# OPTML-Group/Unlearn-Saliency

Hardware: AMD Instinct MI355X
Metric: unlearn_steps_per_sec (ResNet-18/CIFAR-10 10%-forget, RL + SalUn mask, batch 256/GPU) (higher is better)
Workload: dtype f32

## Files before the change

include/salun.h:

```cpp
#ifndef SALUN_H
#define SALUN_H

#include <stddef.h>
#include <stdint.h>

#ifdef __cplusplus
extern "C" {
#endif

#define SALUN_OK 0
#define SALUN_EINVAL (-22)
#define SALUN_ENOSPC (-28)
#define SALUN_EIO (-5)

#define SALUN_MAX_THRESHOLDS 16

typedef void *salun_stream_t;

int salun_version(void);
const char *salun_strerror(int code);
const char *salun_arch(void);
int salun_clock_probe(unsigned long long *out , int samples, int spins, salun_stream_t stream);

int salun_saliency_accumulate(float *acc , const float *g ,
                              double scale, const float *sqnorm ,
                              double max_norm, int64_t n, salun_stream_t stream);

#define SALUN_TOPK_FORCE_FULL_SCAN 1u
#define SALUN_TOPK_VALUES_ONLY 2u
size_t salun_mask_topk_workspace_bytes(int64_t n, int nk);
int salun_mask_topk(const float *acc , int64_t n, const int64_t *ks ,
                    int nk, uint8_t *const *masks_out ,
                    void *ws , size_t ws_bytes, salun_stream_t stream);
int salun_mask_topk_ex(const float *acc , int64_t n, const int64_t *ks ,
                       int nk, uint8_t *const *masks_out ,
                       void *ws , size_t ws_bytes, unsigned flags, salun_stream_t stream);
int salun_mask_topk_status(const void *ws , int *route_out , int *error_out ,
                           salun_stream_t stream);
int salun_mask_topk_thresholds(const void *ws , int nk, float *tau_out ,
                               salun_stream_t stream);

int salun_mask_u8_to_i64(const uint8_t *m , int64_t *out , int64_t n,
                         salun_stream_t stream);
int salun_mask_i64_to_u8(const int64_t *m , uint8_t *out , int64_t n,
                         salun_stream_t stream);
int salun_mask_popcount(const uint8_t *m , int64_t n, int64_t *count ,
                        void *ws , size_t ws_bytes, salun_stream_t stream);

int salun_masked_sgd_step(float *p , const float *g , float *buf ,
                          const uint8_t *m , double lr, double mu,
                          double wd, int first_step, int64_t n, salun_stream_t stream);

size_t salun_reduce_workspace_bytes(int64_t n);
int salun_grad_sqnorm(const float *g , int64_t n, float *out ,
                      void *ws , size_t ws_bytes, salun_stream_t stream);

int salun_masked_adam_step(float *p , const float *g , float *m1 ,
                           float *v , const uint8_t *mask ,
                           const float *sqnorm , double max_norm,
                           double gscale, double lr, double b1, double b2, double eps,
                           double wd, int step, int64_t n, salun_stream_t stream);

int salun_adam_coefficients(int64_t *step , double lr, double b1, double b2, float *coef ,
                            salun_stream_t stream);
int salun_masked_adam_step_coef(float *p , const float *g , float *m1 , float *v ,
                                const uint8_t *mask , const float *sqnorm ,
                                double max_norm, double gscale, const float *coef , double b1, double b2,
                                double eps, double wd, int64_t n, salun_stream_t stream);

int salun_adam_ema_step(float *p , const float *g , float *m1 , float *v ,
                        float *shadow , const uint8_t *mask ,
                        const float *sqnorm , double max_norm, double gscale, double lr, double b1,
                        double b2, double eps, double wd, double mu, int step, int64_t n, salun_stream_t stream);
int salun_adam_ema_step_coef(float *p , const float *g , float *m1 , float *v ,
                             float *shadow , const uint8_t *mask ,
                             const float *sqnorm , double max_norm, double gscale,
                             const float *coef , double b1, double b2, double eps, double wd, double mu,
                             int64_t n, salun_stream_t stream);

int salun_qsample(const float *x0 , const float *e ,
                  const float *sqrt_ab , const float *sqrt_1mab ,
                  const int64_t *t , int64_t T, float *xt , int64_t B,
                  int64_t chw, salun_stream_t stream);

size_t salun_sqerr_workspace_bytes(int64_t B, int64_t chw);
int salun_sqerr_loss(const float *a , const float *b , int64_t B,
                     int64_t chw, double coef, float *loss ,
                     float *per_sample , float *dloss_db ,
                     void *ws , size_t ws_bytes, salun_stream_t stream);

int salun_fim_square_accumulate(float *F , float *tmp , double n_data,
                                int64_t n, salun_stream_t stream);

int salun_conv2d_forward(const float *x , const float *w , const float *bias ,
                         float *y , int N, int C, int H, int W, int K, int R, int stride, int pad,
                         int P, int Q, salun_stream_t stream);
int salun_conv2d_forward_fused(const float *x , const float *w , const float *bias ,
                               const float *nbias , const float *addend ,
                               float *y , int N, int C, int H, int W, int K, int R, int stride, int pad,
                               int P, int Q, void *ws , size_t ws_bytes, salun_stream_t stream);
size_t salun_conv2d_data_workspace_bytes(int N, int outC, int outH, int outW, int R, int conv_stride);
int salun_conv2d_backward_data_ws(const float *dy , const float *w , const float *addend ,
                                  float *dx , int N, int C, int H, int W, int K, int R, int stride, int pad,
                                  int P, int Q, void *ws , size_t ws_bytes, salun_stream_t stream);
int salun_conv2d_backward_data(const float *dy , const float *w , float *dx , int N, int C,
                               int H, int W, int K, int R, int stride, int pad, int P, int Q,
                               salun_stream_t stream);
int salun_conv2d_backward_data_add(const float *dy , const float *w , const float *addend ,
                                   float *dx , int N, int C, int H, int W, int K, int R, int stride, int pad,
                                   int P, int Q, salun_stream_t stream);
size_t salun_channel_sum_workspace_bytes(int N, int K);
int salun_channel_sum(const float *dy , float *out , int N, int K, int HW, int accumulate,
                      void *ws , size_t ws_bytes, salun_stream_t stream);
size_t salun_conv2d_wgrad_workspace_bytes(int N, int C, int K, int R, int P, int Q);
int salun_conv2d_backward_weight(const float *x , const float *dy , float *dw , int N, int C,
                                 int H, int W, int K, int R, int stride, int pad, int P, int Q, int accumulate,
                                 void *ws , size_t ws_bytes, salun_stream_t stream);
#define SALUN_WGRAD_SHARED 1u
int salun_conv2d_backward_weight_ex(const float *x , const float *dy , float *dw , int N, int C,
                                    int H, int W, int K, int R, int stride, int pad, int P, int Q, int accumulate,
                                    unsigned flags, void *ws , size_t ws_bytes, salun_stream_t stream);
#define SALUN_ROUTE_FORWARD 0
#define SALUN_ROUTE_BACKWARD_DATA 1
#define SALUN_ROUTE_BACKWARD_WEIGHT 2
#define SALUN_ROUTE_EPI 2u
#define SALUN_ROUTE_W_UNALIGNED 4u
#define SALUN_ROUTE_OUT_UNALIGNED 8u
#define SALUN_ROUTE_IN_UNALIGNED 16u
int salun_conv2d_route(int direction, int N, int C, int H, int W, int K, int R, int stride, int pad, int P, int Q,
                       unsigned flags, size_t ws_bytes, char *buf, size_t buflen, int *nsplit );

size_t salun_conv3x3_pack_bytes(int K, int C, int dgrad);
#define SALUN_PACK_MAX_JOBS 32
typedef struct {
  const float *w;
  float *img_fwd;
  float *img_dgrad;
  int32_t K, C;
} salun_pack_job_t;
int salun_conv3x3_pack_weights(const salun_pack_job_t *jobs , int njobs, salun_stream_t stream);
int salun_conv3x3_packed(const float *x , const float *img , const float *bias ,
                         const float *nbias , const float *addend , float *y ,
                         int N, int Cred, int H, int W, int Kout, int cfg, salun_stream_t stream);

int salun_conv2d_bf16_supported(int C, int K, int R, int stride, int pad);
int salun_conv2d_bf16_pack_weights(const float *w , uint16_t *wp , int K, int C, int R,
                                   salun_stream_t stream);
#define SALUN_BF16_PACK_MAX_JOBS 64
typedef struct {
  const float *w;
  uint16_t *wp;
  int32_t K, C, R, transposed;
} salun_bf16_pack_job_t;
int salun_bf16_pack_weights_batch(const salun_bf16_pack_job_t *jobs, int n, salun_stream_t stream);
size_t salun_conv2d_bf16_data_workspace_bytes(int N, int H, int W, int C, int K, int R, int stride, int pad);
int salun_conv2d_bf16_forward(const uint16_t *x , const uint16_t *wp , const float *bias ,
                              const float *nbias , const uint16_t *addend ,
                              uint16_t *y , int N, int H, int W, int C, int K, int R, int stride, int pad,
                              void *ws , size_t ws_bytes, salun_stream_t stream);
int salun_conv2d_bf16_backward_data(const uint16_t *dy , const uint16_t *wp ,
                                    const uint16_t *addend , uint16_t *dx , int N, int H, int W,
                                    int C, int K, int R, int stride, int pad, void *ws , size_t ws_bytes,
                                    salun_stream_t stream);
size_t salun_conv2d_bf16_wgrad_workspace_bytes(int N, int H, int W, int C, int K, int R, int stride, int pad);
int salun_conv2d_bf16_backward_weight(const uint16_t *x , const uint16_t *dy , float *dw ,
                                      float *db , int N, int H, int W, int C, int K, int R, int stride,
                                      int pad, int accumulate, void *ws , size_t ws_bytes,
                                      salun_stream_t stream);
size_t salun_colsum_bf16_workspace_bytes(int K);
int salun_colsum_bf16(const uint16_t *dy , float *db , float *dnb , int64_t M, int K,
                      int images, int accumulate, void *ws , size_t ws_bytes, salun_stream_t stream);
int salun_conv2d_bf16_backward_weight_ex(const uint16_t *x , const uint16_t *dy , float *dw ,
                                         float *db , float *dnb , int N, int H, int W, int C,
                                         int K, int R, int stride, int pad, int accumulate, void *ws ,
                                         size_t ws_bytes, salun_stream_t stream);
#define SALUN_ROUTE_RING_SHIFT 8
#define SALUN_ROUTE_RING(v) ((unsigned)((v) + 1) << SALUN_ROUTE_RING_SHIFT)
#define SALUN_ROUTE_WGRAD_TN_SHIFT 12
#define SALUN_ROUTE_WGRAD_TN(v) ((unsigned)((v) + 1) << SALUN_ROUTE_WGRAD_TN_SHIFT)
int salun_conv2d_bf16_route(int direction, int N, int H, int W, int C, int K, int R, int stride, int pad, unsigned flags,
                            size_t ws_bytes, char *buf, size_t buflen, int *nsplit );

size_t salun_gn_bf16_workspace_bytes(int N, int C, int HW, int G);
int salun_gn_bf16_forward(const uint16_t *x , const float *gamma , const float *beta ,
                          uint16_t *y , float *mr , float *ab , int N, int C, int HW, int G,
                          double eps, int silu, void *ws , size_t ws_bytes, salun_stream_t stream);
int salun_gn_bf16_backward(const uint16_t *dy , const uint16_t *x , const float *gamma ,
                           const float *mr , const float *ab , uint16_t *dx , float *dgamma ,
                           float *dbeta , int N, int C, int HW, int G, int silu, int accumulate, void *ws ,
                           size_t ws_bytes, salun_stream_t stream);

int salun_attn_supported(int D);
int salun_attn_forward(const uint16_t *q , const uint16_t *k , const uint16_t *v , uint16_t *o ,
                       float *lse , int B, int H, int Nq, int Nk, int D, long long q_bs, int q_ld,
                       long long k_bs, int k_ld, long long v_bs, int v_ld, long long o_bs, int o_ld, double scale,
                       salun_stream_t stream);
int salun_attn_backward(const uint16_t *q , const uint16_t *k , const uint16_t *v ,
                        const uint16_t *o , const uint16_t *d_o , const float *lse ,
                        uint16_t *dq , uint16_t *dk , uint16_t *dv , float *dsum , int B, int H,
                        int Nq, int Nk, int D, long long q_bs, int q_ld, long long k_bs, int k_ld, long long v_bs, int v_ld,
                        long long o_bs, int o_ld, long long do_bs, int do_ld, double scale, salun_stream_t stream);

size_t salun_ln_bf16_workspace_bytes(int64_t rows, int C);
int salun_ln_bf16_forward(const uint16_t *x , const float *gamma , const float *beta ,
                          uint16_t *y , float *stats , int64_t rows, int C, double eps,
                          salun_stream_t stream);
int salun_ln_bf16_backward(const uint16_t *dy , const uint16_t *x , const float *gamma ,
                           const float *stats , uint16_t *dx , float *dgamma , float *dbeta ,
                           int64_t rows, int C, int accumulate, void *ws , size_t ws_bytes, salun_stream_t stream);
int salun_geglu_bf16_forward(const uint16_t *h , uint16_t *out , int64_t rows, int F, salun_stream_t stream);
int salun_geglu_bf16_backward(const uint16_t *h , const uint16_t *dy , uint16_t *dh , int64_t rows,
                              int F, salun_stream_t stream);

size_t salun_bn_workspace_bytes(int C);
int salun_bn_forward(const float *x , const float *res , float *y ,
                     const float *gamma , const float *beta , float *running_mean ,
                     float *running_var , long long *num_batches_tracked ,
                     float *save_mean , float *save_invstd ,
                     int N, int C, int HW, int training, double momentum, double eps, int relu, void *ws ,
                     size_t ws_bytes, salun_stream_t stream);
int salun_bn_backward(const float *dy , const float *y , const float *x ,
                      const float *gamma , const float *save_mean , const float *save_invstd ,
                      float *dx , float *dres , float *dgamma , float *dbeta ,
                      float *grad_gamma_acc , float *grad_beta_acc ,
                      int N, int C, int HW, int training, int relu, void *ws , size_t ws_bytes,
                      salun_stream_t stream);

size_t salun_gn_workspace_bytes(int N, int C);
int salun_gn_forward(const float *x , float *y , const float *gamma , const float *beta ,
                     float *save_mean , float *save_rstd , int N, int C, int HW, int G, double eps,
                     int silu, salun_stream_t stream);
int salun_gn_backward(const float *dz , const float *x , const float *gamma ,
                      const float *beta , const float *save_mean , const float *save_rstd ,
                      float *dx , float *dgamma , float *dbeta ,
                      float *grad_gamma_acc , float *grad_beta_acc ,
                      int N, int C, int HW, int G, int silu, void *ws , size_t ws_bytes,
                      salun_stream_t stream);

int salun_gn_backward_fused(const float *dz , const float *x , const float *gamma ,
                            const float *beta , const float *save_mean , const float *save_rstd ,
                            const float *addend , float *dx , float *dgamma ,
                            float *dbeta , float *grad_gamma_acc ,
                            float *grad_beta_acc , float *nk_sum ,
                            float *csum , float *csum_acc , int N, int C, int HW, int G,
                            int silu, void *ws , size_t ws_bytes, salun_stream_t stream);

int salun_param_diff(const float *p , const float *p0 , float *out , int64_t n,
                     salun_stream_t stream);
int salun_soft_threshold_step(float *p , const float *p0 , const float *tau ,
                              int64_t n, salun_stream_t stream);

size_t salun_ewc_workspace_bytes(int64_t n);
int salun_ewc_penalty_grad(const float *p , const float *p_star , const float *F ,
                           float *g , double lambda, float *loss_out , int64_t n,
                           void *ws , size_t ws_bytes, salun_stream_t stream);

int salun_image_batch(const uint8_t *data , const int64_t *idx ,
                      const int32_t *crop , const uint8_t *flip ,
                      float *out , int64_t B, int H, int W, int C, int pad,
                      salun_stream_t stream);

#define SALUN_GEMM_MAX_JOBS 32
#define SALUN_GEMM_MAX_SEGS 32
typedef struct {
  const float *A , *B ;
  int32_t K;
  int32_t a_i, a_k, b_j, b_k;
} salun_gemm_seg_t;
typedef struct {
  float *C ;
  const float *bias ;
  int32_t M, N, ldc;
  int32_t seg0, nseg;
  int32_t accumulate;
} salun_gemm_job_t;
size_t salun_gemm_f32_workspace_bytes(const salun_gemm_job_t *jobs , int njobs,
                                      const salun_gemm_seg_t *segs , int nsegs,
                                      int batch_outer, int batch_inner);
int salun_gemm_f32(const salun_gemm_job_t *jobs , int njobs, const salun_gemm_seg_t *segs , int nsegs,
                   int batch_outer, int batch_inner, const int64_t *batch_strides ,
                   double alpha, void *ws , size_t ws_bytes, salun_stream_t stream);
typedef struct {
  int32_t tile, nsplit, nsplit_wanted, njobs, nsegs;
  int64_t tiles;
  int32_t nchunks[SALUN_GEMM_MAX_JOBS], per[SALUN_GEMM_MAX_JOBS], empty_shares[SALUN_GEMM_MAX_JOBS];
  int32_t tile0[SALUN_GEMM_MAX_JOBS], fast_tiles[SALUN_GEMM_MAX_JOBS];
  int32_t amode[SALUN_GEMM_MAX_SEGS], bmode[SALUN_GEMM_MAX_SEGS], chunk0[SALUN_GEMM_MAX_SEGS];
} salun_gemm_route_t;
int salun_gemm_f32_route(const salun_gemm_job_t *jobs , int njobs, const salun_gemm_seg_t *segs , int nsegs,
                         int batch_outer, int batch_inner, const int64_t *batch_strides ,
                         const void *ws , size_t ws_bytes, salun_gemm_route_t *out );
size_t salun_colsum_f32_workspace_bytes(int64_t M, int N);
int salun_colsum_f32(const float *x , float *out , int64_t M, int N, int64_t ld, int accumulate,
                     void *ws , size_t ws_bytes, salun_stream_t stream);
int salun_softmax_rows(float *s , int64_t rows, int n, int ld, salun_stream_t stream);
int salun_softmax_rows_backward(const float *p , float *dp , int64_t rows, int n, int ld,
                                double scale, salun_stream_t stream);

int salun_gemm_bf16_supported(int64_t M, int N, int K);
int salun_gemm_bf16_nt(const void *x , const void *w , const float *bias ,
                       const void *addend , void *y , int64_t M, int N, int K,
                       int variant, salun_stream_t stream);
int salun_gemm_bf16_tn_supported(int64_t M, int Na, int Nb);
size_t salun_gemm_bf16_tn_workspace_bytes(int64_t M, int Na, int Nb, int variant);
int salun_gemm_bf16_tn(const void *dy , const void *x , float *dw , int64_t M, int Na, int Nb,
                       int accumulate, int variant, void *ws , size_t ws_bytes, salun_stream_t stream);
#define SALUN_GEMM_BF16_NT 0
#define SALUN_GEMM_BF16_TN 1
int salun_gemm_bf16_route(int op, int64_t M, int N, int K, int variant, size_t ws_bytes, char *buf, size_t buflen,
                          int *nsplit );
int salun_pack_bf16(const float *w , void *wp , int N, int K, int transposed, salun_stream_t stream);

int salun_dropout(const float *x , float *y , int64_t n_samples, int64_t chw,
                  int64_t sample_offset, double p, uint64_t seed,
                  const uint64_t *seed_dev , salun_stream_t stream);
int salun_u64_add(uint64_t *value , uint64_t inc, salun_stream_t stream);

size_t salun_iu_dot_workspace_bytes(int B, int64_t n);
int salun_iu_conv_dot(const float *y2 , const float *dy , int B, int64_t n, double *out ,
                      void *ws , size_t ws_bytes, salun_stream_t stream);
int salun_iu_bn_dot(const float *x , const float *dy , const float *running_mean ,
                    const float *running_var , double eps, const float *u0_gamma ,
                    const float *u0_beta , const float *u1_gamma , const float *u1_beta ,
                    int B, int C, int HW, double *out , void *ws , size_t ws_bytes,
                    salun_stream_t stream);
int salun_iu_linear_dot(const float *x , const float *dy , const float *u0_w ,
                        const float *u0_b , const float *u1_w , const float *u1_b ,
                        int B, int M, int K, double *out , salun_stream_t stream);
int salun_iu_recurrence(const double *ab , int64_t n, double N, double *out ,
                        salun_stream_t stream);
int salun_iu_apply(float *p , const float *v , const float *g0 , const double *beta ,
                   const uint8_t *mask , double alpha, int64_t n, salun_stream_t stream);

size_t salun_ff_conv_sq_workspace_bytes(int G, int B, int C, int K, int R, int P, int Q);
int salun_ff_conv_sq(const float *x , const float *dy , const float *w , float *F ,
                     int G, int B, int C, int H, int W, int K, int R, int stride, int pad, int P, int Q,
                     void *ws , size_t ws_bytes, salun_stream_t stream);
int salun_ff_linear_sq(const float *x , const float *dy , const float *w , float *F ,
                       int G, int B, int M, int K, salun_stream_t stream);
size_t salun_ff_vec_sq_workspace_bytes(int G, int C);
int salun_ff_vec_sq(const float *x , const float *dy , const float *running_mean ,
                    const float *running_var , double eps, const float *w , int G, int B,
                    int C, int HW, float *F_gamma , float *F_beta , void *ws ,
                    size_t ws_bytes, salun_stream_t stream);
int salun_ff_apply(float *p , const float *F , const int64_t *table , int nparam, int64_t ntiles,
                   double nbatches, double alpha, uint64_t seed, salun_stream_t stream);

int salun_fill_uniform(float *out , int64_t n, uint64_t seed, double lo, double hi,
                       salun_stream_t stream);
int salun_fill_normal(float *out , int64_t n, uint64_t seed, double mean, double std,
                      salun_stream_t stream);
int salun_fill_u8(uint8_t *out , int64_t n, uint64_t seed, salun_stream_t stream);

#define SALUN_SAMPLER_ANCESTRAL 0
#define SALUN_SAMPLER_GENERALIZED 1
int salun_sampler_step(const float *x_t , const float *eps_cond , const float *eps_null ,
                       double cond_scale, const float *abar , int table_len, int idx_t, int idx_next, int variant,
                       double eta, const float *noise , uint64_t seed,
                       const int64_t *image_ids , int64_t step, float *x_next ,
                       float *x0 , int64_t B, int64_t chw, salun_stream_t stream);

int salun_sampler_noise(float *out , uint64_t seed, const int64_t *image_ids , int64_t step, int64_t B,
                        int64_t chw, salun_stream_t stream);

size_t salun_minmax_workspace_bytes(int64_t n);
int salun_minmax(const float *x , int64_t n, float *lohi , void *ws , size_t ws_bytes,
                 salun_stream_t stream);

int salun_images_to_u8(const float *x , uint8_t *out , int64_t B, int C, int HW, int rescaled,
                       const float *range , salun_stream_t stream);

int salun_ldm_ddim_step(const float *x , const float *eps2 , int guided, double scale,
                        double c_s1m, double c_sqrt_at, double c_dir, double c_sqrt_aprev, double c_sigma,
                        const float *z , float *x_prev , float *x0_out , int64_t B,
                        int64_t chw, salun_stream_t stream);

size_t salun_esd_loss_workspace_bytes(int64_t B, int64_t chw);
int salun_esd_loss(const float *e_n , const float *e_0p , int64_t B, int64_t chw,
                   double negative_guidance, float *loss , float *d_e_n ,
                   float *target , void *ws , size_t ws_bytes, salun_stream_t stream);

#define SALUN_PRUNE_MAX_SEGMENTS 512
size_t salun_prune_workspace_bytes(int64_t n_sel);
int salun_prune_global(float *p , float *buf , uint8_t *keep , int64_t n,
                       const int64_t *segs , int nseg, int64_t n_sel, int64_t alive, int64_t k_prune,
                       const float *rnd , unsigned flags, void *ws , size_t ws_bytes,
                       salun_stream_t stream);
int salun_prune_status(const void *ws , int64_t n_sel, int ranked, int *route_out ,
                       int *error_out , salun_stream_t stream);
int salun_prune_count_zeros(const float *p , int64_t n, const int64_t *segs , int nseg,
                            int64_t n_sel, int64_t *count , salun_stream_t stream);

#define SALUN_CLS_HEAD_MAX_C 8192
#define SALUN_CLS_HEAD_MAX_K 1024
size_t salun_cls_head_workspace_bytes(int64_t B, int C, int K);
int salun_cls_head_forward(const float *x , const float *w , const float *bias ,
                           const int64_t *labels , float *pooled , float *logits ,
                           float *p , float *loss , float *loss_mean ,
                           double *loss_sum , int64_t *hits ,
                           int64_t *count , int64_t B, int C, int HW, int K, void *ws ,
                           size_t ws_bytes, salun_stream_t stream);
int salun_cls_head_backward(const float *p , const float *pooled , const float *w ,
                            const int64_t *labels , const float *grad_out ,
                            float *dlogits , float *dx , float *dw ,
                            float *db , int accumulate_w, int accumulate_b, int64_t B, int C, int HW,
                            int K, salun_stream_t stream);

int salun_maxpool2x2_forward(const float *x , float *y , uint8_t *idx ,
                             int64_t NC, int H, int W, salun_stream_t stream);
int salun_maxpool2x2_backward(const float *dy , const uint8_t *idx , float *dx ,
                              int64_t NC, int H, int W, salun_stream_t stream);

#ifdef __cplusplus
}
#endif
#endif
```

unlearn_saliency_amd/_lib.py:

```python
from __future__ import annotations

import ctypes
import os
import subprocess

_HERE = os.path.dirname(os.path.abspath(__file__))
LIB_PATH = os.environ.get("SALUN_LIB") or os.path.join(_HERE, "libsalun.so")
CSRC_DIR = os.path.join(_HERE, "csrc")

SALUN_OK = 0
SALUN_EINVAL = -22
SALUN_ENOSPC = -28
SALUN_EIO = -5
SALUN_MAX_THRESHOLDS = 16
SALUN_TOPK_FORCE_FULL_SCAN = 1
SALUN_TOPK_VALUES_ONLY = 2
SALUN_WGRAD_SHARED = 1

c_void_p, c_int, c_int64, c_uint64 = ctypes.c_void_p, ctypes.c_int, ctypes.c_int64, ctypes.c_uint64
c_double, c_size_t = ctypes.c_double, ctypes.c_size_t

class GemmSeg(ctypes.Structure):
    _fields_ = [("A", c_void_p), ("B", c_void_p), ("K", ctypes.c_int32), ("a_i", ctypes.c_int32),
                ("a_k", ctypes.c_int32), ("b_j", ctypes.c_int32), ("b_k", ctypes.c_int32)]


class GemmJob(ctypes.Structure):
    _fields_ = [("C", c_void_p), ("bias", c_void_p), ("M", ctypes.c_int32), ("N", ctypes.c_int32),
                ("ldc", ctypes.c_int32), ("seg0", ctypes.c_int32), ("nseg", ctypes.c_int32),
                ("accumulate", ctypes.c_int32)]


class GemmRoute(ctypes.Structure):
    _fields_ = [(n, ctypes.c_int32) for n in ("tile", "nsplit", "nsplit_wanted", "njobs", "nsegs")] + \
               [("tiles", ctypes.c_int64)] + \
               [(n, ctypes.c_int32 * 32) for n in ("nchunks", "per", "empty_shares", "tile0", "fast_tiles", "amode", "bmode",
                                                   "chunk0")]


class PackJob(ctypes.Structure):
    _fields_ = [("w", c_void_p), ("img_fwd", c_void_p), ("img_dgrad", c_void_p), ("K", ctypes.c_int32),
                ("C", ctypes.c_int32)]


class Bf16PackJob(ctypes.Structure):
    _fields_ = [("w", c_void_p), ("wp", c_void_p), ("K", ctypes.c_int32), ("C", ctypes.c_int32), ("R", ctypes.c_int32),
                ("transposed", ctypes.c_int32)]


SALUN_BF16_PACK_MAX_JOBS = 64
SALUN_GEMM_MAX_JOBS = 32
SALUN_GEMM_MAX_SEGS = 32
SALUN_CLS_HEAD_MAX_C = 8192
SALUN_CLS_HEAD_MAX_K = 1024

SIGNATURES = {
    "salun_version": (c_int, []),
    "salun_strerror": (ctypes.c_char_p, [c_int]),
    "salun_arch": (ctypes.c_char_p, []),
    "salun_clock_probe": (c_int, [c_void_p, c_int, c_int, c_void_p]),
    "salun_saliency_accumulate": (c_int, [c_void_p, c_void_p, c_double, c_void_p, c_double, c_int64, c_void_p]),
    "salun_mask_topk_workspace_bytes": (c_size_t, [c_int64, c_int]),
    "salun_mask_topk": (c_int, [c_void_p, c_int64, ctypes.POINTER(c_int64), c_int, ctypes.POINTER(c_void_p),
                                c_void_p, c_size_t, c_void_p]),
    "salun_mask_topk_ex": (c_int, [c_void_p, c_int64, ctypes.POINTER(c_int64), c_int, ctypes.POINTER(c_void_p),
                                   c_void_p, c_size_t, ctypes.c_uint, c_void_p]),
    "salun_mask_topk_status": (c_int, [c_void_p, ctypes.POINTER(c_int), ctypes.POINTER(c_int), c_void_p]),
    "salun_mask_topk_thresholds": (c_int, [c_void_p, c_int, c_void_p, c_void_p]),
    "salun_mask_u8_to_i64": (c_int, [c_void_p, c_void_p, c_int64, c_void_p]),
    "salun_mask_i64_to_u8": (c_int, [c_void_p, c_void_p, c_int64, c_void_p]),
    "salun_mask_popcount": (c_int, [c_void_p, c_int64, c_void_p, c_void_p, c_size_t, c_void_p]),
    "salun_masked_sgd_step": (c_int, [c_void_p, c_void_p, c_void_p, c_void_p, c_double, c_double, c_double, c_int,
                                      c_int64, c_void_p]),
    "salun_reduce_workspace_bytes": (c_size_t, [c_int64]),
    "salun_grad_sqnorm": (c_int, [c_void_p, c_int64, c_void_p, c_void_p, c_size_t, c_void_p]),
    "salun_masked_adam_step": (c_int, [c_void_p, c_void_p, c_void_p, c_void_p, c_void_p, c_void_p, c_double,
                                       c_double, c_double, c_double, c_double, c_double, c_double, c_int, c_int64,
                                       c_void_p]),
    "salun_adam_coefficients": (c_int, [c_void_p, c_double, c_double, c_double, c_void_p, c_void_p]),
    "salun_masked_adam_step_coef": (c_int, [c_void_p, c_void_p, c_void_p, c_void_p, c_void_p, c_void_p, c_double,
                                            c_double, c_void_p, c_double, c_double, c_double, c_double, c_int64,
                                            c_void_p]),
    "salun_adam_ema_step": (c_int, [c_void_p, c_void_p, c_void_p, c_void_p, c_void_p, c_void_p, c_void_p, c_double,
                                    c_double, c_double, c_double, c_double, c_double, c_double, c_double, c_int, c_int64,
                                    c_void_p]),
    "salun_adam_ema_step_coef": (c_int, [c_void_p, c_void_p, c_void_p, c_void_p, c_void_p, c_void_p, c_void_p, c_double,
                                         c_double, c_void_p, c_double, c_double, c_double, c_double, c_double, c_int64,
                                         c_void_p]),
    "salun_qsample": (c_int, [c_void_p, c_void_p, c_void_p, c_void_p, c_void_p, c_int64, c_void_p, c_int64, c_int64,
                              c_void_p]),
    "salun_sqerr_workspace_bytes": (c_size_t, [c_int64, c_int64]),
    "salun_sqerr_loss": (c_int, [c_void_p, c_void_p, c_int64, c_int64, c_double, c_void_p, c_void_p, c_void_p,
                                 c_void_p, c_size_t, c_void_p]),
    "salun_fim_square_accumulate": (c_int, [c_void_p, c_void_p, c_double, c_int64, c_void_p]),
    "salun_conv2d_forward": (c_int, [c_void_p, c_void_p, c_void_p, c_void_p] + [c_int] * 10 + [c_void_p]),
    "salun_conv2d_forward_fused": (c_int, [c_void_p] * 6 + [c_int] * 10 + [c_void_p, c_size_t, c_void_p]),
    "salun_conv2d_data_workspace_bytes": (c_size_t, [c_int] * 6),
    "salun_conv2d_backward_data_ws": (c_int, [c_void_p] * 4 + [c_int] * 10 + [c_void_p, c_size_t, c_void_p]),
    "salun_conv2d_backward_data": (c_int, [c_void_p, c_void_p, c_void_p] + [c_int] * 10 + [c_void_p]),
    "salun_channel_sum_workspace_bytes": (c_size_t, [c_int] * 2),
    "salun_channel_sum": (c_int, [c_void_p, c_void_p] + [c_int] * 4 + [c_void_p, c_size_t, c_void_p]),
    "salun_conv2d_wgrad_workspace_bytes": (c_size_t, [c_int] * 6),
    "salun_conv3x3_pack_bytes": (c_size_t, [c_int] * 3),
    "salun_conv3x3_pack_weights": (c_int, [c_void_p, c_int, c_void_p]),
    "salun_conv3x3_packed": (c_int, [c_void_p] * 6 + [c_int] * 6 + [c_void_p]),
    "salun_conv2d_backward_weight": (c_int, [c_void_p, c_void_p, c_void_p] + [c_int] * 11 + [c_void_p, c_size_t,
                                                                                          c_void_p]),
    "salun_conv2d_backward_weight_ex": (c_int, [c_void_p, c_void_p, c_void_p] + [c_int] * 11 + [ctypes.c_uint, c_void_p,
                                                                                                 c_size_t, c_void_p]),
    "salun_conv2d_route": (c_int, [c_int] * 11 + [ctypes.c_uint, c_size_t, ctypes.c_char_p, c_size_t,
                                   ctypes.POINTER(c_int)]),
    "salun_conv2d_bf16_supported": (c_int, [c_int] * 5),
    "salun_conv2d_bf16_pack_weights": (c_int, [c_void_p, c_void_p, c_int, c_int, c_int, c_void_p]),
    "salun_bf16_pack_weights_batch": (c_int, [c_void_p, c_int, c_void_p]),
    "salun_conv2d_bf16_data_workspace_bytes": (c_size_t, [c_int] * 8),
    "salun_conv2d_bf16_forward": (c_int, [c_void_p] * 6 + [c_int] * 8 + [c_void_p, c_size_t, c_void_p]),
    "salun_conv2d_bf16_backward_data": (c_int, [c_void_p] * 4 + [c_int] * 8 + [c_void_p, c_size_t, c_void_p]),
    "salun_conv2d_bf16_wgrad_workspace_bytes": (c_size_t, [c_int] * 8),
    "salun_conv2d_bf16_backward_weight": (c_int, [c_void_p] * 4 + [c_int] * 9 + [c_void_p, c_size_t, c_void_p]),
    "salun_colsum_bf16_workspace_bytes": (c_size_t, [c_int]),
    "salun_colsum_bf16": (c_int, [c_void_p, c_void_p, c_void_p, c_int64, c_int, c_int, c_int, c_void_p, c_size_t, c_void_p]),
    "salun_conv2d_bf16_backward_weight_ex": (c_int, [c_void_p] * 5 + [c_int] * 9 + [c_void_p, c_size_t, c_void_p]),
    "salun_conv2d_bf16_route": (c_int, [c_int] * 9 + [ctypes.c_uint, c_size_t, ctypes.c_char_p, c_size_t,
                                        ctypes.POINTER(c_int)]),
    "salun_gn_bf16_workspace_bytes": (c_size_t, [c_int] * 4),
    "salun_gn_bf16_forward": (c_int, [c_void_p] * 6 + [c_int] * 4 + [c_double, c_int, c_void_p, c_size_t, c_void_p]),
    "salun_gn_bf16_backward": (c_int, [c_void_p] * 8 + [c_int] * 6 + [c_void_p, c_size_t, c_void_p]),
    "salun_attn_supported": (c_int, [c_int]),
    "salun_attn_forward": (c_int, [c_void_p] * 5 + [c_int] * 5 + [ctypes.c_longlong, c_int] * 4 + [c_double, c_void_p]),
    "salun_attn_backward": (c_int, [c_void_p] * 10 + [c_int] * 5 + [ctypes.c_longlong, c_int] * 5 + [c_double, c_void_p]),
    "salun_ln_bf16_workspace_bytes": (c_size_t, [c_int64, c_int]),
    "salun_ln_bf16_forward": (c_int, [c_void_p] * 5 + [c_int64, c_int, c_double, c_void_p]),
    "salun_ln_bf16_backward": (c_int, [c_void_p] * 7 + [c_int64, c_int, c_int, c_void_p, c_size_t, c_void_p]),
    "salun_geglu_bf16_forward": (c_int, [c_void_p, c_void_p, c_int64, c_int, c_void_p]),
    "salun_geglu_bf16_backward": (c_int, [c_void_p, c_void_p, c_void_p, c_int64, c_int, c_void_p]),
    "salun_bn_workspace_bytes": (c_size_t, [c_int]),
    "salun_bn_forward": (c_int, [c_void_p] * 10 + [c_int] * 4 + [c_double, c_double, c_int, c_void_p, c_size_t, c_void_p]),
    "salun_bn_backward": (c_int, [c_void_p] * 12 + [c_int] * 5 + [c_void_p, c_size_t, c_void_p]),
    "salun_conv2d_backward_data_add": (c_int, [c_void_p] * 4 + [c_int] * 10 + [c_void_p]),
    "salun_gn_workspace_bytes": (c_size_t, [c_int, c_int]),
    "salun_gn_forward": (c_int, [c_void_p] * 6 + [c_int] * 4 + [c_double, c_int, c_void_p]),
    "salun_gn_backward": (c_int, [c_void_p] * 11 + [c_int] * 5 + [c_void_p, c_size_t, c_void_p]),
    "salun_gn_backward_fused": (c_int, [c_void_p] * 15 + [c_int] * 5 + [c_void_p, c_size_t, c_void_p]),
    "salun_param_diff": (c_int, [c_void_p, c_void_p, c_void_p, c_int64, c_void_p]),
    "salun_soft_threshold_step": (c_int, [c_void_p, c_void_p, c_void_p, c_int64, c_void_p]),
    "salun_ewc_workspace_bytes": (c_size_t, [c_int64]),
    "salun_ewc_penalty_grad": (c_int, [c_void_p] * 4 + [c_double, c_void_p, c_int64, c_void_p, c_size_t, c_void_p]),
    "salun_image_batch": (c_int, [c_void_p, c_void_p, c_void_p, c_void_p, c_void_p, c_int64, c_int, c_int, c_int,
                                  c_int, c_void_p]),
    "salun_gemm_f32_workspace_bytes": (c_size_t, [ctypes.POINTER(GemmJob), c_int, ctypes.POINTER(GemmSeg), c_int, c_int,
                                                  c_int]),
    "salun_gemm_f32": (c_int, [ctypes.POINTER(GemmJob), c_int, ctypes.POINTER(GemmSeg), c_int, c_int, c_int,
                               ctypes.POINTER(c_int64), c_double, c_void_p, c_size_t, c_void_p]),
    "salun_gemm_f32_route": (c_int, [ctypes.POINTER(GemmJob), c_int, ctypes.POINTER(GemmSeg), c_int, c_int, c_int,
                                     ctypes.POINTER(c_int64), c_void_p, c_size_t, ctypes.POINTER(GemmRoute)]),
    "salun_colsum_f32_workspace_bytes": (c_size_t, [c_int64, c_int]),
    "salun_colsum_f32": (c_int, [c_void_p, c_void_p, c_int64, c_int, c_int64, c_int, c_void_p, c_size_t, c_void_p]),
    "salun_softmax_rows": (c_int, [c_void_p, c_int64, c_int, c_int, c_void_p]),
    "salun_softmax_rows_backward": (c_int, [c_void_p, c_void_p, c_int64, c_int, c_int, c_double, c_void_p]),
    "salun_gemm_bf16_supported": (c_int, [c_int64, c_int, c_int]),
    "salun_gemm_bf16_nt": (c_int, [c_void_p, c_void_p, c_void_p, c_void_p, c_void_p, c_int64, c_int, c_int, c_int, c_void_p]),
    "salun_pack_bf16": (c_int, [c_void_p, c_void_p, c_int, c_int, c_int, c_void_p]),
    "salun_gemm_bf16_tn_supported": (c_int, [c_int64, c_int, c_int]),
    "salun_gemm_bf16_tn_workspace_bytes": (c_size_t, [c_int64, c_int, c_int, c_int]),
    "salun_gemm_bf16_tn": (c_int, [c_void_p, c_void_p, c_void_p, c_int64, c_int, c_int, c_int, c_int, c_void_p, c_size_t, c_void_p]),
    "salun_gemm_bf16_route": (c_int, [c_int, c_int64, c_int, c_int, c_int, c_size_t, ctypes.c_char_p, c_size_t,
                                      ctypes.POINTER(c_int)]),
    "salun_dropout": (c_int, [c_void_p, c_void_p, c_int64, c_int64, c_int64, c_double, c_uint64, c_void_p, c_void_p]),
    "salun_u64_add": (c_int, [c_void_p, c_uint64, c_void_p]),
    "salun_iu_dot_workspace_bytes": (c_size_t, [c_int, c_int64]),
    "salun_iu_conv_dot": (c_int, [c_void_p, c_void_p, c_int, c_int64, c_void_p, c_void_p, c_size_t, c_void_p]),
    "salun_iu_bn_dot": (c_int, [c_void_p] * 4 + [c_double] + [c_void_p] * 4 + [c_int] * 3 + [c_void_p, c_void_p,
                                                                                           c_size_t, c_void_p]),
    "salun_iu_linear_dot": (c_int, [c_void_p] * 6 + [c_int] * 3 + [c_void_p, c_void_p]),
    "salun_iu_recurrence": (c_int, [c_void_p, c_int64, c_double, c_void_p, c_void_p]),
    "salun_iu_apply": (c_int, [c_void_p] * 5 + [c_double, c_int64, c_void_p]),
    "salun_ff_conv_sq_workspace_bytes": (c_size_t, [c_int] * 7),
    "salun_ff_conv_sq": (c_int, [c_void_p] * 4 + [c_int] * 11 + [c_void_p, c_size_t, c_void_p]),
    "salun_ff_linear_sq": (c_int, [c_void_p] * 4 + [c_int] * 4 + [c_void_p]),
    "salun_ff_vec_sq_workspace_bytes": (c_size_t, [c_int, c_int]),
    "salun_ff_vec_sq": (c_int, [c_void_p] * 4 + [c_double, c_void_p] + [c_int] * 4 + [c_void_p] * 3
                        + [c_size_t, c_void_p]),
    "salun_ff_apply": (c_int, [c_void_p] * 3 + [c_int, c_int64, c_double, c_double, c_uint64, c_void_p]),
    "salun_fill_uniform": (c_int, [c_void_p, c_int64, c_uint64, c_double, c_double, c_void_p]),
    "salun_fill_normal": (c_int, [c_void_p, c_int64, c_uint64, c_double, c_double, c_void_p]),
    "salun_fill_u8": (c_int, [c_void_p, c_int64, c_uint64, c_void_p]),
    "salun_sampler_step": (c_int, [c_void_p, c_void_p, c_void_p, c_double, c_void_p, c_int, c_int, c_int, c_int,
                                   c_double, c_void_p, c_uint64, c_void_p, c_int64, c_void_p, c_void_p, c_int64,
                                   c_int64, c_void_p]),
    "salun_sampler_noise": (c_int, [c_void_p, c_uint64, c_void_p, c_int64, c_int64, c_int64, c_void_p]),
    "salun_minmax_workspace_bytes": (c_size_t, [c_int64]),
    "salun_minmax": (c_int, [c_void_p, c_int64, c_void_p, c_void_p, c_size_t, c_void_p]),
    "salun_images_to_u8": (c_int, [c_void_p, c_void_p, c_int64, c_int, c_int, c_int, c_void_p, c_void_p]),
    "salun_ldm_ddim_step": (c_int, [c_void_p, c_void_p, c_int] + [c_double] * 6 + [c_void_p, c_void_p, c_void_p, c_int64,
                                                                                   c_int64, c_void_p]),
    "salun_esd_loss_workspace_bytes": (c_size_t, [c_int64, c_int64]),
    "salun_esd_loss": (c_int, [c_void_p, c_void_p, c_int64, c_int64, c_double, c_void_p, c_void_p, c_void_p, c_void_p,
                               c_size_t, c_void_p]),
    "salun_prune_workspace_bytes": (c_size_t, [c_int64]),
    "salun_prune_global": (c_int, [c_void_p, c_void_p, c_void_p, c_int64, c_void_p, c_int, c_int64, c_int64, c_int64,
                                   c_void_p, ctypes.c_uint, c_void_p, c_size_t, c_void_p]),
    "salun_prune_status": (c_int, [c_void_p, c_int64, c_int, ctypes.POINTER(c_int), ctypes.POINTER(c_int), c_void_p]),
    "salun_prune_count_zeros": (c_int, [c_void_p, c_int64, c_void_p, c_int, c_int64, c_void_p, c_void_p]),
    "salun_cls_head_workspace_bytes": (c_size_t, [c_int64, c_int, c_int]),
    "salun_cls_head_forward": (c_int, [c_void_p] * 12 + [c_int64, c_int, c_int, c_int, c_void_p, c_size_t, c_void_p]),
    "salun_cls_head_backward": (c_int, [c_void_p] * 9 + [c_int, c_int, c_int64, c_int, c_int, c_int, c_void_p]),
    "salun_maxpool2x2_forward": (c_int, [c_void_p, c_void_p, c_void_p, c_int64, c_int, c_int, c_void_p]),
    "salun_maxpool2x2_backward": (c_int, [c_void_p, c_void_p, c_void_p, c_int64, c_int, c_int, c_void_p]),
}

_lib = None


def build(verbose: bool = False) -> str:
    cmd = ["make", "-C", CSRC_DIR, "-j4"] + ([] if verbose else ["-s"])
    subprocess.check_call(cmd)
    if not os.path.exists(LIB_PATH):
        raise RuntimeError(f"build did not produce {LIB_PATH}")
    return LIB_PATH


def lib() -> ctypes.CDLL:
    global _lib
    if _lib is None:
        if not os.path.exists(LIB_PATH):
            raise ImportError(
                f"{LIB_PATH} is missing: the SalUn HIP extension has not been built "
                f"(run `make -C {CSRC_DIR}` or `python -c 'import __graft_entry__ as g; g.build()'`). "
                "There is no CPU fallback.")
        L = ctypes.CDLL(LIB_PATH)
        for name, (res, args) in SIGNATURES.items():
            try:
                fn = getattr(L, name)
            except AttributeError as e:
                raise ImportError(f"{LIB_PATH} does not export {name}; rebuild it") from e
            fn.restype = res
            fn.argtypes = args
        _lib = L
    return _lib


class SalunError(RuntimeError):
    pass


def check(code: int, what: str) -> None:
    if code != SALUN_OK:
        msg = lib().salun_strerror(code).decode()
        raise SalunError(f"{what} failed: {msg} ({code})")
```

unlearn_saliency_amd/csrc/salun_conv_ring.hip:

```cpp
#include "salun_common.h"
#include <mutex>
#include <type_traits>
#include <unordered_set>

namespace {

typedef float f32x16 __attribute__((ext_vector_type(16)));
typedef __attribute__((address_space(3))) char *ring_lds_ptr_t;

constexpr int RCC = 8;
constexpr int RSTEPS = 36;
constexpr int RGROUPS = 9;

__device__ float g_ring_zero[256];

__device__ __forceinline__ void ring_dma16(const float *src, unsigned dst) {
  unsigned keep;
  asm volatile("s_mov_b32 %0, m0\n\ts_mov_b32 m0, %2\n\ts_nop 0\n\tglobal_load_lds_dwordx4 %1, off\n\ts_mov_b32 m0, %0"
               : "=&s"(keep)
               : "v"(src), "s"(dst)
               : "memory");
}

struct PackJobs {
  salun_pack_job_t job[SALUN_PACK_MAX_JOBS];
};

__global__ __launch_bounds__(256) void k_ring_pack(const PackJobs jobs) {
  const salun_pack_job_t jb = jobs.job[blockIdx.y];
  const int dgrad = blockIdx.z;
  float *__restrict__ img = dgrad ? jb.img_dgrad : jb.img_fwd;
  if (!img) return;
  const float *__restrict__ w = jb.w;
  const int K = jb.K, C = jb.C;
  const int rows = dgrad ? C : K, red = dgrad ? K : C;
  if (red % RCC != 0) return;
  const int nchunk = red / RCC, ntile = (rows + 31) / 32;
  const long long total = (long long)ntile * nchunk * RGROUPS * 64;
  for (long long i = (long long)blockIdx.x * 256 + threadIdx.x; i < total; i += (long long)gridDim.x * 256) {
    const int lane = (int)(i & 63);
    long long r = i >> 6;
    const int gq = (int)(r % RGROUPS);
    r /= RGROUPS;
    const int chunk = (int)(r % nchunk), tile = (int)(r / nchunk);
    const int lo = lane & 31, hi = lane >> 5, row = tile * 32 + lo;
    float v[4];
#pragma unroll
    for (int e = 0; e < 4; ++e) {
      const int s = 4 * gq + e, cp = s / 9, rs = s - 9 * cp, ch = chunk * RCC + 2 * cp + hi;
      float t = 0.f;
      if (row < rows) t = dgrad ? w[((size_t)ch * C + row) * 9 + (8 - rs)] : w[((size_t)row * C + ch) * 9 + rs];
      v[e] = t;
    }
    *reinterpret_cast<float4 *>(img + i * 4) = make_float4(v[0], v[1], v[2], v[3]);
  }
}

struct RingArgs {
  const float *x;
  const float *aimg;
  const float *bias;
  const float *nbias;
  const float *addend;
  const float *zero;
  float *y;
  int N, Cred, H, Kout;
  int NI, TP;
  int ntile_k, ntiles;
  int nchunk;
};

template <int LOGW, int PT, int KT, int WP, int WK, bool EPI>
__global__ __launch_bounds__(256, 2) void conv3x3_ring(const RingArgs g) {
  constexpr int W = 1 << LOGW, W4 = W / 4;
  constexpr int KTW = WK * KT, KB = KTW * 32;
  constexpr int A_BYTES = KTW * RGROUPS * 1024;
  constexpr int NA = KTW * RGROUPS;
  constexpr int NAW = (NA + 3) / 4;
  constexpr int NPW = 3;
  static_assert(WP * WK == 4, "four waves");
  extern __shared__ __attribute__((aligned(1024))) char lds[];

  const int tid = threadIdx.x, lane = tid & 63;
  const int wave = __builtin_amdgcn_readfirstlane(tid >> 6);
  const int lo = lane & 31, hi = lane >> 5;
  const int wp = wave % WP, wk = wave / WP;
  const int H = g.H, TP = g.TP, NI = g.NI, N = g.N, Cred = g.Cred;
  const int PRI = TP + 2;
  const int IRS = (W == 4 && NI > 1) ? 12 : PRI;
  const int PSZ = NI * IRS * W;
  const int PSZ4 = PSZ / 4;
  const int npiece = RCC * PSZ4;
  const int P_BYTES = ((npiece + 63) / 64) * 1024;
  const int STAGE = A_BYTES + P_BYTES;
  const int HW = H * W;
  const int tiles_per_img = (NI > 1) ? 1 : H / TP;
  const int nchunk = g.nchunk;
  const unsigned lds_base = (unsigned)(uintptr_t)(ring_lds_ptr_t)lds;

  const float *psrc[NPW];
  int pstep[NPW];
  bool pact[NPW];
  const float *asrc[NAW];
  auto setup_issue = [&](int tile) {
    const int kb = tile % g.ntile_k, ptile = tile / g.ntile_k;
    int n0, p0;
    if (NI > 1) { n0 = ptile * NI; p0 = 0; }
    else { n0 = ptile / tiles_per_img; p0 = (ptile - n0 * tiles_per_img) * TP; }
#pragma unroll
    for (int j = 0; j < NPW; ++j) {
      const int e = (wave + 4 * j) * 64 + lane;
      const int c = e / PSZ4, jj = e - c * PSZ4;
      const int row = jj >> (LOGW - 2), col4 = jj & (W4 - 1);
      const int ni = row / IRS, rr = row - ni * IRS;
      const int ih = p0 - 1 + rr, n = n0 + ni;
      const bool act = e < npiece && rr < PRI;
      const bool valid = act && n < N && ih >= 0 && ih < H;
      pact[j] = act;
      psrc[j] = valid ? g.x + ((size_t)(n * Cred + c) * H + ih) * W + 4 * col4 : g.zero + 4 * lane;
      pstep[j] = valid ? RCC * HW : 0;
    }
#pragma unroll
    for (int j = 0; j < NAW; ++j) {
      const int a = wave + 4 * j, t = a / RGROUPS, gq = a - t * RGROUPS;
      const int rt = min(kb * KTW + t, (g.Kout + 31) / 32 - 1);
      asrc[j] = g.aimg + ((size_t)rt * nchunk * RGROUPS + gq) * 256 + 4 * lane;
    }
  };
  auto issue = [&](int chunk, int stage) {
    const unsigned base = lds_base + stage * STAGE;
#pragma unroll
    for (int j = 0; j < NAW; ++j) {
      const int a = wave + 4 * j;
      if (NA % 4 == 0 || a < NA) {
        const float *p = asrc[j] + (size_t)chunk * (RGROUPS * 256);
        ring_dma16(p, base + a * 1024);
      }
    }
#pragma unroll
    for (int j = 0; j < NPW; ++j) {
      if (pact[j]) {
        const float *p = psrc[j] + (size_t)chunk * pstep[j];
        ring_dma16(p, base + A_BYTES + (wave + 4 * j) * 1024);
      }
    }
  };

  const int total = g.ntiles;
  int it_tile = blockIdx.x, it_chunk = 0;
  if (it_tile < total) {
    setup_issue(it_tile);
    issue(0, 0);
    it_chunk = 1;
    if (it_chunk == nchunk) { it_chunk = 0; it_tile += gridDim.x; if (it_tile < total) setup_issue(it_tile); }
  }
  int stage = 0;

  for (int tile = blockIdx.x; tile < total; tile += gridDim.x) {
    const int kb = tile % g.ntile_k, ptile = tile / g.ntile_k;
    int n0, p0;
    if (NI > 1) { n0 = ptile * NI; p0 = 0; }
    else { n0 = ptile / tiles_per_img; p0 = (ptile - n0 * tiles_per_img) * TP; }
    int q_l[PT], n_l[PT], p_l[PT], boff[PT];
    bool okL[PT], okR[PT];
#pragma unroll
    for (int pt = 0; pt < PT; ++pt) {
      const int mloc = (wp * PT + pt) * 32 + lo;
      q_l[pt] = mloc & (W - 1);
      const int pr = mloc >> LOGW;
      const int ni = pr / TP;
      p_l[pt] = pr - ni * TP;
      n_l[pt] = n0 + ni;
      boff[pt] = ((hi * PSZ) + (ni * IRS + p_l[pt]) * W + q_l[pt] - 1) * 4;
      okL[pt] = q_l[pt] != 0;
      okR[pt] = q_l[pt] != W - 1;
    }

    f32x16 acc[PT][KT];
#pragma unroll
    for (int pt = 0; pt < PT; ++pt)
#pragma unroll
      for (int t = 0; t < KT; ++t)
#pragma unroll
        for (int v = 0; v < 16; ++v) acc[pt][t][v] = 0.f;

    for (int ch = 0; ch < nchunk; ++ch) {
      if (ch > 0 || tile == (int)blockIdx.x) __builtin_amdgcn_s_waitcnt(0x0f70);
      __builtin_amdgcn_s_barrier();
      if (it_tile < total) {
        issue(it_chunk, stage ^ 1);
        if (++it_chunk == nchunk) { it_chunk = 0; it_tile += gridDim.x; if (it_tile < total) setup_issue(it_tile); }
      }
      const char *A = lds + stage * STAGE + (wk * KT * RGROUPS) * 1024 + lane * 16;
      const char *Pb = lds + stage * STAGE + A_BYTES;
      const char *bb[PT][RCC / 2];
#pragma unroll
      for (int pt = 0; pt < PT; ++pt)
#pragma unroll
        for (int cp = 0; cp < RCC / 2; ++cp) bb[pt][cp] = Pb + boff[pt] + cp * (2 * PSZ * 4);
      float4 a_cur[KT], a_nxt[KT];
      float b_cur[PT], b_nxt[PT];
      auto read_b = [&](int s, float (&bv)[PT]) {
        const int cp = s / 9, rs = s % 9, r = rs / 3, sx = rs % 3;
#pragma unroll
        for (int pt = 0; pt < PT; ++pt) bv[pt] = *reinterpret_cast<const float *>(bb[pt][cp] + (r * W + sx) * 4);
      };
      auto mask_b = [&](int s, float (&bv)[PT]) {
        const int sx = (s % 9) % 3;
#pragma unroll
        for (int pt = 0; pt < PT; ++pt) {
          if (sx == 0) bv[pt] = okL[pt] ? bv[pt] : 0.f;
          if (sx == 2) bv[pt] = okR[pt] ? bv[pt] : 0.f;
        }
      };
      auto read_a = [&](int gq, float4 (&av)[KT]) {
#pragma unroll
        for (int t = 0; t < KT; ++t) av[t] = *reinterpret_cast<const float4 *>(A + (t * RGROUPS + gq) * 1024);
      };
      read_a(0, a_cur);
      read_b(0, b_cur);
      mask_b(0, b_cur);
#pragma unroll
      for (int s = 0; s < RSTEPS; ++s) {
        if (s + 1 < RSTEPS) read_b(s + 1, b_nxt);
        if ((s & 3) == 0 && s + 4 < RSTEPS) read_a(s / 4 + 1, a_nxt);
        __builtin_amdgcn_sched_barrier(0);
#pragma unroll
        for (int pt = 0; pt < PT; ++pt)
#pragma unroll
          for (int t = 0; t < KT; ++t) {
            const float4 a4 = a_cur[t];
            const float av = (s & 3) == 0 ? a4.x : (s & 3) == 1 ? a4.y : (s & 3) == 2 ? a4.z : a4.w;
            acc[pt][t] = __builtin_amdgcn_mfma_f32_32x32x2f32(av, b_cur[pt], acc[pt][t], 0, 0, 0);
          }
        __builtin_amdgcn_sched_barrier(0);
        if (s + 1 < RSTEPS) mask_b(s + 1, b_nxt);
#pragma unroll
        for (int pt = 0; pt < PT; ++pt) b_cur[pt] = b_nxt[pt];
        if ((s & 3) == 3) {
#pragma unroll
          for (int t = 0; t < KT; ++t) a_cur[t] = a_nxt[t];
        }
      }
      stage ^= 1;
    }

    __builtin_amdgcn_s_waitcnt(0x0f70);
#pragma unroll
    for (int pt = 0; pt < PT; ++pt) {
      const int n_out = n_l[pt], p_out = p0 + p_l[pt];
      if (n_out < N) {
#pragma unroll
        for (int t = 0; t < KT; ++t) {
          const int kbase = kb * KB + (wk * KT + t) * 32 + 4 * hi;
          const size_t obase = (((size_t)n_out * g.Kout + kbase) * H + p_out) * W + q_l[pt];
          const size_t kstride = (size_t)HW;
          const int klast = g.Kout - 1 - kbase;
          float bv[16], nv[16], av[16];
          if (EPI) {
            if (g.bias) {
#pragma unroll
              for (int v = 0; v < 16; ++v) bv[v] = g.bias[kbase + max(min((v & 3) + 8 * (v >> 2), klast), -kbase)];
            }
            if (g.nbias) {
#pragma unroll
              for (int v = 0; v < 16; ++v)
                nv[v] = g.nbias[(size_t)n_out * g.Kout + kbase + max(min((v & 3) + 8 * (v >> 2), klast), -kbase)];
            }
            if (g.addend) {
#pragma unroll
              for (int v = 0; v < 16; ++v)
                av[v] = g.addend[obase + (long long)max(min((v & 3) + 8 * (v >> 2), klast), -kbase) * (long long)kstride];
            }
          }
#pragma unroll
          for (int v = 0; v < 16; ++v) {
            const int kr = (v & 3) + 8 * (v >> 2);
            if (kbase + kr < g.Kout) {
              float o = acc[pt][t][v];
              if (EPI) {
                if (g.bias) o += bv[v];
                if (g.nbias) o += nv[v];
                if (g.addend) o += av[v];
              }
              g.y[obase + kr * kstride] = o;
            }
          }
        }
      }
    }
  }
}

struct WgradRingArgs {
  const float *x;
  const float *dy;
  const float *zero;
  float *part;
  int N, C, K, nchunks;
};

template <int LOGW>
__global__ __launch_bounds__(256) void conv3x3_wgrad_ring(const WgradRingArgs g) {
  constexpr int W = 1 << LOGW, W4 = W / 4, H = W;
  constexpr int TP = (W * W >= 64) ? 64 / W : W;
  constexpr int NI = (W * W >= 64) ? 1 : 64 / (W * W);
  constexpr int PRI = TP + 2;
  constexpr int PSZ4 = NI * PRI * W4;
  constexpr int PRX = PSZ4 | 1;
  constexpr int DRW = 17;
  constexpr int D_BYTES = 64 * DRW * 16, X_BYTES = 64 * PRX * 16, STAGE = D_BYTES + X_BYTES;
  constexpr int NDU = DRW, NXU = PRX;
  constexpr int NDW = (NDU + 3) / 4, NXW = (NXU + 3) / 4;
  constexpr int TPI = (NI > 1) ? 1 : H / TP;
  extern __shared__ __attribute__((aligned(1024))) char lds[];
  const unsigned lds_base = (unsigned)(uintptr_t)(ring_lds_ptr_t)lds;

  const int tid = threadIdx.x, lane = tid & 63;
  const int wave = __builtin_amdgcn_readfirstlane(tid >> 6);
  const int lo = lane & 31, hi = lane >> 5;
  const int kt = wave & 1, ct = wave >> 1;
  const int k0 = blockIdx.x * 64, c0 = blockIdx.y * 64;
  const int split = blockIdx.z, nsplit = gridDim.z;
  const int N = g.N, C = g.C, K = g.K;
  constexpr int HW = H * W;

  constexpr int NEVER = 1 << 24;
  int d_lane[NDW], d_ni[NDW];
#pragma unroll
  for (int j = 0; j < NDW; ++j) {
    const int e = (wave + 4 * j) * 64 + lane;
    const int k = e / DRW, pc = e - k * DRW;
    const int pix = 4 * pc;
    const int ni = pix / (TP * W), rem = pix - ni * (TP * W);
    d_ni[j] = (pc == 16 || k0 + k >= K) ? NEVER : ni;
    d_lane[j] = (ni * K + k) * HW + rem;
  }
  int x_lane[NXW], x_ni[NXW], x_rr[NXW];
#pragma unroll
  for (int j = 0; j < NXW; ++j) {
    const int e = (wave + 4 * j) * 64 + lane;
    const int c = e / PRX, pc = e - c * PRX;
    const int row = pc / W4, col4 = pc - row * W4;
    const int ni = row / PRI, rr = row - ni * PRI;
    x_ni[j] = (pc >= PSZ4) ? NEVER : ni;
    x_rr[j] = rr;
    x_lane[j] = ((ni * C + c) * H + rr) * W + 4 * col4;
  }
  const float *const zero = g.zero + 4 * lane;
  auto issue_unit = [&](int u, int chunk, int stage) {
    int n0, p0;
    if (NI > 1) { n0 = chunk * NI; p0 = 0; }
    else { n0 = chunk / TPI; p0 = (chunk - n0 * TPI) * TP; }
    const unsigned base = lds_base + stage * STAGE;
    if (u < NDW) {
      const int j = u;
      if ((wave + 4 * j) < NDU) {
        const float *src = g.dy + ((size_t)(n0 * K + k0) * H + p0) * W;
        const float *p = (d_ni[j] < N - n0) ? src + d_lane[j] : zero;
        ring_dma16(p, base + (wave + 4 * j) * 1024);
      }
    } else {
      const int j = u - NDW;
      if ((wave + 4 * j) < NXU) {
        const float *src = g.x + ((long long)(n0 * C + c0) * H + (p0 - 1)) * W;
        const bool ok = x_ni[j] < N - n0 && x_rr[j] >= 1 - p0 && x_rr[j] < H + 1 - p0;
        const float *p = ok ? src + x_lane[j] : zero;
        ring_dma16(p, base + D_BYTES + (wave + 4 * j) * 1024);
      }
    }
  };

  f32x16 acc[9];
#pragma unroll
  for (int t = 0; t < 9; ++t)
#pragma unroll
    for (int v = 0; v < 16; ++v) acc[t][v] = 0.f;

  if (split < g.nchunks) {
#pragma unroll
    for (int u = 0; u < NDW + NXW; ++u) issue_unit(u, split, 0);
    int stage = 0;
    const int a_lane = (kt * 32 + lo) * (DRW * 16) + hi * 16;
    const int b_lane = D_BYTES + (ct * 32 + lo) * (PRX * 16) + hi * 16;
    for (int chunk = split; chunk < g.nchunks; chunk += nsplit) {
      __builtin_amdgcn_s_waitcnt(0x0f70);
      __builtin_amdgcn_s_barrier();
      const int nxt_chunk = chunk + nsplit;
      const bool more = nxt_chunk < g.nchunks;
      const char *A = lds + stage * STAGE + a_lane;
      const char *B = lds + stage * STAGE + b_lane;
      struct Row { float l; float4 v; float r; };
      struct Ops { float4 a; Row b0, b1, b2; };
      auto group_off = [&](int m) {
        const int pix = 8 * m, ni = pix / (TP * W), rem = pix - ni * (TP * W), p = rem / W, q0 = rem - p * W;
        return (ni * PRI + p) * W + q0;
      };
      auto read_row = [&](int off) {
        Row o;
        o.v = *reinterpret_cast<const float4 *>(B + off);
        if (W > 4) {
          typedef float f32x4v __attribute__((ext_vector_type(4)));
          typedef const volatile __attribute__((address_space(3))) f32x4v *lds_v4_t;
          const f32x4v lv = *(lds_v4_t)(ring_lds_ptr_t)(B + off - 16);
          const f32x4v rv = *(lds_v4_t)(ring_lds_ptr_t)(B + off + 16);
          o.l = lv.w;
          o.r = rv.x;
        } else {
          o.l = 0.f;
          o.r = 0.f;
        }
        return o;
      };
      auto read_group = [&](int m) {
        Ops o;
        o.a = *reinterpret_cast<const float4 *>(A + m * 32);
        const int off = group_off(m) * 4;
        o.b0 = read_row(off);
        o.b1 = read_row(off + W * 4);
        o.b2 = read_row(off + 2 * W * 4);
        return o;
      };
      auto mask_row = [&](int m, Row o) {
        if (W > 4) {
          const int q00 = (8 * m) & (W - 1);
          if (q00 == 0) o.l = hi ? o.l : 0.f;
          if (q00 == W - 8) o.r = hi ? 0.f : o.r;
        }
        return o;
      };
      auto pick = [](const Row &o, int i) {
        return i == 0 ? o.l : i == 1 ? o.v.x : i == 2 ? o.v.y : i == 3 ? o.v.z : i == 4 ? o.v.w : o.r;
      };
      Ops cur = read_group(0), nxt = cur;
      cur.b0 = mask_row(0, cur.b0); cur.b1 = mask_row(0, cur.b1); cur.b2 = mask_row(0, cur.b2);
#pragma unroll
      for (int m = 0; m < 8; ++m) {
        if (m + 1 < 8) nxt = read_group(m + 1);
        __builtin_amdgcn_sched_barrier(0);
#pragma unroll
        for (int e = 0; e < 4; ++e) {
          const float av = e == 0 ? cur.a.x : e == 1 ? cur.a.y : e == 2 ? cur.a.z : cur.a.w;
#pragma unroll
          for (int t = 0; t < 9; ++t) {
            const float bv = pick(t / 3 == 0 ? cur.b0 : t / 3 == 1 ? cur.b1 : cur.b2, e + t % 3);
            acc[t] = __builtin_amdgcn_mfma_f32_32x32x2f32(av, bv, acc[t], 0, 0, 0);
            if (t == 0) {
              __builtin_amdgcn_sched_barrier(0);
              const int u = 4 * m + e;
              if (u < NDW + NXW && more) issue_unit(u, nxt_chunk, stage ^ 1);
              __builtin_amdgcn_sched_barrier(0);
            }
          }
        }
        __builtin_amdgcn_sched_barrier(0);
        if (m + 1 < 8) {
          cur.a = nxt.a;
          cur.b0 = mask_row(m + 1, nxt.b0); cur.b1 = mask_row(m + 1, nxt.b1); cur.b2 = mask_row(m + 1, nxt.b2);
        }
      }
      stage ^= 1;
    }
  }
  static_assert(NDW + NXW <= 32, "one DMA unit per MFMA step");
  float *out = g.part + (size_t)split * K * C * 9;
  const int c = c0 + ct * 32 + lo;
#pragma unroll
  for (int t = 0; t < 9; ++t)
#pragma unroll
    for (int v = 0; v < 16; ++v) {
      const int k = k0 + kt * 32 + (v & 3) + 8 * (v >> 2) + 4 * hi;
      if (k < K) out[((size_t)t * K + k) * C + c] = acc[t][v];
    }
}

inline void ring_allow_lds(const void *fn) {
  static std::mutex mu;
  static std::unordered_set<uintptr_t> done;
  std::lock_guard<std::mutex> lk(mu);
  if (done.insert(reinterpret_cast<uintptr_t>(fn) ^ ((uintptr_t)(salun_device_bit() + 1) << 56)).second)
    (void)hipFuncSetAttribute(fn, hipFuncAttributeMaxDynamicSharedMemorySize, 160 * 1024);
}

inline const float *ring_zero_page() {
  static const float *page[64] = {nullptr};
  static std::mutex mu;
  const int b = salun_device_bit();
  std::lock_guard<std::mutex> lk(mu);
  if (!page[b]) {
    void *p = nullptr;
    if (hipGetSymbolAddress(&p, HIP_SYMBOL(g_ring_zero)) != hipSuccess) return nullptr;
    page[b] = static_cast<const float *>(p);
  }
  return page[b];
}

inline int ring_cu_count() {
  static int cus[64] = {0};
  const int b = salun_device_bit();
  if (cus[b] == 0) {
    int dev = 0, n = 0;
    if (hipGetDevice(&dev) != hipSuccess || hipDeviceGetAttribute(&n, hipDeviceAttributeMultiprocessorCount, dev) != hipSuccess || n <= 0)
      n = 256;
    cus[b] = n;
  }
  return cus[b];
}

struct RingTile { int tpix, kb; };

inline int ring_choose(int cfg, int N, int H, int W, int Kout) {
  if (cfg) return cfg;
  const long long pix = (long long)N * H * W;
  const int kb64 = (Kout + 63) / 64;
  if (pix / 256 * kb64 >= 512) return 1;
  if (pix / 128 * kb64 >= 512) return 2;
  if (pix / 64 * kb64 >= 384) return 3;
  return -1;
}

template <int LOGW, int PT, int KT, int WP, int WK>
int ring_launch(RingArgs a, int W, bool epi, int wgs_per_cu, hipStream_t st) {
  constexpr int TPIX = WP * PT * 32, KB = WK * KT * 32;
  const int HW = a.H * W;
  if (TPIX % W != 0) return SALUN_EINVAL;
  if (HW >= TPIX) {
    if (HW % TPIX != 0) return SALUN_EINVAL;
    a.NI = 1;
    a.TP = TPIX / W;
  } else {
    if (TPIX % HW != 0) return SALUN_EINVAL;
    a.NI = TPIX / HW;
    a.TP = a.H;
  }
  const int ptiles = (a.NI > 1) ? (a.N + a.NI - 1) / a.NI : a.N * (HW / TPIX);
  a.ntile_k = (a.Kout + KB - 1) / KB;
  a.ntiles = ptiles * a.ntile_k;
  a.nchunk = a.Cred / RCC;
  const int IRS = (W == 4 && a.NI > 1) ? 12 : a.TP + 2;
  if (IRS < a.TP + 2) return SALUN_EINVAL;
  const int PSZ = a.NI * IRS * W;
  const int npiece = RCC * PSZ / 4;
  if (npiece > 12 * 64) return SALUN_EINVAL;
  const size_t stage = (size_t)(WK * KT) * RGROUPS * 1024 + (size_t)((npiece + 63) / 64) * 1024;
  const size_t ldsb = 2 * stage;
  if (ldsb > 80 * 1024) return SALUN_EINVAL;
  int grid = wgs_per_cu * ring_cu_count();
  if (grid > a.ntiles) grid = a.ntiles;
  if (epi) {
    ring_allow_lds(reinterpret_cast<const void *>(conv3x3_ring<LOGW, PT, KT, WP, WK, true>));
    hipLaunchKernelGGL((conv3x3_ring<LOGW, PT, KT, WP, WK, true>), dim3(grid), dim3(256), ldsb, st, a);
  } else {
    ring_allow_lds(reinterpret_cast<const void *>(conv3x3_ring<LOGW, PT, KT, WP, WK, false>));
    hipLaunchKernelGGL((conv3x3_ring<LOGW, PT, KT, WP, WK, false>), dim3(grid), dim3(256), ldsb, st, a);
  }
  SALUN_LAUNCH_CHECK();
  return SALUN_OK;
}

template <int LOGW>
int ring_dispatch(const RingArgs &a, int cfg, bool epi, int wgs_per_cu, hipStream_t st) {
  constexpr int W = 1 << LOGW;
  switch (ring_choose(cfg, a.N, a.H, W, a.Kout)) {
    case 1: return ring_launch<LOGW, 2, 2, 4, 1>(a, W, epi, wgs_per_cu, st);
    case 2: return ring_launch<LOGW, 1, 2, 4, 1>(a, W, epi, wgs_per_cu, st);
    case 3: return ring_launch<LOGW, 1, 1, 2, 2>(a, W, epi, wgs_per_cu, st);
    case 4: return ring_launch<LOGW, 1, 4, 4, 1>(a, W, epi, wgs_per_cu, st);
    case 5: return ring_launch<LOGW, 1, 2, 2, 2>(a, W, epi, wgs_per_cu, st);
    default: return SALUN_EINVAL;
  }
}

}

bool salun_ring_wgrad_fits(int N, int C, int H, int W, int K, int nchunks, bool in_al16) {
  if (H != W || C % 64 != 0 || K % 32 != 0 || !in_al16) return false;
  if ((long long)N * C * H * W >= (1ll << 31) || (long long)N * K * H * W >= (1ll << 31)) return false;
  if (W != 4 && W != 8 && W != 16 && W != 32) return false;
  const int NI = (W * W >= 64) ? 1 : 64 / (W * W);
  return nchunks == ((NI > 1) ? (N + NI - 1) / NI : N * (W * W / 64));
}

int salun_ring_wgrad_launch(const float *x, const float *dy, float *part, int N, int C, int H, int W, int K, int nsplit,
                            int nchunks, hipStream_t st) {
  if (!salun_ring_wgrad_fits(N, C, H, W, K, nchunks, salun_aligned16(x) && salun_aligned16(dy))) return SALUN_EINVAL;
  const float *zero = ring_zero_page();
  if (!zero) return SALUN_EIO;
  WgradRingArgs a{x, dy, zero, part, N, C, K, nchunks};
  dim3 grid((K + 63) / 64, C / 64, nsplit);
  auto launch = [&](auto logw) {
    constexpr int LOGW = decltype(logw)::value;
    constexpr int W_ = 1 << LOGW, TP_ = (W_ * W_ >= 64) ? 64 / W_ : W_, NI_ = (W_ * W_ >= 64) ? 1 : 64 / (W_ * W_);
    constexpr int PRX_ = (NI_ * (TP_ + 2) * (W_ / 4)) | 1;
    const size_t ldsb = 2 * (size_t)(64 * 17 * 16 + 64 * PRX_ * 16);
    ring_allow_lds(reinterpret_cast<const void *>(conv3x3_wgrad_ring<LOGW>));
    hipLaunchKernelGGL((conv3x3_wgrad_ring<LOGW>), grid, dim3(256), ldsb, st, a);
  };
  switch (W) {
    case 4: launch(std::integral_constant<int, 2>{}); break;
    case 8: launch(std::integral_constant<int, 3>{}); break;
    case 16: launch(std::integral_constant<int, 4>{}); break;
    default: launch(std::integral_constant<int, 5>{}); break;
  }
  SALUN_LAUNCH_CHECK();
  return SALUN_OK;
}

SALUN_EXPORT size_t salun_conv3x3_pack_bytes(int K, int C, int dgrad) {
  const int rows = dgrad ? C : K, red = dgrad ? K : C;
  if (rows <= 0 || red <= 0 || red % RCC != 0) return 0;
  return (size_t)((rows + 31) / 32) * (red / RCC) * RGROUPS * 1024;
}

SALUN_EXPORT int salun_conv3x3_pack_weights(const salun_pack_job_t *jobs, int njobs, salun_stream_t stream) {
  if (!jobs || njobs <= 0) return SALUN_EINVAL;
  for (int j0 = 0; j0 < njobs; j0 += SALUN_PACK_MAX_JOBS) {
    PackJobs pj{};
    const int n = (njobs - j0 < SALUN_PACK_MAX_JOBS) ? njobs - j0 : SALUN_PACK_MAX_JOBS;
    long long most = 0;
    for (int j = 0; j < n; ++j) {
      const salun_pack_job_t &jb = jobs[j0 + j];
      if (!jb.w || jb.K <= 0 || jb.C <= 0 || (!jb.img_fwd && !jb.img_dgrad)) return SALUN_EINVAL;
      if ((jb.img_fwd && (jb.C % RCC != 0 || !salun_aligned16(jb.img_fwd))) ||
          (jb.img_dgrad && (jb.K % RCC != 0 || !salun_aligned16(jb.img_dgrad))))
        return SALUN_EINVAL;
      pj.job[j] = jb;
      const long long it = (long long)(((jb.K > jb.C ? jb.K : jb.C) + 31) / 32) * ((jb.K > jb.C ? jb.K : jb.C) / RCC + 1) *
                           RGROUPS * 64;
      if (it > most) most = it;
    }
    int gx = (int)((most + 255) / 256);
    if (gx > 1024) gx = 1024;
    hipLaunchKernelGGL(k_ring_pack, dim3(gx, n, 2), dim3(256), 0, salun_hip_stream(stream), pj);
    SALUN_LAUNCH_CHECK();
  }
  return SALUN_OK;
}

SALUN_EXPORT int salun_conv3x3_packed(const float *x, const float *img, const float *bias, const float *nbias,
                                      const float *addend, float *y, int N, int Cred, int H, int W, int Kout, int cfg,
                                      salun_stream_t stream) {
  if (!x || !img || !y || N <= 0 || Cred <= 0 || Kout <= 0 || H <= 0) return SALUN_EINVAL;
  if (Cred % RCC != 0 || !salun_aligned16(x) || !salun_aligned16(img)) return SALUN_EINVAL;
  if ((long long)N * Cred * H * W >= (1ll << 31) || (long long)N * Kout * H * W >= (1ll << 31)) return SALUN_EINVAL;
  RingArgs a{};
  a.x = x; a.aimg = img; a.bias = bias; a.nbias = nbias; a.addend = addend; a.y = y;
  a.zero = ring_zero_page();
  if (!a.zero) return SALUN_EIO;
  a.N = N; a.Cred = Cred; a.H = H; a.Kout = Kout;
  const bool epi = bias || nbias || addend;
  const int wgs = (cfg >> 8) ? (cfg >> 8) : 2;
  hipStream_t st = salun_hip_stream(stream);
  switch (W) {
    case 4: return ring_dispatch<2>(a, cfg & 255, epi, wgs, st);
    case 8: return ring_dispatch<3>(a, cfg & 255, epi, wgs, st);
    case 16: return ring_dispatch<4>(a, cfg & 255, epi, wgs, st);
    case 32: return ring_dispatch<5>(a, cfg & 255, epi, wgs, st);
    default: return SALUN_EINVAL;
  }
}
```

unlearn_saliency_amd/csrc/salun_norm.hip:

```cpp
#include "salun_common.h"

namespace {

constexpr int BN_MAX_SPLIT = 64;


struct BnWalk {
  int n, i, dn, di, hw4;
  __device__ __forceinline__ BnWalk(int n_lo, int hw4_) : hw4(hw4_) {
    const int t = threadIdx.x;
    n = n_lo + t / hw4_;
    i = t - (t / hw4_) * hw4_;
    dn = 256 / hw4_;
    di = 256 - dn * hw4_;
  }
  __device__ __forceinline__ void next() {
    n += dn;
    i += di;
    if (i >= hw4) { i -= hw4; ++n; }
  }
};

__global__ __launch_bounds__(256) void k_bn_stats_partial(const float *__restrict__ x, int N, int C, int HW, int nsplit,
                                                          double *__restrict__ partial) {
  __shared__ double lds[4];
  const int c = blockIdx.x, s = blockIdx.y;
  const int n_lo = (int)((int64_t)N * s / nsplit), n_hi = (int)((int64_t)N * (s + 1) / nsplit);
  float s1 = 0.f, s2 = 0.f;
  double d1 = 0.0, d2 = 0.0;
  const int hw4 = HW >> 2;
  const int work = (n_hi - n_lo) * hw4;
  int it = 0;
  BnWalk wk(n_lo, hw4);
#pragma unroll 2
  for (int e = threadIdx.x; e < work; e += 256, ++it, wk.next()) {
    const int n = wk.n, i = wk.i;
    const float4 v = reinterpret_cast<const float4 *>(x + ((size_t)n * C + c) * HW)[i];
    s1 += (v.x + v.y) + (v.z + v.w);
    s2 += (v.x * v.x + v.y * v.y) + (v.z * v.z + v.w * v.w);
    if ((it & 7) == 7) { d1 += s1; d2 += s2; s1 = 0.f; s2 = 0.f; }
  }
  d1 += s1; d2 += s2;
  const double t1 = salun_block_sum(d1, lds);
  const double t2 = salun_block_sum(d2, lds);
  if (threadIdx.x == 0) {
    partial[((size_t)c * nsplit + s) * 2 + 0] = t1;
    partial[((size_t)c * nsplit + s) * 2 + 1] = t2;
  }
}

__device__ __forceinline__ void bn_channel_stats(const double *__restrict__ partial, int c, int nsplit, double M,
                                                 float eps, float *s_out , bool publish,
                                                 float momentum, float *__restrict__ mean, float *__restrict__ invstd,
                                                 float *__restrict__ running_mean, float *__restrict__ running_var) {
  if (threadIdx.x < 64) {
    double s1 = 0.0, s2 = 0.0;
    if ((int)threadIdx.x < nsplit) {
      s1 = partial[((size_t)c * nsplit + threadIdx.x) * 2 + 0];
      s2 = partial[((size_t)c * nsplit + threadIdx.x) * 2 + 1];
    }
    s1 = salun_wave_sum(s1);
    s2 = salun_wave_sum(s2);
    if (threadIdx.x == 0) {
      const double mu = s1 / M;
      double var = s2 / M - mu * mu;
      if (var < 0.0) var = 0.0;
      const float is = (float)(1.0 / sqrt(var + (double)eps));
      s_out[0] = (float)mu;
      s_out[1] = is;
      if (publish) {
        mean[c] = (float)mu;
        invstd[c] = is;
        if (running_mean) {
          running_mean[c] = (1.f - momentum) * running_mean[c] + momentum * (float)mu;
          const double unbiased = (M > 1.0) ? var * M / (M - 1.0) : var;
          running_var[c] = (1.f - momentum) * running_var[c] + momentum * (float)unbiased;
        }
      }
    }
  }
  __syncthreads();
}

template <bool RELU, bool RES, bool TRAIN>
__global__ __launch_bounds__(256) void k_bn_apply(const float *__restrict__ x, const float *__restrict__ res,
                                                  float *__restrict__ y, const double *__restrict__ partial,
                                                  float *__restrict__ mean, float *__restrict__ invstd,
                                                  const float *__restrict__ gamma, const float *__restrict__ beta,
                                                  float *__restrict__ running_mean, float *__restrict__ running_var,
                                                  long long *__restrict__ num_batches_tracked, int N, int C, int HW,
                                                  int nsplit, float eps, float momentum) {
  __shared__ float st[2];
  const int c = blockIdx.x, s = blockIdx.y;
  if (TRAIN) {
    if (num_batches_tracked && c == 0 && s == 0 && threadIdx.x == 0) *num_batches_tracked += 1;
    bn_channel_stats(partial, c, nsplit, (double)N * HW, eps, st, s == 0, momentum, mean, invstd, running_mean,
                     running_var);
  } else {
    if (threadIdx.x == 0) {
      st[0] = running_mean[c];
      st[1] = 1.0f / sqrtf(running_var[c] + eps);
      if (s == 0) { mean[c] = st[0]; invstd[c] = st[1]; }
    }
    __syncthreads();
  }
  const float a = st[1] * gamma[c];
  const float b = beta[c] - st[0] * a;
  const int n_lo = (int)((int64_t)N * s / nsplit), n_hi = (int)((int64_t)N * (s + 1) / nsplit);
  const int hw4 = HW >> 2;
  const int work = (n_hi - n_lo) * hw4;
  BnWalk wk(n_lo, hw4);
#pragma unroll 2
  for (int e = threadIdx.x; e < work; e += 256, wk.next()) {
    const int n = wk.n, i = wk.i;
    const size_t off = ((size_t)n * C + c) * HW;
    const float4 v = reinterpret_cast<const float4 *>(x + off)[i];
    float4 o;
    o.x = v.x * a + b; o.y = v.y * a + b; o.z = v.z * a + b; o.w = v.w * a + b;
    if (RES) {
      const float4 r = reinterpret_cast<const float4 *>(res + off)[i];
      o.x += r.x; o.y += r.y; o.z += r.z; o.w += r.w;
    }
    if (RELU) {
      o.x = o.x > 0.f ? o.x : 0.f; o.y = o.y > 0.f ? o.y : 0.f;
      o.z = o.z > 0.f ? o.z : 0.f; o.w = o.w > 0.f ? o.w : 0.f;
    }
    reinterpret_cast<float4 *>(y + off)[i] = o;
  }
}

template <bool RELU>
__global__ __launch_bounds__(256) void k_bn_bwd_partial(const float *__restrict__ dy, const float *__restrict__ y,
                                                        const float *__restrict__ x, const float *__restrict__ mean,
                                                        const float *__restrict__ invstd, int N, int C, int HW,
                                                        int nsplit, double *__restrict__ partial) {
  __shared__ double lds[4];
  const int c = blockIdx.x, s = blockIdx.y;
  const int n_lo = (int)((int64_t)N * s / nsplit), n_hi = (int)((int64_t)N * (s + 1) / nsplit);
  const float mu = mean[c], is = invstd[c];
  float s1 = 0.f, s2 = 0.f;
  double d1 = 0.0, d2 = 0.0;
  const int hw4 = HW >> 2;
  const int work = (n_hi - n_lo) * hw4;
  int it = 0;
  BnWalk wk(n_lo, hw4);
#pragma unroll 2
  for (int e = threadIdx.x; e < work; e += 256, ++it, wk.next()) {
    const int n = wk.n, i = wk.i;
    const size_t off = ((size_t)n * C + c) * HW;
    float4 g = reinterpret_cast<const float4 *>(dy + off)[i];
    const float4 xv = reinterpret_cast<const float4 *>(x + off)[i];
    if (RELU) {
      const float4 yv = reinterpret_cast<const float4 *>(y + off)[i];
      g.x = yv.x > 0.f ? g.x : 0.f; g.y = yv.y > 0.f ? g.y : 0.f;
      g.z = yv.z > 0.f ? g.z : 0.f; g.w = yv.w > 0.f ? g.w : 0.f;
    }
    s1 += (g.x + g.y) + (g.z + g.w);
    s2 += (g.x * ((xv.x - mu) * is) + g.y * ((xv.y - mu) * is)) + (g.z * ((xv.z - mu) * is) + g.w * ((xv.w - mu) * is));
    if ((it & 7) == 7) { d1 += s1; d2 += s2; s1 = 0.f; s2 = 0.f; }
  }
  d1 += s1; d2 += s2;
  const double t1 = salun_block_sum(d1, lds);
  const double t2 = salun_block_sum(d2, lds);
  if (threadIdx.x == 0) {
    partial[((size_t)c * nsplit + s) * 2 + 0] = t1;
    partial[((size_t)c * nsplit + s) * 2 + 1] = t2;
  }
}

template <bool RELU, bool TRAIN, bool DRES>
__global__ __launch_bounds__(256) void k_bn_bwd_apply(const float *__restrict__ dy, const float *__restrict__ y,
                                                      const float *__restrict__ x, const float *__restrict__ mean,
                                                      const float *__restrict__ invstd,
                                                      const float *__restrict__ gamma,
                                                      const double *__restrict__ partial, float *__restrict__ dgamma,
                                                      float *__restrict__ dbeta, float *__restrict__ gacc,
                                                      float *__restrict__ bacc, float *__restrict__ dx,
                                                      float *__restrict__ dres, int N, int C, int HW, int nsplit,
                                                      float inv_m) {
  __shared__ float sg[2];
  const int c = blockIdx.x, s = blockIdx.y;
  if (threadIdx.x < 64) {
    double s1 = 0.0, s2 = 0.0;
    if ((int)threadIdx.x < nsplit) {
      s1 = partial[((size_t)c * nsplit + threadIdx.x) * 2 + 0];
      s2 = partial[((size_t)c * nsplit + threadIdx.x) * 2 + 1];
    }
    s1 = salun_wave_sum(s1);
    s2 = salun_wave_sum(s2);
    if (threadIdx.x == 0) {
      sg[0] = (float)s1;
      sg[1] = (float)s2;
      if (s == 0) {
        dbeta[c] = (float)s1;
        dgamma[c] = (float)s2;
        if (gacc) gacc[c] += (float)s2;
        if (bacc) bacc[c] += (float)s1;
      }
    }
  }
  __syncthreads();
  const float mu = mean[c], is = invstd[c];
  const float gi = gamma[c] * is;
  const float kb = sg[0] * inv_m, kg = sg[1] * inv_m;
  const int n_lo = (int)((int64_t)N * s / nsplit), n_hi = (int)((int64_t)N * (s + 1) / nsplit);
  const int hw4 = HW >> 2;
  const int work = (n_hi - n_lo) * hw4;
  BnWalk wk(n_lo, hw4);
#pragma unroll 2
  for (int e = threadIdx.x; e < work; e += 256, wk.next()) {
    const int n = wk.n, i = wk.i;
    const size_t off = ((size_t)n * C + c) * HW;
    float4 g = reinterpret_cast<const float4 *>(dy + off)[i];
    if (RELU) {
      const float4 yv = reinterpret_cast<const float4 *>(y + off)[i];
      g.x = yv.x > 0.f ? g.x : 0.f; g.y = yv.y > 0.f ? g.y : 0.f;
      g.z = yv.z > 0.f ? g.z : 0.f; g.w = yv.w > 0.f ? g.w : 0.f;
    }
    if (DRES) reinterpret_cast<float4 *>(dres + off)[i] = g;
    float4 o;
    if (TRAIN) {
      const float4 xv = reinterpret_cast<const float4 *>(x + off)[i];
      o.x = gi * (g.x - (kb + ((xv.x - mu) * is) * kg));
      o.y = gi * (g.y - (kb + ((xv.y - mu) * is) * kg));
      o.z = gi * (g.z - (kb + ((xv.z - mu) * is) * kg));
      o.w = gi * (g.w - (kb + ((xv.w - mu) * is) * kg));
    } else {
      o.x = gi * g.x; o.y = gi * g.y; o.z = gi * g.z; o.w = gi * g.w;
    }
    reinterpret_cast<float4 *>(dx + off)[i] = o;
  }
}

inline int bn_nsplit(int N, int C) {
  int ns = (1024 + C - 1) / C;
  if (ns > N) ns = N;
  if (ns > BN_MAX_SPLIT) ns = BN_MAX_SPLIT;
  if (ns < 1) ns = 1;
  return ns;
}

}

SALUN_EXPORT size_t salun_bn_workspace_bytes(int C) {
  return sizeof(double) * 2 * (size_t)(C > 0 ? C : 0) * BN_MAX_SPLIT;
}

SALUN_EXPORT int salun_bn_forward(const float *x, const float *res, float *y, const float *gamma, const float *beta,
                                  float *running_mean, float *running_var, long long *num_batches_tracked,
                                  float *save_mean, float *save_invstd, int N, int C, int HW, int training,
                                  double momentum, double eps, int relu, void *ws, size_t ws_bytes,
                                  salun_stream_t stream) {
  if (!x || !y || !gamma || !beta || !save_mean || !save_invstd || N < 1 || C < 1 || HW < 4 || (HW & 3))
    return SALUN_EINVAL;
  if (!training && (!running_mean || !running_var)) return SALUN_EINVAL;
  if (!salun_aligned16(x) || !salun_aligned16(y) || (res && !salun_aligned16(res))) return SALUN_EINVAL;
  hipStream_t st = salun_hip_stream(stream);
  const int ns = bn_nsplit(N, C);
  double *partial = static_cast<double *>(ws);
  if (training) {
    if (!ws || ws_bytes < salun_bn_workspace_bytes(C)) return SALUN_ENOSPC;
    hipLaunchKernelGGL(k_bn_stats_partial, dim3(C, ns), dim3(256), 0, st, x, N, C, HW, ns, partial);
    SALUN_LAUNCH_CHECK();
  }
#define SALUN_BN_APPLY(RELU_, RES_, TRAIN_)                                                                       \
  hipLaunchKernelGGL((k_bn_apply<RELU_, RES_, TRAIN_>), dim3(C, ns), dim3(256), 0, st, x, res, y, partial,         \
                     save_mean, save_invstd, gamma, beta, running_mean, running_var, num_batches_tracked, N, C,  \
                     HW, ns, (float)eps, (float)momentum)
  const bool r = relu != 0, a = res != nullptr, t = training != 0;
  if (r && a && t) SALUN_BN_APPLY(true, true, true);
  else if (r && a) SALUN_BN_APPLY(true, true, false);
  else if (r && t) SALUN_BN_APPLY(true, false, true);
  else if (r) SALUN_BN_APPLY(true, false, false);
  else if (a && t) SALUN_BN_APPLY(false, true, true);
  else if (a) SALUN_BN_APPLY(false, true, false);
  else if (t) SALUN_BN_APPLY(false, false, true);
  else SALUN_BN_APPLY(false, false, false);
#undef SALUN_BN_APPLY
  SALUN_LAUNCH_CHECK();
  return SALUN_OK;
}

SALUN_EXPORT int salun_bn_backward(const float *dy, const float *y, const float *x, const float *gamma,
                                   const float *save_mean, const float *save_invstd, float *dx, float *dres,
                                   float *dgamma, float *dbeta, float *grad_gamma_acc, float *grad_beta_acc, int N,
                                   int C, int HW, int training, int relu, void *ws, size_t ws_bytes,
                                   salun_stream_t stream) {
  if (!dy || !x || !gamma || !save_mean || !save_invstd || !dx || !dgamma || !dbeta || N < 1 || C < 1 || HW < 4 ||
      (HW & 3) || (relu && !y))
    return SALUN_EINVAL;
  if (!ws || ws_bytes < salun_bn_workspace_bytes(C)) return SALUN_ENOSPC;
  if (!salun_aligned16(dy) || !salun_aligned16(x) || !salun_aligned16(dx) || (y && !salun_aligned16(y)) ||
      (dres && !salun_aligned16(dres)))
    return SALUN_EINVAL;
  hipStream_t st = salun_hip_stream(stream);
  const int ns = bn_nsplit(N, C);
  double *partial = static_cast<double *>(ws);
  if (relu) hipLaunchKernelGGL(k_bn_bwd_partial<true>, dim3(C, ns), dim3(256), 0, st, dy, y, x, save_mean, save_invstd, N, C, HW, ns, partial);
  else hipLaunchKernelGGL(k_bn_bwd_partial<false>, dim3(C, ns), dim3(256), 0, st, dy, y, x, save_mean, save_invstd, N, C, HW, ns, partial);
  SALUN_LAUNCH_CHECK();
  const float inv_m = (float)(1.0 / ((double)N * HW));
#define SALUN_BN_BWD(RELU_, TRAIN_, DRES_)                                                                          \
  hipLaunchKernelGGL((k_bn_bwd_apply<RELU_, TRAIN_, DRES_>), dim3(C, ns), dim3(256), 0, st, dy, y, x, save_mean,   \
                     save_invstd, gamma, partial, dgamma, dbeta, grad_gamma_acc, grad_beta_acc, dx, dres, N, C, HW, \
                     ns, inv_m)
  const bool r = relu != 0, t = training != 0, d = dres != nullptr;
  if (r && t && d) SALUN_BN_BWD(true, true, true);
  else if (r && t) SALUN_BN_BWD(true, true, false);
  else if (r && d) SALUN_BN_BWD(true, false, true);
  else if (r) SALUN_BN_BWD(true, false, false);
  else if (t && d) SALUN_BN_BWD(false, true, true);
  else if (t) SALUN_BN_BWD(false, true, false);
  else if (d) SALUN_BN_BWD(false, false, true);
  else SALUN_BN_BWD(false, false, false);
#undef SALUN_BN_BWD
  SALUN_LAUNCH_CHECK();
  return SALUN_OK;
}

namespace {

constexpr int GN_ITEMS = 16;
constexpr int GN_MAX_SEG = 1024;

__device__ __forceinline__ float gn_sigmoid(float y) { return 1.0f / (1.0f + expf(-y)); }

__device__ __forceinline__ float seg_sum(float v, int r) {
  for (int off = 1; off < r; off <<= 1) v += __shfl_xor(v, off, 64);
  return v;
}

template <bool SILU, int ITEMS>
__global__ __launch_bounds__(256) void k_gn_fwd(const float *__restrict__ x, float *__restrict__ y,
                                                const float *__restrict__ gamma, const float *__restrict__ beta,
                                                float *__restrict__ mean, float *__restrict__ rstd, int C, int HW,
                                                int G, float eps) {
  constexpr bool CACHED = ITEMS > 0;
  __shared__ double lds[4];
  __shared__ float st[2];
  const int ng = blockIdx.x, n = ng / G, g = ng - n * G;
  const int cpg = C / G;
  const int L = cpg * HW, nvec = L >> 2;
  const size_t base = ((size_t)n * C + (size_t)g * cpg) * HW;
  const float4 *xv = reinterpret_cast<const float4 *>(x + base);
  float4 v[CACHED ? ITEMS : 1];
  float s1 = 0.f, s2 = 0.f;
  double d1 = 0.0, d2 = 0.0;
  if (CACHED) {
#pragma unroll
    for (int i = 0; i < (CACHED ? ITEMS : 1); ++i) {
      const int e = threadIdx.x + i * 256;
      if (e < nvec) v[i] = xv[e];
    }
#pragma unroll
    for (int i = 0; i < (CACHED ? ITEMS : 1); ++i) {
      const int e = threadIdx.x + i * 256;
      if (e < nvec) {
        s1 += (v[i].x + v[i].y) + (v[i].z + v[i].w);
        s2 += (v[i].x * v[i].x + v[i].y * v[i].y) + (v[i].z * v[i].z + v[i].w * v[i].w);
      }
    }
    d1 = s1; d2 = s2;
  } else {
    int it = 0;
    for (int e = threadIdx.x; e < nvec; e += 256, ++it) {
      const float4 t = xv[e];
      s1 += (t.x + t.y) + (t.z + t.w);
      s2 += (t.x * t.x + t.y * t.y) + (t.z * t.z + t.w * t.w);
      if ((it & 15) == 15) { d1 += s1; d2 += s2; s1 = 0.f; s2 = 0.f; }
    }
    d1 += s1; d2 += s2;
  }
  const double t1 = salun_block_sum(d1, lds);
  const double t2 = salun_block_sum(d2, lds);
  if (threadIdx.x == 0) {
    const double mu = t1 / L;
    double var = t2 / L - mu * mu;
    if (var < 0.0) var = 0.0;
    st[0] = (float)mu;
    st[1] = (float)(1.0 / sqrt(var + (double)eps));
    mean[ng] = st[0];
    rstd[ng] = st[1];
  }
  __syncthreads();
  const float mu = st[0], rs = st[1];
  const int hw4 = HW >> 2;
  float4 *yv = reinterpret_cast<float4 *>(y + base);
  auto apply = [&](int e, float4 t) {
    const int c = g * cpg + e / hw4;
    const float a = rs * gamma[c];
    const float b = beta[c] - mu * a;
    float4 o;
    o.x = t.x * a + b; o.y = t.y * a + b; o.z = t.z * a + b; o.w = t.w * a + b;
    if (SILU) {
      o.x = o.x * gn_sigmoid(o.x); o.y = o.y * gn_sigmoid(o.y);
      o.z = o.z * gn_sigmoid(o.z); o.w = o.w * gn_sigmoid(o.w);
    }
    yv[e] = o;
  };
  if (CACHED) {
#pragma unroll
    for (int i = 0; i < (CACHED ? ITEMS : 1); ++i) {
      const int e = threadIdx.x + i * 256;
      if (e < nvec) apply(e, v[i]);
    }
  } else {
    for (int e = threadIdx.x; e < nvec; e += 256) apply(e, xv[e]);
  }
}

template <bool SILU, int ITEMS, bool EXTRA>
__global__ __launch_bounds__(256) void k_gn_bwd(const float *__restrict__ dz, const float *__restrict__ x,
                                                const float *__restrict__ gamma, const float *__restrict__ beta,
                                                const float *__restrict__ mean, const float *__restrict__ rstd,
                                                float *__restrict__ dx, float *__restrict__ part_dgamma,
                                                float *__restrict__ part_dbeta, int C, int HW, int G,
                                                const float *__restrict__ addend, float *__restrict__ nk_sum) {
  constexpr bool CACHED = ITEMS > 0;
  __shared__ float seg_g[GN_MAX_SEG], seg_b[GN_MAX_SEG];
  __shared__ float grp[2];
  const int ng = blockIdx.x, n = ng / G, g = ng - n * G;
  const int cpg = C / G;
  const int L = cpg * HW, nvec = L >> 2, hw4 = HW >> 2;
  const size_t base = ((size_t)n * C + (size_t)g * cpg) * HW;
  const float4 *xv = reinterpret_cast<const float4 *>(x + base);
  const float4 *gv = reinterpret_cast<const float4 *>(dz + base);
  const float mu = mean[ng], rs = rstd[ng];
  const int r = hw4 < 64 ? hw4 : 64;
  const int segs_per_ch = hw4 / r;
  float4 xc[CACHED ? ITEMS : 1], dc[CACHED ? ITEMS : 1];
  float gac[CACHED ? ITEMS : 1], bec[CACHED ? ITEMS : 1];

  auto dy_of = [&](float ga, float be, float4 xt, float4 gt, float4 &xh) {
    xh.x = (xt.x - mu) * rs; xh.y = (xt.y - mu) * rs; xh.z = (xt.z - mu) * rs; xh.w = (xt.w - mu) * rs;
    if (SILU) {
      const float y0 = xh.x * ga + be, y1 = xh.y * ga + be, y2 = xh.z * ga + be, y3 = xh.w * ga + be;
      const float s0 = gn_sigmoid(y0), s1 = gn_sigmoid(y1), s2 = gn_sigmoid(y2), s3 = gn_sigmoid(y3);
      gt.x = gt.x * (s0 * (1.0f + y0 * (1.0f - s0)));
      gt.y = gt.y * (s1 * (1.0f + y1 * (1.0f - s1)));
      gt.z = gt.z * (s2 * (1.0f + y2 * (1.0f - s2)));
      gt.w = gt.w * (s3 * (1.0f + y3 * (1.0f - s3)));
    }
    return gt;
  };
  auto seg_accumulate = [&](int e, float4 dyv, float4 xh, bool valid) {
    float sg = valid ? (dyv.x * xh.x + dyv.y * xh.y) + (dyv.z * xh.z + dyv.w * xh.w) : 0.f;
    float sb = valid ? (dyv.x + dyv.y) + (dyv.z + dyv.w) : 0.f;
    sg = seg_sum(sg, r);
    sb = seg_sum(sb, r);
    if (valid && (threadIdx.x & (r - 1)) == 0) {
      seg_g[e / r] = sg;
      seg_b[e / r] = sb;
    }
  };
  const int nround = (nvec + 255) / 256;
  if (CACHED) {
#pragma unroll
    for (int i = 0; i < (CACHED ? ITEMS : 1); ++i) {
      const int e = threadIdx.x + i * 256;
      if (e < nvec) {
        xc[i] = xv[e];
        dc[i] = gv[e];
        const int c = g * cpg + e / hw4;
        gac[i] = gamma[c];
        bec[i] = beta[c];
      }
    }
#pragma unroll
    for (int i = 0; i < (CACHED ? ITEMS : 1); ++i) {
      if (i < nround) {
        const int e = threadIdx.x + i * 256;
        const bool valid = e < nvec;
        float4 xh = make_float4(0.f, 0.f, 0.f, 0.f);
        if (valid) dc[i] = dy_of(gac[i], bec[i], xc[i], dc[i], xh);
        seg_accumulate(valid ? e : 0, valid ? dc[i] : xh, xh, valid);
      }
    }
  } else {
    for (int i = 0; i < nround; ++i) {
      const int e = threadIdx.x + i * 256;
      const bool valid = e < nvec;
      float4 xh = make_float4(0.f, 0.f, 0.f, 0.f), d = xh;
      if (valid) {
        const int c = g * cpg + e / hw4;
        d = dy_of(gamma[c], beta[c], xv[e], gv[e], xh);
      }
      seg_accumulate(valid ? e : 0, d, xh, valid);
    }
  }
  __syncthreads();
  float my_g = 0.f, my_b = 0.f;
  if ((int)threadIdx.x < cpg) {
    for (int s = 0; s < segs_per_ch; ++s) {
      my_g += seg_g[threadIdx.x * segs_per_ch + s];
      my_b += seg_b[threadIdx.x * segs_per_ch + s];
    }
    const int c = g * cpg + threadIdx.x;
    part_dgamma[(size_t)n * C + c] = my_g;
    part_dbeta[(size_t)n * C + c] = my_b;
  }
  __syncthreads();
  if ((int)threadIdx.x < cpg) {
    const float ga = gamma[g * cpg + threadIdx.x];
    seg_g[threadIdx.x] = my_g * ga;
    seg_b[threadIdx.x] = my_b * ga;
  }
  __syncthreads();
  if (threadIdx.x == 0) {
    float a = 0.f, b = 0.f;
    for (int c = 0; c < cpg; ++c) { b += seg_g[c]; a += seg_b[c]; }
    grp[0] = a / (float)L;
    grp[1] = b / (float)L;
  }
  __syncthreads();
  const float ma = grp[0], mb = grp[1];
  float4 *ov = reinterpret_cast<float4 *>(dx + base);
  const float4 *av = reinterpret_cast<const float4 *>(EXTRA && addend ? addend + base : nullptr);
  auto emit = [&](int e, float ga, float4 xt, float4 dyv) {
    float4 o;
    o.x = rs * (dyv.x * ga - ma - ((xt.x - mu) * rs) * mb);
    o.y = rs * (dyv.y * ga - ma - ((xt.y - mu) * rs) * mb);
    o.z = rs * (dyv.z * ga - ma - ((xt.z - mu) * rs) * mb);
    o.w = rs * (dyv.w * ga - ma - ((xt.w - mu) * rs) * mb);
    if (EXTRA && av) {
      const float4 ad = av[e];
      o.x += ad.x; o.y += ad.y; o.z += ad.z; o.w += ad.w;
    }
    ov[e] = o;
    return o;
  };
  const bool want_nk = EXTRA && nk_sum != nullptr;
  auto nk_accumulate = [&](int e, float4 o, bool valid) {
    float sv = valid ? (o.x + o.y) + (o.z + o.w) : 0.f;
    sv = seg_sum(sv, r);
    if (valid && (threadIdx.x & (r - 1)) == 0) seg_g[e / r] = sv;
  };
  if (CACHED) {
#pragma unroll
    for (int i = 0; i < (CACHED ? ITEMS : 1); ++i) {
      const int e = threadIdx.x + i * 256;
      const bool valid = e < nvec;
      float4 o = make_float4(0.f, 0.f, 0.f, 0.f);
      if (valid) o = emit(e, gac[i], xc[i], dc[i]);
      if (EXTRA) {
        if (want_nk && i < nround) nk_accumulate(valid ? e : 0, o, valid);
      }
    }
  } else {
    for (int i = 0; i < nround; ++i) {
      const int e = threadIdx.x + i * 256;
      const bool valid = e < nvec;
      float4 o = make_float4(0.f, 0.f, 0.f, 0.f);
      if (valid) {
        float4 xh;
        const float4 xt = xv[e];
        const int c = g * cpg + e / hw4;
        const float ga = gamma[c];
        o = emit(e, ga, xt, dy_of(ga, beta[c], xt, gv[e], xh));
      }
      if (EXTRA) {
        if (want_nk) nk_accumulate(valid ? e : 0, o, valid);
      }
    }
  }
  if (EXTRA) {
    if (want_nk) {
      __syncthreads();
      if ((int)threadIdx.x < cpg) {
        float t = 0.f;
        for (int sgi = 0; sgi < segs_per_ch; ++sgi) t += seg_g[threadIdx.x * segs_per_ch + sgi];
        nk_sum[(size_t)n * C + g * cpg + threadIdx.x] = t;
      }
    }
  }
}

__global__ __launch_bounds__(256) void k_gn_bwd_final(const float *__restrict__ part_dgamma,
                                                      const float *__restrict__ part_dbeta, int N, int C,
                                                      float *__restrict__ dgamma, float *__restrict__ dbeta,
                                                      float *__restrict__ gacc, float *__restrict__ bacc,
                                                      const float *__restrict__ part_nk ,
                                                      float *__restrict__ csum ,
                                                      float *__restrict__ csum_acc ) {
  __shared__ double s_g[8][33], s_b[8][33], s_k[8][33];
  const int cx = threadIdx.x & 31, ry = threadIdx.x >> 5;
  const int c = blockIdx.x * 32 + cx;
  double sg = 0.0, sb = 0.0, sk = 0.0;
  if (c < C)
    for (int n = ry; n < N; n += 8) {
      sg += (double)part_dgamma[(size_t)n * C + c];
      sb += (double)part_dbeta[(size_t)n * C + c];
      if (part_nk) sk += (double)part_nk[(size_t)n * C + c];
    }
  s_g[ry][cx] = sg; s_b[ry][cx] = sb; s_k[ry][cx] = sk;
  __syncthreads();
  if (ry != 0 || c >= C) return;
  for (int q = 1; q < 8; ++q) { sg += s_g[q][cx]; sb += s_b[q][cx]; sk += s_k[q][cx]; }
  dgamma[c] = (float)sg;
  dbeta[c] = (float)sb;
  if (gacc) gacc[c] += (float)sg;
  if (bacc) bacc[c] += (float)sb;
  if (part_nk && csum) csum[c] = (float)sk;
  if (part_nk && csum_acc) csum_acc[c] += (float)sk;
}

inline int gn_items(int C, int HW, int G) {
  const int64_t nvec = (int64_t)(C / G) * HW / 4;
  for (int it = 1; it <= GN_ITEMS; it <<= 1)
    if (nvec <= (int64_t)it * 256) return it;
  return 0;
}

inline bool gn_shape_ok(int N, int C, int HW, int G) {
  if (N < 1 || C < 1 || G < 1 || C % G != 0 || HW < 4 || (HW & (HW - 1)) != 0) return false;
  const int cpg = C / G;
  if (cpg > 256) return false;
  const int hw4 = HW >> 2, r = hw4 < 64 ? hw4 : 64;
  return (int64_t)cpg * hw4 / r <= GN_MAX_SEG && (int64_t)cpg * HW < (1 << 30);
}

}

SALUN_EXPORT size_t salun_gn_workspace_bytes(int N, int C) {
  return sizeof(float) * 2 * (size_t)(N > 0 ? N : 0) * (size_t)(C > 0 ? C : 0);
}

SALUN_EXPORT int salun_gn_forward(const float *x, float *y, const float *gamma, const float *beta, float *save_mean,
                                  float *save_rstd, int N, int C, int HW, int G, double eps, int silu,
                                  salun_stream_t stream) {
  if (!x || !y || !gamma || !beta || !save_mean || !save_rstd || !gn_shape_ok(N, C, HW, G)) return SALUN_EINVAL;
  if (!salun_aligned16(x) || !salun_aligned16(y)) return SALUN_EINVAL;
  hipStream_t st = salun_hip_stream(stream);
  const int items = gn_items(C, HW, G);
#define SALUN_GN_FWD(S_, I_) \
  hipLaunchKernelGGL((k_gn_fwd<S_, I_>), dim3(N * G), dim3(256), 0, st, x, y, gamma, beta, save_mean, save_rstd, C, HW, G, (float)eps)
#define SALUN_GN_FWD_I(S_)                    \
  switch (items) {                            \
    case 1: SALUN_GN_FWD(S_, 1); break;       \
    case 2: SALUN_GN_FWD(S_, 2); break;       \
    case 4: SALUN_GN_FWD(S_, 4); break;       \
    case 8: SALUN_GN_FWD(S_, 8); break;       \
    case 16: SALUN_GN_FWD(S_, 16); break;     \
    default: SALUN_GN_FWD(S_, 0); break;      \
  }
  if (silu) { SALUN_GN_FWD_I(true) } else { SALUN_GN_FWD_I(false) }
#undef SALUN_GN_FWD_I
#undef SALUN_GN_FWD
  SALUN_LAUNCH_CHECK();
  return SALUN_OK;
}

SALUN_EXPORT int salun_gn_backward_fused(const float *dz, const float *x, const float *gamma, const float *beta,
                                         const float *save_mean, const float *save_rstd, const float *addend,
                                         float *dx, float *dgamma, float *dbeta, float *grad_gamma_acc,
                                         float *grad_beta_acc, float *nk_sum, float *csum, float *csum_acc, int N,
                                         int C, int HW, int G, int silu, void *ws, size_t ws_bytes,
                                         salun_stream_t stream) {
  if (!dz || !x || !gamma || !beta || !save_mean || !save_rstd || !dx || !dgamma || !dbeta || !gn_shape_ok(N, C, HW, G))
    return SALUN_EINVAL;
  if ((csum || csum_acc) && !nk_sum) return SALUN_EINVAL;
  if (addend == dx) return SALUN_EINVAL;
  if (!ws || ws_bytes < salun_gn_workspace_bytes(N, C)) return SALUN_ENOSPC;
  if (!salun_aligned16(dz) || !salun_aligned16(x) || !salun_aligned16(dx) || (addend && !salun_aligned16(addend)))
    return SALUN_EINVAL;
  hipStream_t st = salun_hip_stream(stream);
  float *pg = static_cast<float *>(ws), *pb = pg + (size_t)N * C;
  const int items = gn_items(C, HW, G);
  const bool extra = addend != nullptr || nk_sum != nullptr;
#define SALUN_GN_BWD(S_, I_, E_) \
  hipLaunchKernelGGL((k_gn_bwd<S_, I_, E_>), dim3(N * G), dim3(256), 0, st, dz, x, gamma, beta, save_mean, save_rstd, dx, pg, pb, C, HW, G, addend, nk_sum)
#define SALUN_GN_BWD_I(S_, E_)                    \
  switch (items) {                                \
    case 1: SALUN_GN_BWD(S_, 1, E_); break;       \
    case 2: SALUN_GN_BWD(S_, 2, E_); break;       \
    case 4: SALUN_GN_BWD(S_, 4, E_); break;       \
    case 8: SALUN_GN_BWD(S_, 8, E_); break;       \
    case 16: SALUN_GN_BWD(S_, 16, E_); break;     \
    default: SALUN_GN_BWD(S_, 0, E_); break;      \
  }
  if (silu) {
    if (extra) { SALUN_GN_BWD_I(true, true) } else { SALUN_GN_BWD_I(true, false) }
  } else {
    if (extra) { SALUN_GN_BWD_I(false, true) } else { SALUN_GN_BWD_I(false, false) }
  }
#undef SALUN_GN_BWD_I
#undef SALUN_GN_BWD
  SALUN_LAUNCH_CHECK();
  hipLaunchKernelGGL(k_gn_bwd_final, dim3((C + 31) / 32), dim3(256), 0, st, pg, pb, N, C, dgamma, dbeta,
                     grad_gamma_acc, grad_beta_acc, nk_sum, csum, csum_acc);
  SALUN_LAUNCH_CHECK();
  return SALUN_OK;
}

SALUN_EXPORT int salun_gn_backward(const float *dz, const float *x, const float *gamma, const float *beta,
                                   const float *save_mean, const float *save_rstd, float *dx, float *dgamma,
                                   float *dbeta, float *grad_gamma_acc, float *grad_beta_acc, int N, int C, int HW,
                                   int G, int silu, void *ws, size_t ws_bytes, salun_stream_t stream) {
  return salun_gn_backward_fused(dz, x, gamma, beta, save_mean, save_rstd, nullptr, dx, dgamma, dbeta, grad_gamma_acc,
                                 grad_beta_acc, nullptr, nullptr, nullptr, N, C, HW, G, silu, ws, ws_bytes, stream);
}
```

unlearn_saliency_amd/ops.py:

```python
from __future__ import annotations

import ctypes
from typing import Optional, Sequence

import torch

from .fastfn import FastFunction

from . import _lib, ringpack, weightimg
from ._lib import c_double, c_int, c_int64, c_size_t, c_uint64, c_void_p, check
from .streams import _stream, _stream_handle


def _dev(t: Optional[torch.Tensor], dtype: torch.dtype, name: str, allow_none: bool = False) -> c_void_p:
    if t is None:
        if allow_none:
            return c_void_p(None)
        raise ValueError(f"{name} must not be None")
    if not t.is_cuda:
        raise RuntimeError(f"{name}: the SalUn HIP kernels need a device tensor (got {t.device}); no CPU fallback")
    if t.dtype != dtype:
        raise TypeError(f"{name}: expected {dtype}, got {t.dtype}")
    if not t.is_contiguous():
        raise ValueError(f"{name} must be contiguous")
    return c_void_p(t.data_ptr())


_shape_memo: dict = {}


def _q(name: str, *args):
    key = (name,) + args
    v = _shape_memo.get(key)
    if v is None:
        fn = getattr(_lib.lib(), name)
        v = _shape_memo[key] = fn(*[c_int64(a) if t is c_int64 else a for a, t in zip(args, fn.argtypes)])
    return v


_ws: dict[tuple, torch.Tensor] = {}


def workspace(nbytes: int, device: torch.device, tag: str = "",
              stream: Optional[torch.cuda.Stream] = None) -> torch.Tensor:
    idx = device.index if device.index is not None else torch.cuda.current_device()
    key = (idx, None if tag == "topk" else _stream_handle(idx) if stream is None else stream.cuda_stream, tag)
    w = _ws.get(key)
    if w is None or w.numel() < nbytes:
        with torch.cuda.stream(stream):
            w = torch.empty(max(int(nbytes), 1 << 20), dtype=torch.uint8, device=device)
        _ws[key] = w
    return w


PARAM_EPOCH = weightimg.PARAM_EPOCH
PACK_CALLS = weightimg.BF16_LAUNCHES


def saliency_accumulate(acc: torch.Tensor, g: torch.Tensor, scale: float = 1.0,
                        sqnorm: Optional[torch.Tensor] = None, max_norm: float = 1.0) -> None:
    assert acc.numel() == g.numel()
    check(_lib.lib().salun_saliency_accumulate(_dev(acc, torch.float32, "acc"), _dev(g, torch.float32, "g"),
                                               c_double(scale), _dev(sqnorm, torch.float32, "sqnorm", True),
                                               c_double(max_norm), c_int64(acc.numel()), _stream()),
          "salun_saliency_accumulate")


class TopkFailed(RuntimeError):
    """The full-scan route's grid barrier timed out (its workgroups were not co-resident): the masks are garbage."""


def mask_topk(acc: torch.Tensor, ks: Sequence[int], out: Optional[Sequence[torch.Tensor]] = None,
              flags: int = 0, check: bool = False) -> list[torch.Tensor]:
    L = _lib.lib()
    n, nk = acc.numel(), len(ks)
    if not 1 <= nk <= _lib.SALUN_MAX_THRESHOLDS:
        raise ValueError(f"1 <= len(ks) <= {_lib.SALUN_MAX_THRESHOLDS}")
    values_only = bool(flags & _lib.SALUN_TOPK_VALUES_ONLY)
    if values_only:
        out, marr = [], None
    else:
        if out is None:
            n_pad = (n + 255) & ~255
            out = [r[:n] for r in torch.empty((nk, n_pad), dtype=torch.uint8, device=acc.device).unbind(0)]
        assert len(out) == nk and all(o.numel() == n for o in out)
        marr = (c_void_p * nk)(*[_dev(o, torch.uint8, "mask").value for o in out])
    nbytes = L.salun_mask_topk_workspace_bytes(c_int64(n), c_int(nk))
    ws = workspace(nbytes, acc.device, "topk")
    karr = (c_int64 * nk)(*[int(k) for k in ks])
    _lib.check(L.salun_mask_topk_ex(_dev(acc, torch.float32, "acc"), c_int64(n), karr, c_int(nk), marr,
                                    c_void_p(ws.data_ptr()), c_size_t(ws.numel()), ctypes.c_uint(flags), _stream()),
               "salun_mask_topk")
    if check:
        route, err = mask_topk_status(acc.device)
        from . import dist as sdist
        if sdist.collectives_on():
            flag = torch.tensor([int(err)], dtype=torch.int32, device=acc.device)
            torch.distributed.all_reduce(flag, op=torch.distributed.ReduceOp.MAX)
            err = int(flag.item())
        if err:
            raise TopkFailed(f"salun_mask_topk: the full scan's grid barrier timed out (route {route}, n = {n}): "
                             "its workgroups were not co-resident; no mask was produced")
    return list(out)


def mask_topk_status(device: torch.device) -> tuple[int, int]:
    ws = workspace(0, device, "topk")
    route, err = c_int(0), c_int(0)
    check(_lib.lib().salun_mask_topk_status(c_void_p(ws.data_ptr()), ctypes.byref(route), ctypes.byref(err), _stream()),
          "salun_mask_topk_status")
    return route.value, err.value


def mask_topk_thresholds(device: torch.device, nk: int) -> torch.Tensor:
    ws = workspace(0, device, "topk")
    out = torch.empty(nk, dtype=torch.float32, device=device)
    check(_lib.lib().salun_mask_topk_thresholds(c_void_p(ws.data_ptr()), c_int(nk), c_void_p(out.data_ptr()),
                                                _stream()), "salun_mask_topk_thresholds")
    return out


def mask_u8_to_i64(m: torch.Tensor) -> torch.Tensor:
    out = torch.empty(m.shape, dtype=torch.int64, device=m.device)
    check(_lib.lib().salun_mask_u8_to_i64(_dev(m, torch.uint8, "mask"), c_void_p(out.data_ptr()),
                                          c_int64(m.numel()), _stream()), "salun_mask_u8_to_i64")
    return out


def mask_i64_to_u8(m: torch.Tensor, out: Optional[torch.Tensor] = None) -> torch.Tensor:
    if out is None:
        out = torch.empty(m.shape, dtype=torch.uint8, device=m.device)
    check(_lib.lib().salun_mask_i64_to_u8(_dev(m, torch.int64, "mask"), _dev(out, torch.uint8, "out"),
                                          c_int64(m.numel()), _stream()), "salun_mask_i64_to_u8")
    return out


def mask_popcount(m: torch.Tensor) -> int:
    L = _lib.lib()
    ws = workspace(L.salun_reduce_workspace_bytes(c_int64(m.numel())), m.device)
    out = torch.empty(1, dtype=torch.int64, device=m.device)
    check(L.salun_mask_popcount(_dev(m, torch.uint8, "mask"), c_int64(m.numel()), c_void_p(out.data_ptr()),
                                c_void_p(ws.data_ptr()), c_size_t(ws.numel()), _stream()), "salun_mask_popcount")
    return int(out.item())


def masked_sgd_step(p: torch.Tensor, g: torch.Tensor, buf: Optional[torch.Tensor], m: Optional[torch.Tensor],
                    lr: float, momentum: float, weight_decay: float, first_step: bool) -> None:
    n = p.numel()
    assert g.numel() == n and (buf is None or buf.numel() == n) and (m is None or m.numel() == n)
    weightimg.params_written()
    check(_lib.lib().salun_masked_sgd_step(_dev(p, torch.float32, "p"), _dev(g, torch.float32, "g"),
                                           _dev(buf, torch.float32, "buf", True), _dev(m, torch.uint8, "mask", True),
                                           c_double(lr), c_double(momentum), c_double(weight_decay),
                                           c_int(int(first_step)), c_int64(n), _stream()), "salun_masked_sgd_step")


def grad_sqnorm(g: torch.Tensor, out: Optional[torch.Tensor] = None) -> torch.Tensor:
    L = _lib.lib()
    if out is None:
        out = torch.empty(1, dtype=torch.float32, device=g.device)
    ws = workspace(L.salun_reduce_workspace_bytes(c_int64(g.numel())), g.device)
    check(L.salun_grad_sqnorm(_dev(g, torch.float32, "g"), c_int64(g.numel()), _dev(out, torch.float32, "out"),
                              c_void_p(ws.data_ptr()), c_size_t(ws.numel()), _stream()), "salun_grad_sqnorm")
    return out


def masked_adam_step(p: torch.Tensor, g: torch.Tensor, m1: torch.Tensor, v: torch.Tensor,
                     mask: Optional[torch.Tensor], lr: float, beta1: float, beta2: float, eps: float,
                     weight_decay: float, step: int, sqnorm: Optional[torch.Tensor] = None,
                     max_norm: float = 1.0, gscale: float = 1.0) -> None:
    n = p.numel()
    assert g.numel() == n and m1.numel() == n and v.numel() == n and (mask is None or mask.numel() == n)
    weightimg.params_written()
    check(_lib.lib().salun_masked_adam_step(_dev(p, torch.float32, "p"), _dev(g, torch.float32, "g"),
                                            _dev(m1, torch.float32, "exp_avg"), _dev(v, torch.float32, "exp_avg_sq"),
                                            _dev(mask, torch.uint8, "mask", True),
                                            _dev(sqnorm, torch.float32, "sqnorm", True), c_double(max_norm),
                                            c_double(gscale), c_double(lr), c_double(beta1), c_double(beta2),
                                            c_double(eps), c_double(weight_decay), c_int(int(step)), c_int64(n),
                                            _stream()), "salun_masked_adam_step")


def adam_coefficients(step_dev: torch.Tensor, lr: float, beta1: float, beta2: float, coef: torch.Tensor) -> None:
    check(_lib.lib().salun_adam_coefficients(_dev(step_dev, torch.int64, "step"), c_double(lr), c_double(beta1),
                                             c_double(beta2), _dev(coef, torch.float32, "coef"), _stream()),
          "salun_adam_coefficients")


def masked_adam_step_coef(p, g, m1, v, mask, coef, beta1, beta2, eps, weight_decay, sqnorm=None, max_norm=1.0,
                          gscale=1.0) -> None:
    n = p.numel()
    weightimg.params_written()
    check(_lib.lib().salun_masked_adam_step_coef(_dev(p, torch.float32, "p"), _dev(g, torch.float32, "g"),
                                                 _dev(m1, torch.float32, "exp_avg"), _dev(v, torch.float32, "exp_avg_sq"),
                                                 _dev(mask, torch.uint8, "mask", True),
                                                 _dev(sqnorm, torch.float32, "sqnorm", True), c_double(max_norm),
                                                 c_double(gscale), _dev(coef, torch.float32, "coef"), c_double(beta1),
                                                 c_double(beta2), c_double(eps), c_double(weight_decay), c_int64(n),
                                                 _stream()), "salun_masked_adam_step_coef")


def adam_ema_step(p: torch.Tensor, g: torch.Tensor, m1: torch.Tensor, v: torch.Tensor, shadow: torch.Tensor,
                  mask: Optional[torch.Tensor], lr: float, beta1: float, beta2: float, eps: float, weight_decay: float,
                  mu: float, step: int, sqnorm: Optional[torch.Tensor] = None, max_norm: float = 1.0,
                  gscale: float = 1.0) -> None:
    n = p.numel()
    assert g.numel() == n and m1.numel() == n and v.numel() == n and shadow.numel() == n
    assert mask is None or mask.numel() == n
    weightimg.params_written()
    check(_lib.lib().salun_adam_ema_step(_dev(p, torch.float32, "p"), _dev(g, torch.float32, "g"),
                                         _dev(m1, torch.float32, "exp_avg"), _dev(v, torch.float32, "exp_avg_sq"),
                                         _dev(shadow, torch.float32, "shadow"), _dev(mask, torch.uint8, "mask", True),
                                         _dev(sqnorm, torch.float32, "sqnorm", True), c_double(max_norm),
                                         c_double(gscale), c_double(lr), c_double(beta1), c_double(beta2),
                                         c_double(eps), c_double(weight_decay), c_double(mu), c_int(int(step)),
                                         c_int64(n), _stream()), "salun_adam_ema_step")


def adam_ema_step_coef(p, g, m1, v, shadow, mask, coef, beta1, beta2, eps, weight_decay, mu, sqnorm=None, max_norm=1.0,
                       gscale=1.0) -> None:
    n = p.numel()
    assert g.numel() == n and m1.numel() == n and v.numel() == n and shadow.numel() == n
    assert mask is None or mask.numel() == n
    weightimg.params_written()
    check(_lib.lib().salun_adam_ema_step_coef(_dev(p, torch.float32, "p"), _dev(g, torch.float32, "g"),
                                              _dev(m1, torch.float32, "exp_avg"), _dev(v, torch.float32, "exp_avg_sq"),
                                              _dev(shadow, torch.float32, "shadow"),
                                              _dev(mask, torch.uint8, "mask", True),
                                              _dev(sqnorm, torch.float32, "sqnorm", True), c_double(max_norm),
                                              c_double(gscale), _dev(coef, torch.float32, "coef"), c_double(beta1),
                                              c_double(beta2), c_double(eps), c_double(weight_decay), c_double(mu),
                                              c_int64(n), _stream()), "salun_adam_ema_step_coef")


def qsample(x0: torch.Tensor, e: torch.Tensor, sqrt_ab: torch.Tensor, sqrt_1mab: torch.Tensor,
            t: torch.Tensor) -> torch.Tensor:
    B = x0.shape[0]
    chw = x0.numel() // max(B, 1)
    xt = torch.empty_like(x0)
    check(_lib.lib().salun_qsample(_dev(x0, torch.float32, "x0"), _dev(e, torch.float32, "e"),
                                   _dev(sqrt_ab, torch.float32, "sqrt_ab"), _dev(sqrt_1mab, torch.float32, "sqrt_1mab"),
                                   _dev(t, torch.int64, "t"), c_int64(sqrt_ab.numel()), c_void_p(xt.data_ptr()),
                                   c_int64(B), c_int64(chw), _stream()), "salun_qsample")
    return xt


def sqerr_loss(a: torch.Tensor, b: torch.Tensor, coef: float, want_per_sample: bool = False,
               want_grad: bool = True):
    L = _lib.lib()
    B = a.shape[0]
    chw = a.numel() // B
    loss = torch.empty(1, dtype=torch.float32, device=a.device)
    per = torch.empty(B, dtype=torch.float32, device=a.device) if want_per_sample else None
    d = torch.empty_like(b) if want_grad else None
    ws = workspace(L.salun_sqerr_workspace_bytes(c_int64(B), c_int64(chw)), a.device)
    check(L.salun_sqerr_loss(_dev(a, torch.float32, "a"), _dev(b, torch.float32, "b"), c_int64(B), c_int64(chw),
                             c_double(coef), c_void_p(loss.data_ptr()), _dev(per, torch.float32, "per_sample", True),
                             _dev(d, torch.float32, "dloss", True), c_void_p(ws.data_ptr()), c_size_t(ws.numel()),
                             _stream()), "salun_sqerr_loss")
    return loss, per, d


class _SqErr(FastFunction):

    @staticmethod
    def forward(ctx, target, pred, coef):
        loss, _, d = sqerr_loss(target.contiguous(), pred.contiguous(), coef, want_grad=True)
        ctx.save_for_backward(d)
        return loss.reshape(())

    @staticmethod
    def backward(ctx, grad_out):
        (d,) = ctx.saved_tensors
        return None, d * grad_out, None


def eps_mse(e: torch.Tensor, out: torch.Tensor) -> torch.Tensor:
    return _SqErr.apply(e, out, 1.0 / e.shape[0])


def mse_loss(target: torch.Tensor, pred: torch.Tensor) -> torch.Tensor:
    return _SqErr.apply(target, pred, 1.0 / target.numel())


def esd_loss_raw(e_n: torch.Tensor, e_0p: torch.Tensor, negative_guidance: float, want_grad: bool = True,
                 want_target: bool = False):
    L = _lib.lib()
    B = e_n.shape[0]
    if e_0p.shape[0] != 2 * B or e_0p.shape[1:] != e_n.shape[1:]:
        raise ValueError(f"e_0p {tuple(e_0p.shape)} is not the two-fold batch of e_n {tuple(e_n.shape)}")
    chw = e_n.numel() // B
    loss = torch.empty(1, dtype=torch.float32, device=e_n.device)
    d = torch.empty_like(e_n) if want_grad else None
    tgt = torch.empty_like(e_n) if want_target else None
    ws = workspace(L.salun_esd_loss_workspace_bytes(c_int64(B), c_int64(chw)), e_n.device)
    check(L.salun_esd_loss(_dev(e_n, torch.float32, "e_n"), _dev(e_0p, torch.float32, "e_0p"), c_int64(B), c_int64(chw),
                           c_double(negative_guidance), c_void_p(loss.data_ptr()), _dev(d, torch.float32, "d_e_n", True),
                           _dev(tgt, torch.float32, "target", True), c_void_p(ws.data_ptr()), c_size_t(ws.numel()),
                           _stream()), "salun_esd_loss")
    return loss, d, tgt


class _EsdLoss(FastFunction):

    @staticmethod
    def forward(ctx, e_n, e_0p, negative_guidance):
        loss, d, _ = esd_loss_raw(e_n.contiguous(), e_0p.contiguous(), negative_guidance)
        ctx.save_for_backward(d)
        return loss.reshape(())

    @staticmethod
    def backward(ctx, grad_out):
        (d,) = ctx.saved_tensors
        return d * grad_out, None, None


def esd_loss(e_n: torch.Tensor, e_0p: torch.Tensor, negative_guidance: float) -> torch.Tensor:
    return _EsdLoss.apply(e_n, e_0p, float(negative_guidance))


def dropout(x: torch.Tensor, p: float, key: int, sample_offset: int = 0, out: Optional[torch.Tensor] = None,
            seed_dev: Optional[torch.Tensor] = None) -> torch.Tensor:
    n = x.shape[0]
    chw = x.numel() // max(n, 1)
    y = out if out is not None else torch.empty_like(x)
    check(_lib.lib().salun_dropout(_dev(x, torch.float32, "x"), _dev(y, torch.float32, "y"), c_int64(n), c_int64(chw),
                                   c_int64(sample_offset), c_double(p), c_uint64(key & 0xFFFFFFFFFFFFFFFF),
                                   _dev(seed_dev, torch.int64, "seed_dev", True), _stream()), "salun_dropout")
    return y


class _Dropout(FastFunction):
    @staticmethod
    def forward(ctx, x, p, key, offset):
        ctx.cfg = (float(p), int(key), int(offset))
        return dropout(x.contiguous(), p, key, offset)

    @staticmethod
    def backward(ctx, dy):
        p, key, offset = ctx.cfg
        return dropout(dy.contiguous(), p, key, offset), None, None, None


def dropout_fn(x: torch.Tensor, p: float, key: int, sample_offset: int = 0) -> torch.Tensor:
    return _Dropout.apply(x, float(p), int(key), int(sample_offset))


def fim_square_accumulate(F: torch.Tensor, tmp: torch.Tensor, n_data: float) -> None:
    check(_lib.lib().salun_fim_square_accumulate(_dev(F, torch.float32, "F"), _dev(tmp, torch.float32, "tmp"),
                                                 c_double(n_data), c_int64(F.numel()), _stream()),
          "salun_fim_square_accumulate")


def _data_ws_bytes(N: int, outC: int, outH: int, outW: int, R: int, conv_stride: int) -> int:
    return _q("salun_conv2d_data_workspace_bytes", N, outC, outH, outW, R, conv_stride)


def conv2d_forward(x: torch.Tensor, w: torch.Tensor, bias: Optional[torch.Tensor], stride: int, pad: int,
                   P: int, Q: int, nbias: Optional[torch.Tensor] = None,
                   addend: Optional[torch.Tensor] = None) -> Optional[torch.Tensor]:
    N, C, H, W = x.shape
    K, _, R, _ = w.shape
    if nbias is not None and tuple(nbias.shape) != (N, K):
        raise ValueError(f"nbias must be [{N}, {K}], got {tuple(nbias.shape)}")
    if addend is not None and tuple(addend.shape) != (N, K, P, Q):
        raise ValueError(f"addend must be {(N, K, P, Q)}, got {tuple(addend.shape)}")
    if R == 3 and stride == 1 and pad == 1 and P == H and Q == W:
        imgs = ringpack.images(w)
        if imgs is not None:
            y = conv3x3_packed(x, imgs[0], K, bias=bias, nbias=nbias, addend=addend)
            if y is not None:
                return y
    y = torch.empty((N, K, P, Q), dtype=torch.float32, device=x.device)
    L = _lib.lib()
    wsb = _data_ws_bytes(N, K, P, Q, R, stride)
    ws = workspace(wsb, x.device) if wsb else None
    rc = L.salun_conv2d_forward_fused(_dev(x, torch.float32, "x"), _dev(w, torch.float32, "w"),
                                      _dev(bias, torch.float32, "bias", True),
                                      _dev(nbias, torch.float32, "nbias", True),
                                      _dev(addend, torch.float32, "addend", True), c_void_p(y.data_ptr()),
                                      N, C, H, W, K, R, stride, pad, P, Q,
                                      c_void_p(ws.data_ptr() if ws is not None else None), c_size_t(wsb), _stream())
    if rc == _lib.SALUN_EINVAL:
        return None
    check(rc, "salun_conv2d_forward_fused")
    return y


def conv2d_backward_data(dy: torch.Tensor, w: torch.Tensor, x_shape, stride: int, pad: int,
                         addend: Optional[torch.Tensor] = None) -> Optional[torch.Tensor]:
    N, C, H, W = x_shape
    K, _, R, _ = w.shape
    P, Q = dy.shape[2], dy.shape[3]
    if R == 3 and stride == 1 and pad == 1 and P == H and Q == W:
        imgs = ringpack.images(w)
        if imgs is not None:
            dx = conv3x3_packed(dy, imgs[1], C, addend=addend)
            if dx is not None:
                return dx
    dx = torch.empty((N, C, H, W), dtype=torch.float32, device=dy.device)
    L = _lib.lib()
    wsb = _data_ws_bytes(N, C, H, W, R, 1) if stride == 1 else 0
    ws = workspace(wsb, dy.device) if wsb else None
    rc = L.salun_conv2d_backward_data_ws(_dev(dy, torch.float32, "dy"), _dev(w, torch.float32, "w"),
                                         _dev(addend, torch.float32, "addend", True),
                                         c_void_p(dx.data_ptr()), N, C, H, W, K, R, stride, pad, P, Q,
                                         c_void_p(ws.data_ptr() if ws is not None else None), c_size_t(wsb), _stream())
    if rc == _lib.SALUN_EINVAL:
        return None
    check(rc, "salun_conv2d_backward_data")
    return dx


WGRAD_KERNEL = [None]


def conv2d_backward_weight(x: torch.Tensor, dy: torch.Tensor, w_shape, stride: int, pad: int,
                           out: Optional[torch.Tensor] = None, accumulate: bool = False,
                           shared: bool = False, stream: Optional[torch.cuda.Stream] = None) -> Optional[torch.Tensor]:
    N, C, H, W = x.shape
    K, _, R, _ = w_shape
    P, Q = dy.shape[2], dy.shape[3]
    L = _lib.lib()
    nbytes = L.salun_conv2d_wgrad_workspace_bytes(N, C, K, R, P, Q)
    if nbytes == 0:
        return None
    ws = workspace(nbytes, x.device, stream=stream)
    dw = out if out is not None else torch.empty(tuple(w_shape), dtype=torch.float32, device=x.device)
    rc = L.salun_conv2d_backward_weight_ex(_dev(x, torch.float32, "x"), _dev(dy, torch.float32, "dy"),
                                           _dev(dw, torch.float32, "dw"), N, C, H, W, K, R, stride, pad, P, Q,
                                           int(bool(accumulate and out is not None)),
                                           _lib.SALUN_WGRAD_SHARED if (shared if WGRAD_KERNEL[0] is None
                                                                       else WGRAD_KERNEL[0] == "shared") else 0,
                                           c_void_p(ws.data_ptr()), c_size_t(ws.numel()),
                                           c_void_p(_stream_handle() if stream is None else stream.cuda_stream))
    if rc == _lib.SALUN_EINVAL:
        return None
    check(rc, "salun_conv2d_backward_weight")
    return dw


def conv3x3_pack(w: torch.Tensor, dgrad: bool, out: Optional[torch.Tensor] = None) -> Optional[torch.Tensor]:
    K, C = w.shape[0], w.shape[1]
    L = _lib.lib()
    nbytes = int(L.salun_conv3x3_pack_bytes(K, C, int(dgrad)))
    if nbytes == 0 or tuple(w.shape[2:]) != (3, 3):
        return None
    img = out if out is not None and out.numel() * 4 == nbytes else torch.empty(nbytes // 4, dtype=torch.float32,
                                                                                device=w.device)
    _dev(w, torch.float32, "w")
    job = _lib.PackJob(w.data_ptr(), None if dgrad else img.data_ptr(), img.data_ptr() if dgrad else None, K, C)
    check(L.salun_conv3x3_pack_weights(ctypes.cast(ctypes.pointer(job), c_void_p), 1, _stream()),
          "salun_conv3x3_pack_weights")
    return img


def conv3x3_packed(x: torch.Tensor, img: torch.Tensor, Kout: int, bias: Optional[torch.Tensor] = None,
                   nbias: Optional[torch.Tensor] = None, addend: Optional[torch.Tensor] = None,
                   out: Optional[torch.Tensor] = None, cfg: int = 0) -> Optional[torch.Tensor]:
    N, Cred, H, W = x.shape
    y = out if out is not None else torch.empty((N, Kout, H, W), dtype=torch.float32, device=x.device)
    rc = _lib.lib().salun_conv3x3_packed(_dev(x, torch.float32, "x"), c_void_p(img.data_ptr()),
                                         _dev(bias, torch.float32, "bias", True),
                                         _dev(nbias, torch.float32, "nbias", True),
                                         _dev(addend, torch.float32, "addend", True), c_void_p(y.data_ptr()),
                                         N, Cred, H, W, Kout, int(cfg), _stream())
    if rc == _lib.SALUN_EINVAL:
        return None
    check(rc, "salun_conv3x3_packed")
    return y


def channel_sum(dy: torch.Tensor, out: Optional[torch.Tensor] = None, accumulate: bool = False) -> torch.Tensor:
    N, K = dy.shape[0], dy.shape[1]
    HW = dy.shape[2] * dy.shape[3]
    L = _lib.lib()
    ws = workspace(L.salun_channel_sum_workspace_bytes(N, K), dy.device)
    res = out if out is not None else torch.empty(K, dtype=torch.float32, device=dy.device)
    check(L.salun_channel_sum(_dev(dy, torch.float32, "dy"), _dev(res, torch.float32, "out"), N, K, HW,
                              int(bool(accumulate and out is not None)), c_void_p(ws.data_ptr()), c_size_t(ws.numel()),
                              _stream()), "salun_channel_sum")
    return res


def conv2d_bf16_supported(C: int, K: int, R: int, stride: int, pad: int) -> bool:
    return bool(_q("salun_conv2d_bf16_supported", C, K, R, stride, pad))


def conv2d_bf16_pack(w: torch.Tensor, out: Optional[torch.Tensor] = None) -> torch.Tensor:
    K, C, R, _ = w.shape
    if out is None:
        out = torch.empty((K, R * R, C), dtype=torch.bfloat16, device=w.device)
    check(_lib.lib().salun_conv2d_bf16_pack_weights(_dev(w, torch.float32, "w"), _dev(out, torch.bfloat16, "wp"), K, C, R,
                                                    _stream()), "salun_conv2d_bf16_pack_weights")
    return out


def bf16_pack_batch(jobs) -> int:
    jobs = list(jobs)
    if not jobs:
        return 0
    L, st, cap = _lib.lib(), _stream(), _lib.SALUN_BF16_PACK_MAX_JOBS
    launches = 0
    for i in range(0, len(jobs), cap):
        part = jobs[i:i + cap]
        arr = (_lib.Bf16PackJob * len(part))()
        for a, (w, wp, K, C, R, tr) in zip(arr, part):
            _dev(w, torch.float32, "w")
            _dev(wp, torch.bfloat16, "wp")
            a.w, a.wp, a.K, a.C, a.R, a.transposed = w.data_ptr(), wp.data_ptr(), K, C, R, int(bool(tr))
        check(L.salun_bf16_pack_weights_batch(ctypes.cast(arr, c_void_p), len(part), st), "salun_bf16_pack_weights_batch")
        launches += 1
    return launches


def conv2d_bf16_forward(x: torch.Tensor, wp: torch.Tensor, R: int, stride: int, pad: int,
                        bias: Optional[torch.Tensor] = None, nbias: Optional[torch.Tensor] = None,
                        addend: Optional[torch.Tensor] = None) -> torch.Tensor:
    N, H, W, C = x.shape
    K = wp.shape[0]
    OH, OW = (H + 2 * pad - R) // stride + 1, (W + 2 * pad - R) // stride + 1
    _dev(x, torch.bfloat16, "x")
    y = torch.empty((N, OH, OW, K), dtype=torch.bfloat16, device=x.device)
    ws = workspace(_q("salun_conv2d_bf16_data_workspace_bytes", N, H, W, C, K, R, stride, pad), x.device)
    check(_lib.lib().salun_conv2d_bf16_forward(_dev(x, torch.bfloat16, "x"), _dev(wp, torch.bfloat16, "wp"),
                                               _dev(bias, torch.float32, "bias", True),
                                               _dev(nbias, torch.float32, "nbias", True),
                                               _dev(addend, torch.bfloat16, "addend", True), c_void_p(y.data_ptr()),
                                               N, H, W, C, K, R, stride, pad, c_void_p(ws.data_ptr()),
                                               c_size_t(ws.numel()), _stream()), "salun_conv2d_bf16_forward")
    return y


def conv2d_bf16_backward_data(dy: torch.Tensor, wp: torch.Tensor, x_shape, R: int, stride: int, pad: int,
                              addend: Optional[torch.Tensor] = None) -> torch.Tensor:
    N, H, W, C = x_shape
    K = wp.shape[0]
    _dev(dy, torch.bfloat16, "dy")
    dx = torch.empty((N, H, W, C), dtype=torch.bfloat16, device=dy.device)
    ws = workspace(_q("salun_conv2d_bf16_data_workspace_bytes", N, H, W, C, K, R, stride, pad), dy.device)
    check(_lib.lib().salun_conv2d_bf16_backward_data(_dev(dy, torch.bfloat16, "dy"), _dev(wp, torch.bfloat16, "wp"),
                                                     _dev(addend, torch.bfloat16, "addend", True),
                                                     c_void_p(dx.data_ptr()), N, H, W, C, K, R, stride, pad,
                                                     c_void_p(ws.data_ptr()), c_size_t(ws.numel()), _stream()),
          "salun_conv2d_bf16_backward_data")
    return dx


def conv2d_bf16_backward_weight(x: torch.Tensor, dy: torch.Tensor, w_shape, stride: int, pad: int,
                                out: Optional[torch.Tensor] = None, accumulate: bool = False,
                                bias_out: Optional[torch.Tensor] = None,
                                nbias_out: Optional[torch.Tensor] = None,
                                stream: Optional[torch.cuda.Stream] = None) -> torch.Tensor:
    N, H, W, C = x.shape
    K, _, R, _ = w_shape
    L = _lib.lib()
    nbytes = _q("salun_conv2d_bf16_wgrad_workspace_bytes", N, H, W, C, K, R, stride, pad)
    if nbytes == 0:
        raise ValueError(f"bf16 backward-weight: unsupported shape C={C} K={K} R={R} stride={stride} pad={pad}")
    ws = workspace(nbytes, x.device, stream=stream)
    dw = out if out is not None else torch.empty(tuple(w_shape), dtype=torch.float32, device=x.device)
    if nbias_out is not None and tuple(nbias_out.shape) != (N, K):
        raise ValueError(f"nbias_out must be [{N}, {K}]")
    check(L.salun_conv2d_bf16_backward_weight_ex(_dev(x, torch.bfloat16, "x"), _dev(dy, torch.bfloat16, "dy"),
                                                 _dev(dw, torch.float32, "dw"), _dev(bias_out, torch.float32, "db", True),
                                                 _dev(nbias_out, torch.float32, "dnb", True),
                                                 N, H, W, C, K, R, stride, pad, int(bool(accumulate and out is not None)),
                                                 c_void_p(ws.data_ptr()), c_size_t(ws.numel()),
                                                 c_void_p(_stream_handle() if stream is None else stream.cuda_stream)),
          "salun_conv2d_bf16_backward_weight_ex")
    return dw


def colsum_bf16(dy: torch.Tensor, images: int, bias_out: Optional[torch.Tensor] = None,
                nbias_out: Optional[torch.Tensor] = None, accumulate: bool = False) -> None:
    K = dy.shape[-1]
    M = dy.numel() // K
    ws = workspace(_q("salun_colsum_bf16_workspace_bytes", K), dy.device)
    check(_lib.lib().salun_colsum_bf16(_dev(dy, torch.bfloat16, "dy"), _dev(bias_out, torch.float32, "db", True),
                                       _dev(nbias_out, torch.float32, "dnb", True), c_int64(M), K, int(images),
                                       int(bool(accumulate)), c_void_p(ws.data_ptr()), c_size_t(ws.numel()), _stream()),
          "salun_colsum_bf16")


def gemm_bf16_supported(M: int, N: int, K: int) -> bool:
    return bool(_q("salun_gemm_bf16_supported", int(M), int(N), int(K)))


def gemm_bf16_nt(x: torch.Tensor, w: torch.Tensor, bias: Optional[torch.Tensor] = None,
                 addend: Optional[torch.Tensor] = None, variant: int = 0) -> torch.Tensor:
    M, K = x.shape
    N = w.shape[0]
    assert w.shape[1] == K
    y = torch.empty((M, N), dtype=torch.bfloat16, device=x.device)
    check(_lib.lib().salun_gemm_bf16_nt(_dev(x, torch.bfloat16, "x"), _dev(w, torch.bfloat16, "w"),
                                        _dev(bias, torch.float32, "bias", True), _dev(addend, torch.bfloat16, "addend", True),
                                        c_void_p(y.data_ptr()), c_int64(M), N, K, int(variant), _stream()),
          "salun_gemm_bf16_nt")
    return y


def gemm_bf16_tn_supported(M: int, Na: int, Nb: int) -> bool:
    return bool(_lib.lib().salun_gemm_bf16_tn_supported(c_int64(M), int(Na), int(Nb)))


def gemm_bf16_tn(dy: torch.Tensor, x: torch.Tensor, out: Optional[torch.Tensor] = None, accumulate: bool = False,
                 variant: int = 0) -> torch.Tensor:
    M, Na = dy.shape
    Nb = x.shape[1]
    assert x.shape[0] == M
    L = _lib.lib()
    if not L.salun_gemm_bf16_tn_supported(c_int64(M), Na, Nb):
        raise ValueError(f"gemm_bf16_tn: unsupported shape M={M} Na={Na} Nb={Nb}")
    nbytes = L.salun_gemm_bf16_tn_workspace_bytes(c_int64(M), Na, Nb, int(variant))
    ws = workspace(nbytes, x.device) if nbytes else None
    dw = out if out is not None else torch.empty((Na, Nb), dtype=torch.float32, device=x.device)
    check(L.salun_gemm_bf16_tn(_dev(dy, torch.bfloat16, "dy"), _dev(x, torch.bfloat16, "x"), _dev(dw, torch.float32, "dw"),
                               c_int64(M), Na, Nb, int(bool(accumulate and out is not None)), int(variant),
                               c_void_p(ws.data_ptr() if ws is not None else None), c_size_t(nbytes), _stream()),
          "salun_gemm_bf16_tn")
    return dw


def pack_bf16(w: torch.Tensor, transposed: bool = False, out: Optional[torch.Tensor] = None) -> torch.Tensor:
    N, K = w.shape
    if out is None:
        out = torch.empty((K, N) if transposed else (N, K), dtype=torch.bfloat16, device=w.device)
    check(_lib.lib().salun_pack_bf16(_dev(w, torch.float32, "w"), _dev(out, torch.bfloat16, "wp"), N, K, int(bool(transposed)),
                                     _stream()), "salun_pack_bf16")
    return out


def gn_bf16_forward(x: torch.Tensor, gamma: torch.Tensor, beta: torch.Tensor, groups: int, eps: float, silu: bool):
    N, H, W, C = x.shape
    L = _lib.lib()
    ws = workspace(_q("salun_gn_bf16_workspace_bytes", N, C, H * W, groups), x.device)
    y = torch.empty_like(x)
    mr = torch.empty((N, groups, 2), dtype=torch.float32, device=x.device)
    ab = torch.empty((N, C, 2), dtype=torch.float32, device=x.device)
    check(L.salun_gn_bf16_forward(_dev(x, torch.bfloat16, "x"), _dev(gamma, torch.float32, "gamma"),
                                  _dev(beta, torch.float32, "beta"), c_void_p(y.data_ptr()), c_void_p(mr.data_ptr()),
                                  c_void_p(ab.data_ptr()), N, C, H * W, groups, c_double(eps), int(bool(silu)),
                                  c_void_p(ws.data_ptr()), c_size_t(ws.numel()), _stream()), "salun_gn_bf16_forward")
    return y, mr, ab


def gn_bf16_backward(dy: torch.Tensor, x: torch.Tensor, gamma: torch.Tensor, mr: torch.Tensor, ab: torch.Tensor,
                     groups: int, silu: bool, dgamma: torch.Tensor, dbeta: torch.Tensor, accumulate: bool) -> torch.Tensor:
    N, H, W, C = x.shape
    L = _lib.lib()
    ws = workspace(_q("salun_gn_bf16_workspace_bytes", N, C, H * W, groups), x.device)
    dx = torch.empty_like(x)
    check(L.salun_gn_bf16_backward(_dev(dy, torch.bfloat16, "dy"), _dev(x, torch.bfloat16, "x"),
                                   _dev(gamma, torch.float32, "gamma"), _dev(mr, torch.float32, "mr"),
                                   _dev(ab, torch.float32, "ab"), c_void_p(dx.data_ptr()),
                                   _dev(dgamma, torch.float32, "dgamma"), _dev(dbeta, torch.float32, "dbeta"), N, C, H * W,
                                   groups, int(bool(silu)), int(bool(accumulate)), c_void_p(ws.data_ptr()),
                                   c_size_t(ws.numel()), _stream()), "salun_gn_bf16_backward")
    return dx


def attn_supported(D: int) -> bool:
    return bool(_q("salun_attn_supported", int(D)))


def _tok_view(t: torch.Tensor, name: str):
    if not t.is_cuda or t.dtype != torch.bfloat16 or t.dim() != 4:
        raise TypeError(f"{name}: expected a 4-D bfloat16 device tensor [B, tokens, H, D]")
    B, N, H, D = t.shape
    if t.stride(3) != 1 or (H > 1 and t.stride(2) != D):
        raise ValueError(f"{name}: heads must be adjacent runs of D contiguous channels")
    return c_void_p(t.data_ptr()), ctypes.c_longlong(t.stride(0) if B > 1 else N * t.stride(1)), c_int(t.stride(1))


def attn_forward(q: torch.Tensor, k: torch.Tensor, v: torch.Tensor, scale: float, need_lse: bool = True):
    B, Nq, H, D = q.shape
    Nk = k.shape[1]
    o = torch.empty((B, Nq, H, D), dtype=torch.bfloat16, device=q.device)
    lse = torch.empty((B * H, Nq), dtype=torch.float32, device=q.device) if need_lse else None
    qp, qb, ql = _tok_view(q, "q")
    kp, kb, kl = _tok_view(k, "k")
    vp, vb, vl = _tok_view(v, "v")
    op, ob, ol = _tok_view(o, "o")
    check(_lib.lib().salun_attn_forward(qp, kp, vp, op, c_void_p(lse.data_ptr() if need_lse else None), B, H, Nq, Nk, D,
                                        qb, ql, kb, kl, vb, vl, ob, ol, c_double(scale), _stream()), "salun_attn_forward")
    return o, lse


def attn_backward(q, k, v, o, d_o, lse, scale: float):
    B, Nq, H, D = q.shape
    Nk = k.shape[1]
    dq = torch.empty((B, Nq, H, D), dtype=torch.bfloat16, device=q.device)
    dk = torch.empty((B, Nk, H, D), dtype=torch.bfloat16, device=q.device)
    dv = torch.empty((B, Nk, H, D), dtype=torch.bfloat16, device=q.device)
    dsum = torch.empty((B * H, Nq), dtype=torch.float32, device=q.device)
    qp, qb, ql = _tok_view(q, "q")
    kp, kb, kl = _tok_view(k, "k")
    vp, vb, vl = _tok_view(v, "v")
    op, ob, ol = _tok_view(o, "o")
    dp, db, dl = _tok_view(d_o, "d_o")
    check(_lib.lib().salun_attn_backward(qp, kp, vp, op, dp, _dev(lse, torch.float32, "lse"), c_void_p(dq.data_ptr()),
                                         c_void_p(dk.data_ptr()), c_void_p(dv.data_ptr()), c_void_p(dsum.data_ptr()),
                                         B, H, Nq, Nk, D, qb, ql, kb, kl, vb, vl, ob, ol, db, dl, c_double(scale), _stream()),
          "salun_attn_backward")
    return dq, dk, dv


class _Attn(FastFunction):
    @staticmethod
    def forward(ctx, q, k, v, scale):
        o, lse = attn_forward(q, k, v, scale, need_lse=True)
        ctx.save_for_backward(q, k, v, o, lse)
        ctx.scale = float(scale)
        return o

    @staticmethod
    def backward(ctx, d_o):
        q, k, v, o, lse = ctx.saved_tensors
        if d_o.stride(3) != 1 or d_o.stride(2) != d_o.shape[3]:
            d_o = d_o.contiguous()
        dq, dk, dv = attn_backward(q, k, v, o, d_o.to(torch.bfloat16), lse, ctx.scale)
        return dq, dk, dv, None


def attention(q: torch.Tensor, k: torch.Tensor, v: torch.Tensor, scale: float) -> torch.Tensor:
    return _Attn.apply(q, k, v, float(scale))


class _LayerNorm16(FastFunction):

    @staticmethod
    def forward(ctx, x, weight, bias, eps):
        C = x.shape[-1]
        xc = x.contiguous()
        rows = xc.numel() // C
        y = torch.empty_like(xc)
        stats = torch.empty((rows, 2), dtype=torch.float32, device=x.device)
        check(_lib.lib().salun_ln_bf16_forward(_dev(xc, torch.bfloat16, "x"), _dev(weight, torch.float32, "gamma"),
                                               _dev(bias, torch.float32, "beta"), c_void_p(y.data_ptr()),
                                               c_void_p(stats.data_ptr()), c_int64(rows), C, c_double(eps), _stream()),
              "salun_ln_bf16_forward")
        ctx.save_for_backward(xc, stats)
        ctx.params = (weight, bias)
        return y

    @staticmethod
    def backward(ctx, dy):
        from . import gradsink
        xc, stats = ctx.saved_tensors
        weight, bias = ctx.params
        C = xc.shape[-1]
        rows = xc.numel() // C
        dyc = dy.to(torch.bfloat16).contiguous()
        L = _lib.lib()
        ws = workspace(_q("salun_ln_bf16_workspace_bytes", rows, C), xc.device)
        dg, db = gradsink.pair(weight, bias, torch.empty)
        dx = torch.empty_like(xc)
        check(L.salun_ln_bf16_backward(_dev(dyc, torch.bfloat16, "dy"), _dev(xc, torch.bfloat16, "x"),
                                       _dev(weight, torch.float32, "gamma"), _dev(stats, torch.float32, "stats"),
                                       c_void_p(dx.data_ptr()), _dev(dg.out, torch.float32, "dgamma"),
                                       _dev(db.out, torch.float32, "dbeta"), c_int64(rows), C, int(dg.accumulate),
                                       c_void_p(ws.data_ptr()), c_size_t(ws.numel()), _stream()), "salun_ln_bf16_backward")
        return dx, dg.returned(), db.returned(), None


def layer_norm_bf16(x: torch.Tensor, ln: "torch.nn.LayerNorm") -> torch.Tensor:
    return _LayerNorm16.apply(x, ln.weight, ln.bias, float(ln.eps))


class _Geglu16(FastFunction):

    @staticmethod
    def forward(ctx, h):
        hc = h.contiguous()
        F2 = hc.shape[-1]
        rows = hc.numel() // F2
        out = torch.empty(hc.shape[:-1] + (F2 // 2,), dtype=torch.bfloat16, device=h.device)
        check(_lib.lib().salun_geglu_bf16_forward(_dev(hc, torch.bfloat16, "h"), c_void_p(out.data_ptr()), c_int64(rows),
                                                  F2 // 2, _stream()), "salun_geglu_bf16_forward")
        ctx.save_for_backward(hc)
        return out

    @staticmethod
    def backward(ctx, dy):
        (hc,) = ctx.saved_tensors
        F2 = hc.shape[-1]
        rows = hc.numel() // F2
        dyc = dy.to(torch.bfloat16).contiguous()
        dh = torch.empty_like(hc)
        check(_lib.lib().salun_geglu_bf16_backward(_dev(hc, torch.bfloat16, "h"), _dev(dyc, torch.bfloat16, "dy"),
                                                   c_void_p(dh.data_ptr()), c_int64(rows), F2 // 2, _stream()),
              "salun_geglu_bf16_backward")
        return dh


def geglu_bf16(h: torch.Tensor) -> torch.Tensor:
    return _Geglu16.apply(h)


def bn_forward(x, res, gamma, beta, running_mean, running_var, training, momentum, eps, relu,
               num_batches_tracked=None):
    N, C, H, W = x.shape
    L = _lib.lib()
    y = torch.empty_like(x)
    mean = torch.empty(C, dtype=torch.float32, device=x.device)
    invstd = torch.empty(C, dtype=torch.float32, device=x.device)
    ws = workspace(L.salun_bn_workspace_bytes(C), x.device)
    rc = L.salun_bn_forward(_dev(x, torch.float32, "x"), _dev(res, torch.float32, "res", True), c_void_p(y.data_ptr()),
                            _dev(gamma, torch.float32, "weight"), _dev(beta, torch.float32, "bias"),
                            _dev(running_mean, torch.float32, "running_mean", True),
                            _dev(running_var, torch.float32, "running_var", True),
                            _dev(num_batches_tracked, torch.int64, "num_batches_tracked", True),
                            c_void_p(mean.data_ptr()),
                            c_void_p(invstd.data_ptr()), N, C, H * W, int(bool(training)), c_double(momentum),
                            c_double(eps), int(bool(relu)), c_void_p(ws.data_ptr()), c_size_t(ws.numel()), _stream())
    if rc == _lib.SALUN_EINVAL:
        return None
    check(rc, "salun_bn_forward")
    return y, mean, invstd


def bn_backward(dy, y, x, gamma, mean, invstd, training, relu, want_dres, gamma_grad_acc=None, beta_grad_acc=None):
    N, C, H, W = x.shape
    L = _lib.lib()
    dx = torch.empty_like(x)
    dres = torch.empty_like(x) if want_dres else None
    dgamma = torch.empty(C, dtype=torch.float32, device=x.device)
    dbeta = torch.empty(C, dtype=torch.float32, device=x.device)
    ws = workspace(L.salun_bn_workspace_bytes(C), x.device)
    check(L.salun_bn_backward(_dev(dy, torch.float32, "dy"), _dev(y, torch.float32, "y", True),
                              _dev(x, torch.float32, "x"), _dev(gamma, torch.float32, "weight"),
                              _dev(mean, torch.float32, "mean"), _dev(invstd, torch.float32, "invstd"),
                              c_void_p(dx.data_ptr()), _dev(dres, torch.float32, "dres", True),
                              c_void_p(dgamma.data_ptr()), c_void_p(dbeta.data_ptr()),
                              _dev(gamma_grad_acc, torch.float32, "gamma.grad", True),
                              _dev(beta_grad_acc, torch.float32, "beta.grad", True), N, C, H * W,
                              int(bool(training)), int(bool(relu)), c_void_p(ws.data_ptr()), c_size_t(ws.numel()),
                              _stream()), "salun_bn_backward")
    return dx, dres, dgamma, dbeta


def gn_forward(x, gamma, beta, groups, eps, silu):
    N, C, H, W = x.shape
    z = torch.empty_like(x)
    mean = torch.empty(N * groups, dtype=torch.float32, device=x.device)
    rstd = torch.empty(N * groups, dtype=torch.float32, device=x.device)
    rc = _lib.lib().salun_gn_forward(_dev(x, torch.float32, "x"), c_void_p(z.data_ptr()),
                                     _dev(gamma, torch.float32, "weight"), _dev(beta, torch.float32, "bias"),
                                     c_void_p(mean.data_ptr()), c_void_p(rstd.data_ptr()), N, C, H * W, int(groups),
                                     c_double(eps), int(bool(silu)), _stream())
    if rc == _lib.SALUN_EINVAL:
        return None
    check(rc, "salun_gn_forward")
    return z, mean, rstd


def gn_backward(dz, x, gamma, beta, mean, rstd, groups, silu, gamma_grad_acc=None, beta_grad_acc=None, addend=None,
                nk_sum: bool = False, csum: bool = False, csum_acc=None):
    N, C, H, W = x.shape
    L = _lib.lib()
    dx = torch.empty_like(x)
    dgamma = torch.empty(C, dtype=torch.float32, device=x.device)
    dbeta = torch.empty(C, dtype=torch.float32, device=x.device)
    ws = workspace(L.salun_gn_workspace_bytes(N, C), x.device)
    if addend is not None and addend.shape != x.shape:
        raise ValueError("gn_backward: addend must have the shape of x")
    want_nk = bool(nk_sum or csum or csum_acc is not None)
    nk = torch.empty((N, C), dtype=torch.float32, device=x.device) if want_nk else None
    cs = torch.empty(C, dtype=torch.float32, device=x.device) if csum else None
    check(L.salun_gn_backward_fused(_dev(dz, torch.float32, "dz"), _dev(x, torch.float32, "x"),
                                    _dev(gamma, torch.float32, "weight"), _dev(beta, torch.float32, "bias"),
                                    _dev(mean, torch.float32, "mean"), _dev(rstd, torch.float32, "rstd"),
                                    _dev(addend, torch.float32, "addend", True),
                                    c_void_p(dx.data_ptr()), c_void_p(dgamma.data_ptr()), c_void_p(dbeta.data_ptr()),
                                    _dev(gamma_grad_acc, torch.float32, "weight.grad", True),
                                    _dev(beta_grad_acc, torch.float32, "bias.grad", True),
                                    _dev(nk, torch.float32, "nk_sum", True), _dev(cs, torch.float32, "csum", True),
                                    _dev(csum_acc, torch.float32, "csum_acc", True), N, C, H * W, int(groups),
                                    int(bool(silu)), c_void_p(ws.data_ptr()), c_size_t(ws.numel()), _stream()),
          "salun_gn_backward_fused")
    if want_nk:
        return dx, dgamma, dbeta, nk, cs
    return dx, dgamma, dbeta


def proximal_step(p: torch.Tensor, p0: torch.Tensor, ratio: int, scratch: Optional[torch.Tensor] = None,
                  scratch_mask: Optional[torch.Tensor] = None) -> torch.Tensor:
    weightimg.params_written()
    n = p.numel()
    if ratio < 1:
        raise IndexError("index -1 is out of bounds for dimension 0 with size 0")
    if ratio > n:
        raise RuntimeError("selected index k out of range")
    L = _lib.lib()
    d = scratch if scratch is not None else torch.empty(n, dtype=torch.float32, device=p.device)
    check(L.salun_param_diff(_dev(p, torch.float32, "p"), _dev(p0, torch.float32, "p0"), _dev(d, torch.float32, "d"),
                             c_int64(n), _stream()), "salun_param_diff")
    mask_topk(d, [n - ratio + 1], flags=_lib.SALUN_TOPK_VALUES_ONLY)
    tau = mask_topk_thresholds(p.device, 1)
    check(L.salun_soft_threshold_step(_dev(p, torch.float32, "p"), _dev(p0, torch.float32, "p0"),
                                      c_void_p(tau.data_ptr()), c_int64(n), _stream()), "salun_soft_threshold_step")
    return tau


def ewc_penalty_grad(p: torch.Tensor, p_star: torch.Tensor, F: torch.Tensor, g: torch.Tensor, lam: float
                     ) -> torch.Tensor:
    n = p.numel()
    L = _lib.lib()
    out = torch.empty(2, dtype=torch.float32, device=p.device)
    ws = workspace(L.salun_ewc_workspace_bytes(c_int64(n)), p.device)
    check(L.salun_ewc_penalty_grad(_dev(p, torch.float32, "p"), _dev(p_star, torch.float32, "p_star"),
                                   _dev(F, torch.float32, "F"), _dev(g, torch.float32, "g"), c_double(lam),
                                   c_void_p(out.data_ptr()), c_int64(n), c_void_p(ws.data_ptr()),
                                   c_size_t(ws.numel()), _stream()), "salun_ewc_penalty_grad")
    return out


def image_batch(data: torch.Tensor, idx: torch.Tensor, crop: Optional[torch.Tensor] = None,
                flip: Optional[torch.Tensor] = None, pad: int = 4, out: Optional[torch.Tensor] = None) -> torch.Tensor:
    num, H, W, C = data.shape
    B = idx.numel()
    if out is None:
        out = torch.empty((B, C, H, W), dtype=torch.float32, device=data.device)
    check(_lib.lib().salun_image_batch(_dev(data, torch.uint8, "data"), _dev(idx, torch.int64, "idx"),
                                       _dev(crop, torch.int32, "crop", True), _dev(flip, torch.uint8, "flip", True),
                                       c_void_p(out.data_ptr()), c_int64(B), c_int(H), c_int(W), c_int(C), c_int(pad),
                                       _stream()), "salun_image_batch")
    return out


def fill_uniform(n: int, seed: int, lo: float = 0.0, hi: float = 1.0, device="cuda") -> torch.Tensor:
    out = torch.empty(n, dtype=torch.float32, device=device)
    check(_lib.lib().salun_fill_uniform(c_void_p(out.data_ptr()), c_int64(n), c_uint64(seed), c_double(lo),
                                        c_double(hi), _stream()), "salun_fill_uniform")
    return out


def fill_normal(n: int, seed: int, mean: float = 0.0, std: float = 1.0, device="cuda") -> torch.Tensor:
    out = torch.empty(n, dtype=torch.float32, device=device)
    check(_lib.lib().salun_fill_normal(c_void_p(out.data_ptr()), c_int64(n), c_uint64(seed), c_double(mean),
                                       c_double(std), _stream()), "salun_fill_normal")
    return out


def fill_u8(n: int, seed: int, device="cuda") -> torch.Tensor:
    out = torch.empty(n, dtype=torch.uint8, device=device)
    check(_lib.lib().salun_fill_u8(c_void_p(out.data_ptr()), c_int64(n), c_uint64(seed), _stream()), "salun_fill_u8")
    return out


def prune_amount(amount: float, alive: int) -> int:
    if not 0.0 <= float(amount) <= 1.0:
        raise ValueError(f"amount should be a float in the range [0, 1], got {amount}")
    return int(round(float(amount) * int(alive)))


def prune_global(p: torch.Tensor, buf: Optional[torch.Tensor], keep: torch.Tensor, segs: torch.Tensor, n_sel: int,
                 alive: int, k_prune: int, rnd: Optional[torch.Tensor] = None, flags: int = 0,
                 check: bool = True) -> None:
    L = _lib.lib()
    n, nseg = p.numel(), segs.shape[0]
    assert keep.numel() == n and (buf is None or buf.numel() == n) and segs.dim() == 2 and segs.shape[1] == 2
    assert rnd is None or rnd.numel() == n_sel
    if k_prune == 0:
        return
    weightimg.params_written()
    ws = workspace(L.salun_prune_workspace_bytes(c_int64(n_sel)), p.device, "prune")
    _lib.check(L.salun_prune_global(_dev(p, torch.float32, "p"), _dev(buf, torch.float32, "buf", True),
                                    _dev(keep, torch.uint8, "keep"), c_int64(n), _dev(segs, torch.int64, "segs"),
                                    c_int(nseg), c_int64(n_sel), c_int64(alive), c_int64(k_prune),
                                    _dev(rnd, torch.float32, "rnd", True), ctypes.c_uint(flags),
                                    c_void_p(ws.data_ptr()), c_size_t(ws.numel()), _stream()), "salun_prune_global")
    if check:
        route, err = prune_status(p.device, n_sel, ranked=0 < k_prune < alive)
        if err & 2:
            raise TopkFailed("salun_prune_global: the kernels refused the segment table (not ascending and disjoint, "
                             "outside [0, n), or not n_sel elements in all); nothing was changed")
        if err:
            raise TopkFailed(f"salun_prune_global: the select's grid barrier timed out (route {route}); the round's "
                             "result is invalid")


def prune_status(device: torch.device, n_sel: int, ranked: bool = True) -> tuple[int, int]:
    L = _lib.lib()
    ws = workspace(L.salun_prune_workspace_bytes(c_int64(n_sel)), device, "prune")
    route, err = c_int(0), c_int(0)
    check(L.salun_prune_status(c_void_p(ws.data_ptr()), c_int64(n_sel), c_int(int(ranked)), ctypes.byref(route),
                               ctypes.byref(err), _stream()), "salun_prune_status")
    return route.value, err.value


def prune_count_zeros(p: torch.Tensor, segs: torch.Tensor, n_sel: int) -> torch.Tensor:
    out = torch.empty(1, dtype=torch.int64, device=p.device)
    check(_lib.lib().salun_prune_count_zeros(_dev(p, torch.float32, "p"), c_int64(p.numel()),
                                             _dev(segs, torch.int64, "segs"), c_int(segs.shape[0]), c_int64(n_sel),
                                             c_void_p(out.data_ptr()), _stream()), "salun_prune_count_zeros")
    return out


def maxpool2x2_forward(x: torch.Tensor):
    N, C, H, W = x.shape
    y = torch.empty((N, C, H // 2, W // 2), dtype=torch.float32, device=x.device)
    idx = torch.empty((N, C, H // 2, W // 2), dtype=torch.uint8, device=x.device)
    check(_lib.lib().salun_maxpool2x2_forward(_dev(x, torch.float32, "x"), c_void_p(y.data_ptr()),
                                              c_void_p(idx.data_ptr()), c_int64(N * C), H, W, _stream()),
          "salun_maxpool2x2_forward")
    return y, idx


def maxpool2x2_backward(dy: torch.Tensor, idx: torch.Tensor) -> torch.Tensor:
    N, C, P, Q = dy.shape
    dx = torch.empty((N, C, 2 * P, 2 * Q), dtype=torch.float32, device=dy.device)
    check(_lib.lib().salun_maxpool2x2_backward(_dev(dy, torch.float32, "dy"), _dev(idx, torch.uint8, "idx"),
                                               c_void_p(dx.data_ptr()), c_int64(N * C), 2 * P, 2 * Q, _stream()),
          "salun_maxpool2x2_backward")
    return dx
```

unlearn_saliency_amd/resblock.py:

```python
from __future__ import annotations

import torch

from .fastfn import FastFunction
import torch.nn as nn

import os

from . import draws, gradsink, ops, wgrad_side

FWD_SHORTCUT_BESIDE = os.environ.get("SALUN_FWD_SHORTCUT_BESIDE", "1") != "0"


def _bn_args(bn: nn.BatchNorm2d):
    return bn.running_mean, bn.running_var, bn.training, bn.momentum, bn.eps


class _BasicBlockFn(FastFunction):
    @staticmethod
    def forward(ctx, x, blk, w1, g1, b1, w2, g2, b2, wd, gd, bd):
        s = blk.conv1.stride[0]
        N, C, H, W = x.shape
        P, Q = (H + 2 - 3) // s + 1, (W + 2 - 3) // s + 1
        training = blk.bn1.training
        cd = md = idd = None
        fork = None
        if wd is not None:
            def shortcut():
                cd_ = ops.conv2d_forward(x, wd, None, s, 0, P, Q)
                return (cd_,) + tuple(ops.bn_forward(cd_, None, gd, bd, *_bn_args(blk.downsample[1]), False,
                                                     blk.downsample[1].num_batches_tracked))
            if (FWD_SHORTCUT_BESIDE and wgrad_side.OVERLAP and x.is_cuda
                    and not torch.cuda.is_current_stream_capturing()):
                main, fork = torch.cuda.current_stream(x.device), wgrad_side.stream(x.device)
                fork.wait_stream(main)
                with torch.cuda.stream(fork):
                    cd, skip, md, idd = shortcut()
                x.record_stream(fork)
        c1 = ops.conv2d_forward(x, w1, None, s, 1, P, Q)
        y1, m1, i1 = ops.bn_forward(c1, None, g1, b1, *_bn_args(blk.bn1), True, blk.bn1.num_batches_tracked)
        c2 = ops.conv2d_forward(y1, w2, None, 1, 1, P, Q)
        if wd is None:
            skip = x
        elif fork is None:
            cd, skip, md, idd = shortcut()
        else:
            main.wait_stream(fork)
            for t in (cd, skip, md, idd):
                if t is not None:
                    t.record_stream(main)
        out, m2, i2 = ops.bn_forward(c2, skip, g2, b2, *_bn_args(blk.bn2), True, blk.bn2.num_batches_tracked)
        ctx.save_for_backward(x, c1, y1, c2, out, cd, w1, g1, b1, w2, g2, b2, wd, gd, bd, m1, i1, m2, i2, md, idd)
        ctx.cfg = (s, training)
        return out

    @staticmethod
    def backward(ctx, dout):
        x, c1, y1, c2, out, cd, w1, g1, b1, w2, g2, b2, wd, gd, bd, m1, i1, m2, i2, md, idd = ctx.saved_tensors
        s, training = ctx.cfg
        dout = dout.contiguous()
        grads = {}

        def bn_bwd(dy, y, xin, g, b, m, i, relu, want_dres):
            to_g, to_b = gradsink.pair(g, b)
            dx, dres, dg, db = ops.bn_backward(dy, y, xin, g, m, i, training, relu, want_dres, to_g.out, to_b.out)
            return dx, dres, to_g.returned(dg), to_b.returned(db)

        wgrad = wgrad_side.ConvWgrad(dout.device)

        dc2, dskip, dg2, db2 = bn_bwd(dout, out, c2, g2, b2, m2, i2, True, True)
        dwd = dgd = dbd = None
        dxd = dskip
        if wd is not None:
            dcd, _, dgd, dbd = bn_bwd(dskip, None, cd, gd, bd, md, idd, False, False)
            dwd = wgrad(x, dcd, wd, s, 0)
            dxd = ops.conv2d_backward_data(dcd, wd, x.shape, s, 0) if ctx.needs_input_grad[0] else None
        dw2 = wgrad(y1, dc2, w2, 1, 1)
        dy1 = ops.conv2d_backward_data(dc2, w2, y1.shape, 1, 1)
        dc1, _, dg1, db1 = bn_bwd(dy1, y1, c1, g1, b1, m1, i1, True, False)
        dw1 = wgrad(x, dc1, w1, s, 1)
        dx = ops.conv2d_backward_data(dc1, w1, x.shape, s, 1, addend=dxd) if ctx.needs_input_grad[0] else None
        wgrad.finish()
        return dx, None, dw1, dg1, db1, dw2, dg2, db2, dwd, dgd, dbd


def _probe(blk, shape, device) -> bool:
    N, C, H, W = shape
    s = blk.conv1.stride[0]
    P, Q = (H + 2 - 3) // s + 1, (W + 2 - 3) // s + 1
    K = blk.conv1.out_channels
    if (P * Q) % 4 or (H * W) % 4:
        return False
    e = lambda *sh: torch.empty(sh, dtype=torch.float32, device=device)
    x, y1, dy = e(N, C, H, W), e(N, K, P, Q), e(N, K, P, Q)
    convs = [(x, blk.conv1.weight, s, 1), (y1, blk.conv2.weight, 1, 1)]
    if blk.downsample is not None:
        convs.append((x, blk.downsample[0].weight, s, 0))
    for xin, w, st, pad in convs:
        if ops.conv2d_forward(xin, w, None, st, pad, P, Q) is None:
            return False
        if ops.conv2d_backward_data(dy, w, xin.shape, st, pad, addend=xin) is None:
            return False
        if ops.conv2d_backward_weight(xin, dy, w.shape, st, pad) is None:
            return False
    return True


def _structure_ok(blk) -> bool:
    convs = [blk.conv1, blk.conv2] + ([blk.downsample[0]] if blk.downsample is not None else [])
    bns = [blk.bn1, blk.bn2] + ([blk.downsample[1]] if blk.downsample is not None else [])
    if any(type(b) is not nn.BatchNorm2d or not b.affine or not b.track_running_stats or b.momentum is None
           for b in bns):
        return False
    if any(c.bias is not None or c.groups != 1 or c.dilation != (1, 1) or c.weight.dtype != torch.float32
           for c in convs):
        return False
    if len({b.training for b in bns}) != 1:
        return False
    c1, c2 = blk.conv1, blk.conv2
    ok = (c1.kernel_size == (3, 3) and c1.padding == (1, 1) and c1.stride[0] == c1.stride[1] and c1.stride[0] in (1, 2)
          and c2.kernel_size == (3, 3) and c2.padding == (1, 1) and c2.stride == (1, 1))
    if blk.downsample is not None:
        d = blk.downsample[0]
        ok = ok and d.kernel_size == (1, 1) and d.padding == (0, 0) and d.stride == c1.stride
    else:
        ok = ok and c1.stride == (1, 1) and c1.in_channels == c1.out_channels
    return ok


def _admitted(blk, x: torch.Tensor, structure_ok, probe) -> bool:
    cache = blk.__dict__.setdefault("_fused_shapes", {})
    key = (tuple(x.shape), x.device)
    ok = cache.get(key)
    if ok is None:
        with torch.no_grad():
            ok = cache[key] = structure_ok(blk) and probe(blk, tuple(x.shape), x.device)
    return ok and structure_ok(blk)


def fused_basic_block(blk, x: torch.Tensor):
    if not (x.is_cuda and x.dtype == torch.float32 and x.dim() == 4) or torch.is_autocast_enabled():
        return None
    if not _admitted(blk, x, _structure_ok, _probe):
        return None
    x = x.contiguous()
    d = blk.downsample
    return _BasicBlockFn.apply(x, blk, blk.conv1.weight, blk.bn1.weight, blk.bn1.bias, blk.conv2.weight,
                               blk.bn2.weight, blk.bn2.bias, d[0].weight if d is not None else None,
                               d[1].weight if d is not None else None, d[1].bias if d is not None else None)


class _DiffusionResnetBlockFn(FastFunction):
    @staticmethod
    def forward(ctx, x, proj, blk, n1w, n1b, w1, b1, n2w, n2b, w2, b2, ws, bs):
        N, C, H, W = x.shape
        G1, G2 = blk.norm1.num_groups, blk.norm2.num_groups
        a1, m1, r1 = ops.gn_forward(x, n1w, n1b, G1, blk.norm1.eps, True)
        c1 = ops.conv2d_forward(a1, w1, b1, 1, 1, H, W, nbias=proj)
        a2, m2, r2 = ops.gn_forward(c1, n2w, n2b, G2, blk.norm2.eps, True)
        p = float(blk.dropout.p) if blk.dropout.training else 0.0
        dkey = None
        if p > 0.0:
            dkey = draws.dropout_key()
            a2 = ops.dropout(a2, p, dkey[0], dkey[1], out=a2)
        if ws is not None:
            sc = ops.conv2d_forward(x, ws, bs, 1, (ws.shape[2] - 1) // 2, H, W)
        else:
            sc = x
        out = ops.conv2d_forward(a2, w2, b2, 1, 1, H, W, addend=sc)
        ctx.save_for_backward(x, a1, c1, a2, n1w, n1b, w1, b1, n2w, n2b, w2, b2, ws, bs, m1, r1, m2, r2)
        ctx.cfg = (G1, G2, p, dkey)
        return out

    @staticmethod
    def backward(ctx, dout):
        x, a1, c1, a2, n1w, n1b, w1, b1, n2w, n2b, w2, b2, ws, bs, m1, r1, m2, r2 = ctx.saved_tensors
        G1, G2, p, dkey = ctx.cfg
        dout = dout.contiguous()
        wgrad = wgrad_side.ConvWgrad(dout.device)
        dbs = None
        to_b2 = gradsink.dest(b2)
        if bs is None:
            db2 = to_b2.returned(ops.channel_sum(dout, out=to_b2.out, accumulate=to_b2.accumulate))
        else:
            csum = ops.channel_sum(dout)
            db2, dbs = to_b2.add(csum), gradsink.dest(bs).add(csum)
            if dbs is db2 is csum:
                dbs = csum.clone()
        dw2 = wgrad(a2, dout, w2, 1, 1)
        da2 = ops.conv2d_backward_data(dout, w2, a2.shape, 1, 1)
        if dkey is not None:
            da2 = ops.dropout(da2, p, dkey[0], dkey[1], out=da2)
        to_g, to_b = gradsink.pair(n2w, n2b)
        to_b1 = gradsink.dest(b1)
        dc1, dg2, dbt2, nk, cs = ops.gn_backward(da2, c1, n2w, n2b, m2, r2, G2, True, to_g.out, to_b.out, nk_sum=True,
                                                 csum=not to_b1.accumulate, csum_acc=to_b1.out)
        dg2, dbt2, db1 = to_g.returned(dg2), to_b.returned(dbt2), to_b1.returned(cs)
        dproj = nk if ctx.needs_input_grad[1] else None
        dw1 = wgrad(a1, dc1, w1, 1, 1)
        da1 = ops.conv2d_backward_data(dc1, w1, a1.shape, 1, 1)
        to_g, to_b = gradsink.pair(n1w, n1b)
        dws = None
        if ws is None:
            dx, dg1, dbt1 = ops.gn_backward(da1, x, n1w, n1b, m1, r1, G1, True, to_g.out, to_b.out, addend=dout)
        else:
            pad = (ws.shape[2] - 1) // 2
            dws = wgrad(x, dout, ws, 1, pad)
            dxg, dg1, dbt1 = ops.gn_backward(da1, x, n1w, n1b, m1, r1, G1, True, to_g.out, to_b.out)
            dx = ops.conv2d_backward_data(dout, ws, x.shape, 1, pad, addend=dxg)
        dg1, dbt1 = to_g.returned(dg1), to_b.returned(dbt1)
        wgrad.finish()
        if not ctx.needs_input_grad[0]:
            dx = None
        return dx, dproj, None, dg1, dbt1, dw1, db1, dg2, dbt2, dw2, db2, dws, dbs


def _diffusion_block_structure_ok(blk) -> bool:
    convs = [blk.conv1, blk.conv2]
    skip = getattr(blk, "conv_shortcut", None) if blk.use_conv_shortcut else getattr(blk, "nin_shortcut", None)
    if blk.in_channels != blk.out_channels:
        if skip is None:
            return False
        convs.append(skip)
    if any(type(n) is not nn.GroupNorm or not n.affine or n.weight.dtype != torch.float32
           for n in (blk.norm1, blk.norm2)):
        return False
    for c in convs:
        if (c.bias is None or c.groups != 1 or c.dilation != (1, 1) or c.stride != (1, 1)
                or c.padding_mode != "zeros" or c.weight.dtype != torch.float32):
            return False
    ok = all(c.kernel_size == (3, 3) and c.padding == (1, 1) for c in (blk.conv1, blk.conv2))
    if len(convs) == 3:
        k = convs[2].kernel_size
        ok = ok and k in ((1, 1), (3, 3)) and convs[2].padding == ((k[0] - 1) // 2,) * 2
    return ok and type(blk.dropout) is draws.CounterDropout and 0.0 <= blk.dropout.p < 1.0 and not blk.dropout.inplace


def _diffusion_block_probe(blk, shape, device) -> bool:
    N, C, H, W = shape
    K = blk.out_channels
    hw = H * W
    if hw < 4 or hw & (hw - 1) or C // blk.norm1.num_groups > 256 or K // blk.norm2.num_groups > 256:
        return False
    e = lambda *sh: torch.empty(sh, dtype=torch.float32, device=device)
    x, h, proj = e(N, C, H, W), e(N, K, H, W), e(N, K)
    try:
        for t, n in ((x, blk.norm1), (h, blk.norm2)):
            z, m, r = ops.gn_forward(t, n.weight, n.bias, n.num_groups, n.eps, True)
            ops.gn_backward(z, t, n.weight, n.bias, m, r, n.num_groups, True, addend=t, nk_sum=True)
    except Exception:
        return False
    convs = [(x, blk.conv1), (h, blk.conv2)]
    if C != K:
        convs.append((x, blk.conv_shortcut if blk.use_conv_shortcut else blk.nin_shortcut))
    for xin, c in convs:
        pad = c.padding[0]
        if ops.conv2d_forward(xin, c.weight, c.bias, 1, pad, H, W, nbias=proj, addend=h) is None:
            return False
        if ops.conv2d_backward_data(h, c.weight, xin.shape, 1, pad, addend=xin) is None:
            return False
        if ops.conv2d_backward_weight(xin, h, c.weight.shape, 1, pad) is None:
            return False
    return True


def fused_diffusion_resnet_block(blk, x: torch.Tensor, emb_act: torch.Tensor, proj: torch.Tensor = None):
    from . import norm
    if not (x.is_cuda and x.dtype == torch.float32 and x.dim() == 4) or torch.is_autocast_enabled() or not norm._FUSED_GN:
        return None
    if not _admitted(blk, x, _diffusion_block_structure_ok, _diffusion_block_probe):
        return None
    if proj is None:
        proj = blk.temb_cemb_proj(emb_act)
    if proj.dtype != torch.float32 or tuple(proj.shape) != (x.shape[0], blk.out_channels):
        return None
    skip = None
    if blk.in_channels != blk.out_channels:
        skip = blk.conv_shortcut if blk.use_conv_shortcut else blk.nin_shortcut
    return _DiffusionResnetBlockFn.apply(x.contiguous(), proj.contiguous(), blk, blk.norm1.weight, blk.norm1.bias,
                                         blk.conv1.weight, blk.conv1.bias, blk.norm2.weight, blk.norm2.bias,
                                         blk.conv2.weight, blk.conv2.bias,
                                         skip.weight if skip is not None else None,
                                         skip.bias if skip is not None else None)
```

Baseline: 118.2.

## Fuse BatchNorm statistics reduction into 3x3 ring conv epilogue

Adds a statistics variant of the ring 3x3 conv kernel that reduces per-channel sum and sum-of-squares in registers via cross-lane shuffles, then writes per-workgroup double partials. A new BN forward path consumes those partials, so BN no longer re-reads the conv output to compute its statistics. Stride-1 convs in fused ResNet basic blocks use this path by default during training. Costs: extra register pressure and shuffles in the conv kernel, a grid trimmed to a multiple of the k-tile count, and the path only applies to configs with WK*KT==2.

After: 118.9 (median of 5 runs). No clear change (+0.6%).

```diff
diff --git a/include/salun.h b/include/salun.h
--- a/include/salun.h
+++ b/include/salun.h
@@ -142,6 +142,10 @@
 int salun_conv3x3_packed(const float *x , const float *img , const float *bias ,
                          const float *nbias , const float *addend , float *y ,
                          int N, int Cred, int H, int W, int Kout, int cfg, salun_stream_t stream);
+size_t salun_conv3x3_stats_bytes(int N, int Cred, int H, int W, int Kout, int cfg);
+int salun_conv3x3_packed_stats(const float *x , const float *img , float *y ,
+                               double *partials , size_t partials_bytes, int N, int Cred, int H, int W, int Kout,
+                               int cfg, salun_stream_t stream);
 
 int salun_conv2d_bf16_supported(int C, int K, int R, int stride, int pad);
 int salun_conv2d_bf16_pack_weights(const float *w , uint16_t *wp , int K, int C, int R,
@@ -219,6 +223,12 @@
                      float *save_mean , float *save_invstd ,
                      int N, int C, int HW, int training, double momentum, double eps, int relu, void *ws ,
                      size_t ws_bytes, salun_stream_t stream);
+int salun_bn_forward_from_partials(const float *x , const float *res , float *y ,
+                                   const float *gamma , const float *beta ,
+                                   float *running_mean , float *running_var ,
+                                   long long *num_batches_tracked , float *save_mean ,
+                                   float *save_invstd , int N, int C, int HW, double momentum, double eps,
+                                   int relu, const double *partials , int nslots, salun_stream_t stream);
 int salun_bn_backward(const float *dy , const float *y , const float *x ,
                       const float *gamma , const float *save_mean , const float *save_invstd ,
                       float *dx , float *dres , float *dgamma , float *dbeta ,
diff --git a/unlearn_saliency_amd/_lib.py b/unlearn_saliency_amd/_lib.py
--- a/unlearn_saliency_amd/_lib.py
+++ b/unlearn_saliency_amd/_lib.py
@@ -104,6 +104,8 @@
     "salun_conv3x3_pack_bytes": (c_size_t, [c_int] * 3),
     "salun_conv3x3_pack_weights": (c_int, [c_void_p, c_int, c_void_p]),
     "salun_conv3x3_packed": (c_int, [c_void_p] * 6 + [c_int] * 6 + [c_void_p]),
+    "salun_conv3x3_stats_bytes": (c_size_t, [c_int] * 6),
+    "salun_conv3x3_packed_stats": (c_int, [c_void_p] * 4 + [c_size_t] + [c_int] * 6 + [c_void_p]),
     "salun_conv2d_backward_weight": (c_int, [c_void_p, c_void_p, c_void_p] + [c_int] * 11 + [c_void_p, c_size_t,
                                                                                           c_void_p]),
     "salun_conv2d_backward_weight_ex": (c_int, [c_void_p, c_void_p, c_void_p] + [c_int] * 11 + [ctypes.c_uint, c_void_p,
@@ -136,6 +138,8 @@
     "salun_geglu_bf16_backward": (c_int, [c_void_p, c_void_p, c_void_p, c_int64, c_int, c_void_p]),
     "salun_bn_workspace_bytes": (c_size_t, [c_int]),
     "salun_bn_forward": (c_int, [c_void_p] * 10 + [c_int] * 4 + [c_double, c_double, c_int, c_void_p, c_size_t, c_void_p]),
+    "salun_bn_forward_from_partials": (c_int, [c_void_p] * 10 + [c_int] * 3 + [c_double, c_double, c_int, c_void_p, c_int,
+                                                                             c_void_p]),
     "salun_bn_backward": (c_int, [c_void_p] * 12 + [c_int] * 5 + [c_void_p, c_size_t, c_void_p]),
     "salun_conv2d_backward_data_add": (c_int, [c_void_p] * 4 + [c_int] * 10 + [c_void_p]),
     "salun_gn_workspace_bytes": (c_size_t, [c_int, c_int]),
diff --git a/unlearn_saliency_amd/csrc/salun_conv_ring.hip b/unlearn_saliency_amd/csrc/salun_conv_ring.hip
--- a/unlearn_saliency_amd/csrc/salun_conv_ring.hip
+++ b/unlearn_saliency_amd/csrc/salun_conv_ring.hip
@@ -70,8 +70,29 @@
   int nchunk;
 };
 
-template <int LOGW, int PT, int KT, int WP, int WK, bool EPI>
-__global__ __launch_bounds__(256, 2) void conv3x3_ring(const RingArgs g) {
+struct RingStatsArgs {
+  RingArgs g;
+  double *part;
+  int nslots;
+};
+__device__ __forceinline__ const RingArgs &ring_args(const RingArgs &a) { return a; }
+__device__ __forceinline__ const RingArgs &ring_args(const RingStatsArgs &a) { return a.g; }
+
+template <int HALF>
+__device__ __forceinline__ void ring_scatter_step(float (&q)[32], int lo) {
+  const bool up = (lo & HALF) != 0;
+#pragma unroll
+  for (int j = 0; j < HALF; ++j) {
+    const float keep = up ? q[j + HALF] : q[j];
+    const float send = up ? q[j] : q[j + HALF];
+    q[j] = keep + __shfl_xor(send, HALF, 64);
+  }
+}
+
+template <int LOGW, int PT, int KT, int WP, int WK, bool EPI, bool STATS = false>
+__global__ __launch_bounds__(256, 2) void conv3x3_ring(const std::conditional_t<STATS, RingStatsArgs, RingArgs> ga) {
+  const RingArgs &g = ring_args(ga);
+  static_assert(!(STATS && EPI), "the statistics variant is built without epilogue terms: the stored value is the accumulator");
   constexpr int W = 1 << LOGW, W4 = W / 4;
   constexpr int KTW = WK * KT, KB = KTW * 32;
   constexpr int A_BYTES = KTW * RGROUPS * 1024;
@@ -155,6 +176,11 @@
     if (it_chunk == nchunk) { it_chunk = 0; it_tile += gridDim.x; if (it_tile < total) setup_issue(it_tile); }
   }
   int stage = 0;
+  [[maybe_unused]] double run[KT];
+  if constexpr (STATS) {
+#pragma unroll
+    for (int t = 0; t < KT; ++t) run[t] = 0.0;
+  }
 
   for (int tile = blockIdx.x; tile < total; tile += gridDim.x) {
     const int kb = tile % g.ntile_k, ptile = tile / g.ntile_k;
@@ -288,6 +314,47 @@
           }
         }
       }
+    }
+    if constexpr (STATS) {
+#pragma unroll
+      for (int t = 0; t < KT; ++t) {
+        float q[32];
+#pragma unroll
+        for (int v = 0; v < 16; ++v) {
+          float s1 = 0.f, s2 = 0.f;
+#pragma unroll
+          for (int pt = 0; pt < PT; ++pt) {
+            const float o = (n_l[pt] < N) ? acc[pt][t][v] : 0.f;
+            if (pt == 0) { s1 = o; s2 = o * o; }
+            else { s1 += o; s2 += o * o; }
+          }
+          q[v] = s1;
+          q[16 + v] = s2;
+        }
+        ring_scatter_step<16>(q, lo);
+        ring_scatter_step<8>(q, lo);
+        ring_scatter_step<4>(q, lo);
+        ring_scatter_step<2>(q, lo);
+        ring_scatter_step<1>(q, lo);
+        run[t] += (double)q[0];
+      }
+    }
+  }
+  if constexpr (STATS) {
+    __syncthreads();
+    double *sd = reinterpret_cast<double *>(lds);
+#pragma unroll
+    for (int t = 0; t < KT; ++t) sd[(wave * KT + t) * 64 + lane] = run[t];
+    __syncthreads();
+    if (tid < WK * KT * 64) {
+      const int wk_o = tid / (KT * 64), t_o = (tid >> 6) % KT, ln = tid & 63;
+      double sum = 0.0;
+#pragma unroll
+      for (int w = 0; w < WP; ++w) sum += sd[((wk_o * WP + w) * KT + t_o) * 64 + ln];
+      const int l = ln & 31, which = l >> 4, v = l & 15;
+      const int kb = blockIdx.x % g.ntile_k, slot = blockIdx.x / g.ntile_k;
+      const int ch = kb * KB + (wk_o * KT + t_o) * 32 + (v & 3) + 8 * (v >> 2) + 4 * (ln >> 5);
+      if (ch < g.Kout) ga.part[((size_t)ch * ga.nslots + slot) * 2 + which] = sum;
     }
   }
 }
@@ -519,8 +586,15 @@
   return -1;
 }
 
+struct RingStats {
+  double *part;
+  size_t bytes;
+  bool query;
+  int nslots;
+};
+
 template <int LOGW, int PT, int KT, int WP, int WK>
-int ring_launch(RingArgs a, int W, bool epi, int wgs_per_cu, hipStream_t st) {
+int ring_launch(RingArgs a, int W, bool epi, int wgs_per_cu, hipStream_t st, RingStats *rs) {
   constexpr int TPIX = WP * PT * 32, KB = WK * KT * 32;
   const int HW = a.H * W;
   if (TPIX % W != 0) return SALUN_EINVAL;
@@ -547,6 +621,27 @@
   if (ldsb > 80 * 1024) return SALUN_EINVAL;
   int grid = wgs_per_cu * ring_cu_count();
   if (grid > a.ntiles) grid = a.ntiles;
+  if (rs) {
+    rs->nslots = 0;
+    if constexpr (WK * KT == 2) {
+      const int sgrid = grid - grid % a.ntile_k;
+      if (!epi && sgrid > 0) {
+        const int nslots = sgrid / a.ntile_k;
+        if (rs->query) {
+          rs->nslots = nslots;
+          return SALUN_OK;
+        }
+        if (!rs->part || rs->bytes < sizeof(double) * 2 * (size_t)a.Kout * nslots) return SALUN_ENOSPC;
+        const RingStatsArgs sa{a, rs->part, nslots};
+        ring_allow_lds(reinterpret_cast<const void *>(conv3x3_ring<LOGW, PT, KT, WP, WK, false, true>));
+        hipLaunchKernelGGL((conv3x3_ring<LOGW, PT, KT, WP, WK, false, true>), dim3(sgrid), dim3(256), ldsb, st, sa);
+        SALUN_LAUNCH_CHECK();
+        rs->nslots = nslots;
+        return SALUN_OK;
+      }
+    }
+    if (rs->query) return SALUN_OK;
+  }
   if (epi) {
     ring_allow_lds(reinterpret_cast<const void *>(conv3x3_ring<LOGW, PT, KT, WP, WK, true>));
     hipLaunchKernelGGL((conv3x3_ring<LOGW, PT, KT, WP, WK, true>), dim3(grid), dim3(256), ldsb, st, a);
@@ -559,14 +654,25 @@
 }
 
 template <int LOGW>
-int ring_dispatch(const RingArgs &a, int cfg, bool epi, int wgs_per_cu, hipStream_t st) {
+int ring_dispatch(const RingArgs &a, int cfg, bool epi, int wgs_per_cu, hipStream_t st, RingStats *rs = nullptr) {
   constexpr int W = 1 << LOGW;
   switch (ring_choose(cfg, a.N, a.H, W, a.Kout)) {
-    case 1: return ring_launch<LOGW, 2, 2, 4, 1>(a, W, epi, wgs_per_cu, st);
-    case 2: return ring_launch<LOGW, 1, 2, 4, 1>(a, W, epi, wgs_per_cu, st);
-    case 3: return ring_launch<LOGW, 1, 1, 2, 2>(a, W, epi, wgs_per_cu, st);
-    case 4: return ring_launch<LOGW, 1, 4, 4, 1>(a, W, epi, wgs_per_cu, st);
-    case 5: return ring_launch<LOGW, 1, 2, 2, 2>(a, W, epi, wgs_per_cu, st);
+    case 1: return ring_launch<LOGW, 2, 2, 4, 1>(a, W, epi, wgs_per_cu, st, rs);
+    case 2: return ring_launch<LOGW, 1, 2, 4, 1>(a, W, epi, wgs_per_cu, st, rs);
+    case 3: return ring_launch<LOGW, 1, 1, 2, 2>(a, W, epi, wgs_per_cu, st, rs);
+    case 4: return ring_launch<LOGW, 1, 4, 4, 1>(a, W, epi, wgs_per_cu, st, rs);
+    case 5: return ring_launch<LOGW, 1, 2, 2, 2>(a, W, epi, wgs_per_cu, st, rs);
+    default: return SALUN_EINVAL;
+  }
+}
+
+int ring_dispatch_w(const RingArgs &a, int W, int cfg, bool epi, hipStream_t st, RingStats *rs = nullptr) {
+  const int wgs = (cfg >> 8) ? (cfg >> 8) : 2;
+  switch (W) {
+    case 4: return ring_dispatch<2>(a, cfg & 255, epi, wgs, st, rs);
+    case 8: return ring_dispatch<3>(a, cfg & 255, epi, wgs, st, rs);
+    case 16: return ring_dispatch<4>(a, cfg & 255, epi, wgs, st, rs);
+    case 32: return ring_dispatch<5>(a, cfg & 255, epi, wgs, st, rs);
     default: return SALUN_EINVAL;
   }
 }
@@ -649,13 +755,31 @@
   if (!a.zero) return SALUN_EIO;
   a.N = N; a.Cred = Cred; a.H = H; a.Kout = Kout;
   const bool epi = bias || nbias || addend;
-  const int wgs = (cfg >> 8) ? (cfg >> 8) : 2;
-  hipStream_t st = salun_hip_stream(stream);
-  switch (W) {
-    case 4: return ring_dispatch<2>(a, cfg & 255, epi, wgs, st);
-    case 8: return ring_dispatch<3>(a, cfg & 255, epi, wgs, st);
-    case 16: return ring_dispatch<4>(a, cfg & 255, epi, wgs, st);
-    case 32: return ring_dispatch<5>(a, cfg & 255, epi, wgs, st);
-    default: return SALUN_EINVAL;
-  }
-}
+  return ring_dispatch_w(a, W, cfg, epi, salun_hip_stream(stream));
+}
+
+SALUN_EXPORT size_t salun_conv3x3_stats_bytes(int N, int Cred, int H, int W, int Kout, int cfg) {
+  if (N <= 0 || Cred <= 0 || Kout <= 0 || H <= 0 || Cred % RCC != 0) return 0;
+  RingArgs a{};
+  a.N = N; a.Cred = Cred; a.H = H; a.Kout = Kout;
+  RingStats rs{nullptr, 0, true, 0};
+  if (ring_dispatch_w(a, W, cfg, false, nullptr, &rs) != SALUN_OK) return 0;
+  return sizeof(double) * 2 * (size_t)Kout * rs.nslots;
+}
+
+SALUN_EXPORT int salun_conv3x3_packed_stats(const float *x, const float *img, float *y, double *partials,
+                                            size_t partials_bytes, int N, int Cred, int H, int W, int Kout, int cfg,
+                                            salun_stream_t stream) {
+  if (!x || !img || !y || N <= 0 || Cred <= 0 || Kout <= 0 || H <= 0) return SALUN_EINVAL;
+  if (Cred % RCC != 0 || !salun_aligned16(x) || !salun_aligned16(img)) return SALUN_EINVAL;
+  if ((long long)N * Cred * H * W >= (1ll << 31) || (long long)N * Kout * H * W >= (1ll << 31)) return SALUN_EINVAL;
+  if (partials && (reinterpret_cast<uintptr_t>(partials) & 7u)) return SALUN_EINVAL;
+  RingArgs a{};
+  a.x = x; a.aimg = img; a.y = y;
+  a.zero = ring_zero_page();
+  if (!a.zero) return SALUN_EIO;
+  a.N = N; a.Cred = Cred; a.H = H; a.Kout = Kout;
+  RingStats rs{partials, partials_bytes, false, 0};
+  const int rc = ring_dispatch_w(a, W, cfg, false, salun_hip_stream(stream), &rs);
+  return rc != SALUN_OK ? rc : rs.nslots;
+}
diff --git a/unlearn_saliency_amd/csrc/salun_norm.hip b/unlearn_saliency_amd/csrc/salun_norm.hip
--- a/unlearn_saliency_amd/csrc/salun_norm.hip
+++ b/unlearn_saliency_amd/csrc/salun_norm.hip
@@ -49,6 +49,27 @@
   }
 }
 
+__device__ __forceinline__ void bn_stats_from_sums(double s1, double s2, int c, double M, float eps,
+                                                   float *s_out , bool publish, float momentum,
+                                                   float *__restrict__ mean, float *__restrict__ invstd,
+                                                   float *__restrict__ running_mean, float *__restrict__ running_var) {
+  const double mu = s1 / M;
+  double var = s2 / M - mu * mu;
+  if (var < 0.0) var = 0.0;
+  const float is = (float)(1.0 / sqrt(var + (double)eps));
+  s_out[0] = (float)mu;
+  s_out[1] = is;
+  if (publish) {
+    mean[c] = (float)mu;
+    invstd[c] = is;
+    if (running_mean) {
+      running_mean[c] = (1.f - momentum) * running_mean[c] + momentum * (float)mu;
+      const double unbiased = (M > 1.0) ? var * M / (M - 1.0) : var;
+      running_var[c] = (1.f - momentum) * running_var[c] + momentum * (float)unbiased;
+    }
+  }
+}
+
 __device__ __forceinline__ void bn_channel_stats(const double *__restrict__ partial, int c, int nsplit, double M,
                                                  float eps, float *s_out , bool publish,
                                                  float momentum, float *__restrict__ mean, float *__restrict__ invstd,
@@ -61,25 +82,56 @@
     }
     s1 = salun_wave_sum(s1);
     s2 = salun_wave_sum(s2);
-    if (threadIdx.x == 0) {
-      const double mu = s1 / M;
-      double var = s2 / M - mu * mu;
-      if (var < 0.0) var = 0.0;
-      const float is = (float)(1.0 / sqrt(var + (double)eps));
-      s_out[0] = (float)mu;
-      s_out[1] = is;
-      if (publish) {
-        mean[c] = (float)mu;
-        invstd[c] = is;
-        if (running_mean) {
-          running_mean[c] = (1.f - momentum) * running_mean[c] + momentum * (float)mu;
-          const double unbiased = (M > 1.0) ? var * M / (M - 1.0) : var;
-          running_var[c] = (1.f - momentum) * running_var[c] + momentum * (float)unbiased;
-        }
-      }
-    }
-  }
-  __syncthreads();
+    if (threadIdx.x == 0)
+      bn_stats_from_sums(s1, s2, c, M, eps, s_out, publish, momentum, mean, invstd, running_mean, running_var);
+  }
+  __syncthreads();
+}
+
+__device__ __forceinline__ void bn_channel_stats_slots(const double *__restrict__ partial, int c, int nslots, double M,
+                                                       float eps, float *s_out, double *lds4, bool publish,
+                                                       float momentum, float *__restrict__ mean,
+                                                       float *__restrict__ invstd, float *__restrict__ running_mean,
+                                                       float *__restrict__ running_var) {
+  double s1 = 0.0, s2 = 0.0;
+  const double2 *p = reinterpret_cast<const double2 *>(partial) + (size_t)c * nslots;
+  for (int i = threadIdx.x; i < nslots; i += 256) {
+    const double2 v = p[i];
+    s1 += v.x;
+    s2 += v.y;
+  }
+  s1 = salun_block_sum(s1, lds4);
+  s2 = salun_block_sum(s2, lds4);
+  if (threadIdx.x == 0)
+    bn_stats_from_sums(s1, s2, c, M, eps, s_out, publish, momentum, mean, invstd, running_mean, running_var);
+  __syncthreads();
+}
+
+template <bool RELU, bool RES>
+__device__ __forceinline__ void bn_apply_slice(const float *__restrict__ x, const float *__restrict__ res,
+                                               float *__restrict__ y, float a, float b, int c, int s, int N, int C,
+                                               int HW, int nsplit) {
+  const int n_lo = (int)((int64_t)N * s / nsplit), n_hi = (int)((int64_t)N * (s + 1) / nsplit);
+  const int hw4 = HW >> 2;
+  const int work = (n_hi - n_lo) * hw4;
+  BnWalk wk(n_lo, hw4);
+#pragma unroll 2
+  for (int e = threadIdx.x; e < work; e += 256, wk.next()) {
+    const int n = wk.n, i = wk.i;
+    const size_t off = ((size_t)n * C + c) * HW;
+    const float4 v = reinterpret_cast<const float4 *>(x + off)[i];
+    float4 o;
+    o.x = v.x * a + b; o.y = v.y * a + b; o.z = v.z * a + b; o.w = v.w * a + b;
+    if (RES) {
+      const float4 r = reinterpret_cast<const float4 *>(res + off)[i];
+      o.x += r.x; o.y += r.y; o.z += r.z; o.w += r.w;
+    }
+    if (RELU) {
+      o.x = o.x > 0.f ? o.x : 0.f; o.y = o.y > 0.f ? o.y : 0.f;
+      o.z = o.z > 0.f ? o.z : 0.f; o.w = o.w > 0.f ? o.w : 0.f;
+    }
+    reinterpret_cast<float4 *>(y + off)[i] = o;
+  }
 }
 
 template <bool RELU, bool RES, bool TRAIN>
@@ -106,27 +158,28 @@
   }
   const float a = st[1] * gamma[c];
   const float b = beta[c] - st[0] * a;
-  const int n_lo = (int)((int64_t)N * s / nsplit), n_hi = (int)((int64_t)N * (s + 1) / nsplit);
-  const int hw4 = HW >> 2;
-  const int work = (n_hi - n_lo) * hw4;
-  BnWalk wk(n_lo, hw4);
-#pragma unroll 2
-  for (int e = threadIdx.x; e < work; e += 256, wk.next()) {
-    const int n = wk.n, i = wk.i;
-    const size_t off = ((size_t)n * C + c) * HW;
-    const float4 v = reinterpret_cast<const float4 *>(x + off)[i];
-    float4 o;
-    o.x = v.x * a + b; o.y = v.y * a + b; o.z = v.z * a + b; o.w = v.w * a + b;
-    if (RES) {
-      const float4 r = reinterpret_cast<const float4 *>(res + off)[i];
-      o.x += r.x; o.y += r.y; o.z += r.z; o.w += r.w;
-    }
-    if (RELU) {
-      o.x = o.x > 0.f ? o.x : 0.f; o.y = o.y > 0.f ? o.y : 0.f;
-      o.z = o.z > 0.f ? o.z : 0.f; o.w = o.w > 0.f ? o.w : 0.f;
-    }
-    reinterpret_cast<float4 *>(y + off)[i] = o;
-  }
+  bn_apply_slice<RELU, RES>(x, res, y, a, b, c, s, N, C, HW, nsplit);
+}
+
+template <bool RELU, bool RES>
+__global__ __launch_bounds__(256) void k_bn_apply_slots(const float *__restrict__ x, const float *__restrict__ res,
+                                                        float *__restrict__ y, const double *__restrict__ partial,
+                                                        int nslots, float *__restrict__ mean,
+                                                        float *__restrict__ invstd, const float *__restrict__ gamma,
+                                                        const float *__restrict__ beta,
+                                                        float *__restrict__ running_mean,
+                                                        float *__restrict__ running_var,
+                                                        long long *__restrict__ num_batches_tracked, int N, int C,
+                                                        int HW, int nsplit, float eps, float momentum) {
+  __shared__ float st[2];
+  __shared__ double lds4[4];
+  const int c = blockIdx.x, s = blockIdx.y;
+  if (num_batches_tracked && c == 0 && s == 0 && threadIdx.x == 0) *num_batches_tracked += 1;
+  bn_channel_stats_slots(partial, c, nslots, (double)N * HW, eps, st, lds4, s == 0, momentum, mean, invstd,
+                         running_mean, running_var);
+  const float a = st[1] * gamma[c];
+  const float b = beta[c] - st[0] * a;
+  bn_apply_slice<RELU, RES>(x, res, y, a, b, c, s, N, C, HW, nsplit);
 }
 
 template <bool RELU>
@@ -277,6 +330,32 @@
   else if (t) SALUN_BN_APPLY(false, false, true);
   else SALUN_BN_APPLY(false, false, false);
 #undef SALUN_BN_APPLY
+  SALUN_LAUNCH_CHECK();
+  return SALUN_OK;
+}
+
+SALUN_EXPORT int salun_bn_forward_from_partials(const float *x, const float *res, float *y, const float *gamma,
+                                                const float *beta, float *running_mean, float *running_var,
+                                                long long *num_batches_tracked, float *save_mean, float *save_invstd,
+                                                int N, int C, int HW, double momentum, double eps, int relu,
+                                                const double *partials, int nslots, salun_stream_t stream) {
+  if (!x || !y || !gamma || !beta || !save_mean || !save_invstd || !partials || nslots < 1 || N < 1 || C < 1 ||
+      HW < 4 || (HW & 3))
+    return SALUN_EINVAL;
+  if (!salun_aligned16(x) || !salun_aligned16(y) || (res && !salun_aligned16(res)) || !salun_aligned16(partials))
+    return SALUN_EINVAL;
+  hipStream_t st = salun_hip_stream(stream);
+  const int ns = bn_nsplit(N, C);
+#define SALUN_BN_APPLY_SLOTS(RELU_, RES_)                                                                          \
+  hipLaunchKernelGGL((k_bn_apply_slots<RELU_, RES_>), dim3(C, ns), dim3(256), 0, st, x, res, y, partials, nslots,  \
+                     save_mean, save_invstd, gamma, beta, running_mean, running_var, num_batches_tracked, N, C,   \
+                     HW, ns, (float)eps, (float)momentum)
+  const bool r = relu != 0, a = res != nullptr;
+  if (r && a) SALUN_BN_APPLY_SLOTS(true, true);
+  else if (r) SALUN_BN_APPLY_SLOTS(true, false);
+  else if (a) SALUN_BN_APPLY_SLOTS(false, true);
+  else SALUN_BN_APPLY_SLOTS(false, false);
+#undef SALUN_BN_APPLY_SLOTS
   SALUN_LAUNCH_CHECK();
   return SALUN_OK;
 }
diff --git a/unlearn_saliency_amd/ops.py b/unlearn_saliency_amd/ops.py
--- a/unlearn_saliency_amd/ops.py
+++ b/unlearn_saliency_amd/ops.py
@@ -471,6 +471,36 @@
     return y
 
 
+def conv3x3_packed_stats(x: torch.Tensor, img: torch.Tensor, Kout: int, cfg: int = 0,
+                         partials: Optional[torch.Tensor] = None):
+    N, Cred, H, W = x.shape
+    L = _lib.lib()
+    nbytes = _q("salun_conv3x3_stats_bytes", N, Cred, H, W, Kout, int(cfg))
+    y = torch.empty((N, Kout, H, W), dtype=torch.float32, device=x.device)
+    part = None
+    if nbytes:
+        part = partials if partials is not None else torch.empty(nbytes // 8, dtype=torch.float64, device=x.device)
+        if part.dtype != torch.float64 or part.numel() * 8 < nbytes or not part.is_contiguous():
+            raise ValueError(f"partials must be a contiguous float64 tensor of at least {nbytes // 8} elements")
+    rc = L.salun_conv3x3_packed_stats(_dev(x, torch.float32, "x"), c_void_p(img.data_ptr()), c_void_p(y.data_ptr()),
+                                      c_void_p(part.data_ptr() if part is not None else None), c_size_t(nbytes),
+                                      N, Cred, H, W, Kout, int(cfg), _stream())
+    if rc == _lib.SALUN_EINVAL:
+        return None
+    if rc < 0:
+        check(rc, "salun_conv3x3_packed_stats")
+    return (y, part, rc) if rc > 0 else (y, None, 0)
+
+
+def conv2d_forward_stats(x: torch.Tensor, w: torch.Tensor, cfg: int = 0):
+    if tuple(w.shape[2:]) != (3, 3) or x.shape[3] not in (4, 8, 16, 32):
+        return None
+    imgs = ringpack.images(w)
+    if imgs is None:
+        return None
+    return conv3x3_packed_stats(x, imgs[0], w.shape[0], cfg)
+
+
 def channel_sum(dy: torch.Tensor, out: Optional[torch.Tensor] = None, accumulate: bool = False) -> torch.Tensor:
     N, K = dy.shape[0], dy.shape[1]
     HW = dy.shape[2] * dy.shape[3]
@@ -817,6 +847,27 @@
     if rc == _lib.SALUN_EINVAL:
         return None
     check(rc, "salun_bn_forward")
+    return y, mean, invstd
+
+
+def bn_forward_from_partials(x, partials, nslots, res, gamma, beta, running_mean, running_var, momentum, eps, relu,
+                             num_batches_tracked=None):
+    N, C, H, W = x.shape
+    if partials.dtype != torch.float64 or partials.numel() < 2 * C * nslots or nslots < 1:
+        raise ValueError(f"partials must hold {C} x {nslots} x 2 float64 values")
+    y = torch.empty_like(x)
+    mean = torch.empty(C, dtype=torch.float32, device=x.device)
+    invstd = torch.empty(C, dtype=torch.float32, device=x.device)
+    rc = _lib.lib().salun_bn_forward_from_partials(
+        _dev(x, torch.float32, "x"), _dev(res, torch.float32, "res", True), c_void_p(y.data_ptr()),
+        _dev(gamma, torch.float32, "weight"), _dev(beta, torch.float32, "bias"),
+        _dev(running_mean, torch.float32, "running_mean", True), _dev(running_var, torch.float32, "running_var", True),
+        _dev(num_batches_tracked, torch.int64, "num_batches_tracked", True), c_void_p(mean.data_ptr()),
+        c_void_p(invstd.data_ptr()), N, C, H * W, c_double(momentum), c_double(eps), int(bool(relu)),
+        _dev(partials, torch.float64, "partials"), int(nslots), _stream())
+    if rc == _lib.SALUN_EINVAL:
+        return None
+    check(rc, "salun_bn_forward_from_partials")
     return y, mean, invstd
 
 
diff --git a/unlearn_saliency_amd/resblock.py b/unlearn_saliency_amd/resblock.py
--- a/unlearn_saliency_amd/resblock.py
+++ b/unlearn_saliency_amd/resblock.py
@@ -16,9 +16,28 @@
     return bn.running_mean, bn.running_var, bn.training, bn.momentum, bn.eps
 
 
+BN_EPILOGUE_STATS = [os.environ.get("SALUN_BN_EPILOGUE_STATS", "1") != "0"]
+BN_EPILOGUE_CFG = [0]
+
+
+def _conv_s1(x, w, P, Q, stats: bool):
+    if stats:
+        r = ops.conv2d_forward_stats(x, w, BN_EPILOGUE_CFG[0])
+        if r is not None:
+            return r
+    return ops.conv2d_forward(x, w, None, 1, 1, P, Q), None, 0
+
+
+def _bn(c, part, nslots, res, g, b, bn: nn.BatchNorm2d):
+    if nslots:
+        return ops.bn_forward_from_partials(c, part, nslots, res, g, b, bn.running_mean, bn.running_var, bn.momentum,
+                                            bn.eps, True, bn.num_batches_tracked)
+    return ops.bn_forward(c, res, g, b, *_bn_args(bn), True, bn.num_batches_tracked)
+
+
 class _BasicBlockFn(FastFunction):
     @staticmethod
-    def forward(ctx, x, blk, w1, g1, b1, w2, g2, b2, wd, gd, bd):
+    def forward(ctx, x, blk, stats, w1, g1, b1, w2, g2, b2, wd, gd, bd):
         s = blk.conv1.stride[0]
         N, C, H, W = x.shape
         P, Q = (H + 2 - 3) // s + 1, (W + 2 - 3) // s + 1
@@ -37,9 +56,10 @@
                 with torch.cuda.stream(fork):
                     cd, skip, md, idd = shortcut()
                 x.record_stream(fork)
-        c1 = ops.conv2d_forward(x, w1, None, s, 1, P, Q)
-        y1, m1, i1 = ops.bn_forward(c1, None, g1, b1, *_bn_args(blk.bn1), True, blk.bn1.num_batches_tracked)
-        c2 = ops.conv2d_forward(y1, w2, None, 1, 1, P, Q)
+        stats = stats and training
+        c1, part1, ns1 = _conv_s1(x, w1, P, Q, stats) if s == 1 else (ops.conv2d_forward(x, w1, None, s, 1, P, Q), None, 0)
+        y1, m1, i1 = _bn(c1, part1, ns1, None, g1, b1, blk.bn1)
+        c2, part2, ns2 = _conv_s1(y1, w2, P, Q, stats)
         if wd is None:
             skip = x
         elif fork is None:
@@ -49,7 +69,7 @@
             for t in (cd, skip, md, idd):
                 if t is not None:
                     t.record_stream(main)
-        out, m2, i2 = ops.bn_forward(c2, skip, g2, b2, *_bn_args(blk.bn2), True, blk.bn2.num_batches_tracked)
+        out, m2, i2 = _bn(c2, part2, ns2, skip, g2, b2, blk.bn2)
         ctx.save_for_backward(x, c1, y1, c2, out, cd, w1, g1, b1, w2, g2, b2, wd, gd, bd, m1, i1, m2, i2, md, idd)
         ctx.cfg = (s, training)
         return out
@@ -81,7 +101,7 @@
         dw1 = wgrad(x, dc1, w1, s, 1)
         dx = ops.conv2d_backward_data(dc1, w1, x.shape, s, 1, addend=dxd) if ctx.needs_input_grad[0] else None
         wgrad.finish()
-        return dx, None, dw1, dg1, db1, dw2, dg2, db2, dwd, dgd, dbd
+        return dx, None, None, dw1, dg1, db1, dw2, dg2, db2, dwd, dgd, dbd
 
 
 def _probe(blk, shape, device) -> bool:
@@ -145,7 +165,8 @@
         return None
     x = x.contiguous()
     d = blk.downsample
-    return _BasicBlockFn.apply(x, blk, blk.conv1.weight, blk.bn1.weight, blk.bn1.bias, blk.conv2.weight,
+    stats = BN_EPILOGUE_STATS[0] and torch.is_grad_enabled()
+    return _BasicBlockFn.apply(x, blk, stats, blk.conv1.weight, blk.bn1.weight, blk.bn1.bias, blk.conv2.weight,
                                blk.bn2.weight, blk.bn2.bias, d[0].weight if d is not None else None,
                                d[1].weight if d is not None else None, d[1].bias if d is not None else None)
 
```
